# caishiqing/voice-tts

Measured on AMD Instinct MI355X. Metric: audio_seconds_per_second, higher is better.
Workload: dtype bf16

## Files before the change

### include/ixtts_hip.h

```cpp
#ifndef IXTTS_HIP_H
#define IXTTS_HIP_H

#include <stddef.h>
#include <stdint.h>

#ifdef __cplusplus
extern "C" {
#endif

#define IXTTS_OK 0
#define IXTTS_ERR_ARG (-1)
#define IXTTS_ERR_HIP (-2)
#define IXTTS_ERR_STATE (-3)
#define IXTTS_ERR_NOMEM (-4)
#define IXTTS_ERR_NAME (-5)

const char* ixtts_version(void);
const char* ixtts_last_error(void);

int ixtts_aa_snake_f32(const float* x_dev, float* y_dev, const float* up12_dev, const float* down12_dev,
                       const float* log_alpha_dev, const float* log_beta_dev, int B, int C, int T, void* stream);

size_t ixtts_attn_full_workspace_bytes(int B, int H, int T);
int ixtts_attn_full_f32(const float* q_dev, const float* k_dev, const float* v_dev, float* out_dev, int B, int H, int T,
                        int head_dim, long stride_b, long stride_t, long stride_h, long ostride_b, long ostride_t,
                        long ostride_h, float scale, void* workspace_dev, size_t workspace_bytes, void* stream);

size_t ixtts_attn_full_varlen_workspace_bytes(int nseq, int H, int total_tiles);
int ixtts_attn_full_varlen_f32(const float* q_dev, const float* k_dev, const float* v_dev, float* out_dev, const int* table_dev, int nseq,
                               int total_tiles, int n_work, int H, int head_dim, long stride_t, long stride_h, long ostride_t, long ostride_h,
                               float scale, void* workspace_dev, size_t workspace_bytes, void* stream);

int ixtts_adaln_rmsnorm_f32(const float* x_dev, const float* wb_dev, const float* g_dev, float* out_dev, int B, int T, int H, float eps,
                            void* stream);
int ixtts_ln_modulate_f32(const float* x_dev, const float* shift_scale_dev, float* out_dev, int B, int T, int H, float eps, void* stream);
int ixtts_rope_qk_f32(float* qkv_dev, const float* cos_sin_dev, int B, int T, int H, int head_dim, void* stream);
int ixtts_swiglu_f32(const float* u_dev, float* out_dev, long rows, int F, void* stream);
int ixtts_wn_gate_f32(const float* a_dev, const float* g_dev, float* out_dev, int B, int C, int T, long g_stride, int g_offset, void* stream);
int ixtts_wn_gate_rows_f32(const float* a_dev, const float* g_dev, float* out_dev, long rows, int C, long rows_per_batch, int B, long g_stride,
                           int g_offset, void* stream);
int ixtts_reflect_halo_rows_f32(float* p_dev, int B, int T, int C, int left, int right, void* stream);

int ixtts_adaln_rmsnorm_varlen_f32(const float* x_dev, const float* wb_dev, const float* g_dev, float* out_dev, const int* seq_off_dev, int nseq,
                                   long rows, int H, float eps, void* stream);
int ixtts_ln_modulate_varlen_f32(const float* x_dev, const float* shift_scale_dev, float* out_dev, const int* seq_off_dev, int nseq, long rows, int H,
                                 float eps, void* stream);
int ixtts_rope_qk_varlen_f32(float* qkv_dev, const float* cos_sin_dev, const int* seq_off_dev, int nseq, long rows, int H, int head_dim, void* stream);
int ixtts_wn_gate_rows_varlen_f32(const float* a_dev, const float* g_dev, float* out_dev, long rows, int C, const int* seq_off_dev, int nseq,
                                  long g_stride, int g_offset, void* stream);
int ixtts_reflect_halo_rows_varlen_f32(float* p_dev, const int* seq_off_dev, int nseq, int C, int left, int right, void* stream);

size_t ixtts_gemm_x6_packed_bytes(int N, int K);
int ixtts_gemm_x6_pack(const float* w_dev, void* packed_dev, int N, int K, void* stream);
long ixtts_gemm_x6_rows_padded(long rows);
int ixtts_gemm_x6_split(const float* a_dev, long lda, void* planes_dev, long rows, int K, void* stream);
int ixtts_gemm_x6_f32(const void* a_planes_dev, long rows_total, long row0, const void* packed_dev, const float* bias_dev, float* c_dev, long ldc,
                      int M, int N, int K, int accumulate, int tile, void* stream);
int ixtts_gemm_x6_pair_f32(const void* a_planes_dev, long rows_total, long row0, int taps, const void* packed_dev, const float* bias_dev,
                           const float* gate_dev, long gate_ld, long rows_per_batch, int nbatch, float* c_dev, long ldc, int M, int N, int K,
                           int epilogue, int tile, void* stream);
int ixtts_gemm_x6_pair_gate_varlen_f32(const void* a_planes_dev, long rows_total, long row0, int taps, const void* packed_dev, const float* bias_dev,
                                       const float* gate_dev, long gate_ld, const int* seq_off_dev, int nseq, float* c_dev, long ldc, int M, int N,
                                       int K, int tile, void* stream);

#define IXTTS_BIGVGAN_MAX_STAGES 8
#define IXTTS_BIGVGAN_MAX_RESK 4

typedef struct ixtts_bigvgan_cfg {
  int num_mels;
  int upsample_initial_channel;
  int n_stages;
  int upsample_rates[IXTTS_BIGVGAN_MAX_STAGES];
  int upsample_kernel_sizes[IXTTS_BIGVGAN_MAX_STAGES];
  int n_resblock_kernels;
  int resblock_kernel_sizes[IXTTS_BIGVGAN_MAX_RESK];
  int resblock_dilations[IXTTS_BIGVGAN_MAX_RESK][3];
  int max_frames;
  int fast_sin;
} ixtts_bigvgan_cfg;

typedef struct ixtts_bigvgan ixtts_bigvgan;

int ixtts_bigvgan_create(ixtts_bigvgan** out, const ixtts_bigvgan_cfg* cfg);
int ixtts_bigvgan_set_tensor(ixtts_bigvgan* h, const char* name, const float* data_host, const int64_t* shape, int ndim);
int ixtts_bigvgan_finalize(ixtts_bigvgan* h);
int ixtts_bigvgan_arena(ixtts_bigvgan* h, void** ptr_dev, size_t* bytes);
int ixtts_bigvgan_adopt_arena(ixtts_bigvgan* h);
int ixtts_bigvgan_forward(ixtts_bigvgan* h, const float* mel_dev, int B, int F, float* wav_dev, void* stream);
double ixtts_bigvgan_flops(const ixtts_bigvgan* h, int B, int F);
int ixtts_bigvgan_destroy(ixtts_bigvgan* h);

#define IXTTS_DTYPE_F32 0
#define IXTTS_DTYPE_BF16 1

typedef struct ixtts_gpt_cfg {
  int model_dim;
  int layers;
  int heads;
  int n_mel_codes;
  int n_mel_pos;
  int n_text_tokens;
  int n_text_pos;
  int start_mel_token;
  int stop_mel_token;
  int max_seq;
  int max_batch;
  int weight_dtype;
} ixtts_gpt_cfg;

typedef struct ixtts_sampler_cfg {
  float repetition_penalty;
  float temperature;
  int top_k;
  float top_p;
  int do_sample;
  int suppress_stop;
  uint64_t seed;
  float typical_mass;
  float length_penalty;
} ixtts_sampler_cfg;

typedef struct ixtts_gpt ixtts_gpt;

int ixtts_gpt_create(ixtts_gpt** out, const ixtts_gpt_cfg* cfg);
int ixtts_gpt_set_tensor(ixtts_gpt* h, const char* name, const float* data_host, const int64_t* shape, int ndim);
int ixtts_gpt_finalize(ixtts_gpt* h);
int ixtts_gpt_arena(ixtts_gpt* h, void** ptr_dev, size_t* bytes);
int ixtts_gpt_adopt_arena(ixtts_gpt* h);
int ixtts_gpt_share_arena(ixtts_gpt* h, ixtts_gpt* owner);

int ixtts_gpt_prefill(ixtts_gpt* h, int b, const float* embeds_dev, int n_rows, int n_left_pad, void* stream);
int ixtts_gpt_decode(ixtts_gpt* h, int n_active, int n_steps, const ixtts_sampler_cfg* sc, void* stream);
int ixtts_gpt_read(ixtts_gpt* h, int b, int32_t* ids_host, int cap, int* n_ids, int* finished, void* stream);
int ixtts_gpt_read_logits(ixtts_gpt* h, int b, float* logits_host, void* stream);
int ixtts_gpt_read_probs(ixtts_gpt* h, int b, float* probs_host, void* stream);
int ixtts_gpt_force_next(ixtts_gpt* h, int b, int32_t token, void* stream);

int ixtts_gpt_beam_begin(ixtts_gpt* h, int num_beams, void* stream);
int ixtts_gpt_beam_decode(ixtts_gpt* h, int n_steps, const ixtts_sampler_cfg* sc, void* stream);
int ixtts_gpt_beam_read(ixtts_gpt* h, int max_new, int32_t* ids_host, int cap, int* n_ids, int* done, float* score,
                        float* beam_scores_host, int32_t* last_tokens_host, int32_t* beam_idx_host, void* stream);
int ixtts_gpt_beam_force(ixtts_gpt* h, const int32_t* picks_host, int n, void* stream);

int ixtts_gpt_beam_begin_group(ixtts_gpt* h, int group, int num_beams, uint64_t rng_stream, void* stream);
int ixtts_gpt_beam_park_group(ixtts_gpt* h, int group, void* stream);
int ixtts_gpt_beam_decode_groups(ixtts_gpt* h, int n_groups, int n_steps, const ixtts_sampler_cfg* sc, void* stream);
int ixtts_gpt_beam_read_group(ixtts_gpt* h, int group, int max_new, int32_t* ids_host, int cap, int* n_ids, int* done, float* score,
                              float* beam_scores_host, int32_t* last_tokens_host, int32_t* beam_idx_host, void* stream);
int ixtts_gpt_beam_force_group(ixtts_gpt* h, int group, const int32_t* picks_host, int n, void* stream);

int ixtts_gpt_latent(ixtts_gpt* h, const float* prefix_dev, int n_prefix, const int32_t* codes_dev, int n,
                     float* latent_dev, void* stream);

int ixtts_gpt_bench_gemv(ixtts_gpt* h, int which, int layer, int batch, void* stream);
double ixtts_gpt_step_bytes(const ixtts_gpt* h, int B, int S);

int ixtts_gpt_max_batch(void);

int ixtts_gpt_destroy(ixtts_gpt* h);

#define IXTTS_DTYPE_F16 2
#define IXTTS_QWEN_TOPK_MAX 64
#define IXTTS_QWEN_MAX_EOS 8

typedef struct ixtts_qwen_cfg {
  int hidden_size;
  int layers;
  int heads;
  int kv_heads;
  int head_dim;
  int intermediate_size;
  int vocab_size;
  float rms_norm_eps;
  float rope_theta;
  int tie_word_embeddings;
  int max_seq;
  int weight_dtype;
  int n_eos;
  int eos_ids[IXTTS_QWEN_MAX_EOS];
} ixtts_qwen_cfg;

typedef struct ixtts_qwen_sampling {
  int do_sample;
  float temperature;
  int top_k;
  float top_p;
  uint64_t seed;
} ixtts_qwen_sampling;

typedef struct ixtts_qwen ixtts_qwen;

int ixtts_qwen_create(ixtts_qwen** out, const ixtts_qwen_cfg* cfg);
int ixtts_qwen_set_tensor(ixtts_qwen* h, const char* name, const float* data_host, const int64_t* shape, int ndim);
int ixtts_qwen_finalize(ixtts_qwen* h);
int ixtts_qwen_prefill(ixtts_qwen* h, const int32_t* ids_host, int n, void* stream);
int ixtts_qwen_step(ixtts_qwen* h, int n_steps, const ixtts_qwen_sampling* sc, void* stream);
int ixtts_qwen_read(ixtts_qwen* h, int32_t* ids_host, int cap, int* n_ids, int* finished, void* stream);
int ixtts_qwen_generate(ixtts_qwen* h, int max_new, const ixtts_qwen_sampling* sc, int32_t* ids_host, int cap, int* n_ids,
                        int* finished, void* stream);
int ixtts_qwen_read_logits(ixtts_qwen* h, float* logits_host, void* stream);
int ixtts_qwen_read_kept(ixtts_qwen* h, int32_t* ids_host, float* probs_host, int cap, int* n_kept, void* stream);
int ixtts_qwen_draw(ixtts_qwen* h, uint64_t seed, int n, int32_t* ids_host, void* stream);
double ixtts_qwen_step_bytes(const ixtts_qwen* h, int S);
int ixtts_qwen_destroy(ixtts_qwen* h);

#ifdef __cplusplus
}
#endif
#endif
```

### voice-tts_amd/_lib.py

```python
import ctypes as C
import os

HERE = os.path.dirname(os.path.abspath(__file__))
LIB_PATH = os.environ.get("IXTTS_LIB") or os.path.join(HERE, "libixtts_hip.so")

MAX_STAGES = 8
MAX_RESK = 4


class BigVGANCfg(C.Structure):
    _fields_ = [
        ("num_mels", C.c_int), ("upsample_initial_channel", C.c_int), ("n_stages", C.c_int),
        ("upsample_rates", C.c_int * MAX_STAGES), ("upsample_kernel_sizes", C.c_int * MAX_STAGES),
        ("n_resblock_kernels", C.c_int), ("resblock_kernel_sizes", C.c_int * MAX_RESK),
        ("resblock_dilations", (C.c_int * 3) * MAX_RESK), ("max_frames", C.c_int), ("fast_sin", C.c_int),
    ]


class GptCfg(C.Structure):
    _fields_ = [
        ("model_dim", C.c_int), ("layers", C.c_int), ("heads", C.c_int), ("n_mel_codes", C.c_int),
        ("n_mel_pos", C.c_int), ("n_text_tokens", C.c_int), ("n_text_pos", C.c_int),
        ("start_mel_token", C.c_int), ("stop_mel_token", C.c_int), ("max_seq", C.c_int),
        ("max_batch", C.c_int), ("weight_dtype", C.c_int),
    ]


class SamplerCfg(C.Structure):
    _fields_ = [
        ("repetition_penalty", C.c_float), ("temperature", C.c_float), ("top_k", C.c_int),
        ("top_p", C.c_float), ("do_sample", C.c_int), ("suppress_stop", C.c_int), ("seed", C.c_uint64),
        ("typical_mass", C.c_float), ("length_penalty", C.c_float),
    ]


QWEN_TOPK_MAX = 64
QWEN_MAX_EOS = 8


class QwenCfg(C.Structure):
    _fields_ = [
        ("hidden_size", C.c_int), ("layers", C.c_int), ("heads", C.c_int), ("kv_heads", C.c_int), ("head_dim", C.c_int),
        ("intermediate_size", C.c_int), ("vocab_size", C.c_int), ("rms_norm_eps", C.c_float), ("rope_theta", C.c_float),
        ("tie_word_embeddings", C.c_int), ("max_seq", C.c_int), ("weight_dtype", C.c_int), ("n_eos", C.c_int),
        ("eos_ids", C.c_int * QWEN_MAX_EOS),
    ]


class QwenSampling(C.Structure):
    _fields_ = [("do_sample", C.c_int), ("temperature", C.c_float), ("top_k", C.c_int), ("top_p", C.c_float), ("seed", C.c_uint64)]


_P = C.c_void_p
SYMBOLS = {
    "ixtts_version": (C.c_char_p, []),
    "ixtts_last_error": (C.c_char_p, []),
    "ixtts_aa_snake_f32": (C.c_int, [_P, _P, _P, _P, _P, _P, C.c_int, C.c_int, C.c_int, _P]),
    "ixtts_attn_full_workspace_bytes": (C.c_size_t, [C.c_int, C.c_int, C.c_int]),
    "ixtts_attn_full_f32": (C.c_int, [_P, _P, _P, _P, C.c_int, C.c_int, C.c_int, C.c_int, C.c_long, C.c_long, C.c_long, C.c_long, C.c_long,
                                      C.c_long, C.c_float, _P, C.c_size_t, _P]),
    "ixtts_attn_full_varlen_workspace_bytes": (C.c_size_t, [C.c_int, C.c_int, C.c_int]),
    "ixtts_attn_full_varlen_f32": (C.c_int, [_P, _P, _P, _P, _P, C.c_int, C.c_int, C.c_int, C.c_int, C.c_int, C.c_long, C.c_long, C.c_long, C.c_long,
                                             C.c_float, _P, C.c_size_t, _P]),
    "ixtts_adaln_rmsnorm_f32": (C.c_int, [_P, _P, _P, _P, C.c_int, C.c_int, C.c_int, C.c_float, _P]),
    "ixtts_ln_modulate_f32": (C.c_int, [_P, _P, _P, C.c_int, C.c_int, C.c_int, C.c_float, _P]),
    "ixtts_rope_qk_f32": (C.c_int, [_P, _P, C.c_int, C.c_int, C.c_int, C.c_int, _P]),
    "ixtts_swiglu_f32": (C.c_int, [_P, _P, C.c_long, C.c_int, _P]),
    "ixtts_wn_gate_f32": (C.c_int, [_P, _P, _P, C.c_int, C.c_int, C.c_int, C.c_long, C.c_int, _P]),
    "ixtts_wn_gate_rows_f32": (C.c_int, [_P, _P, _P, C.c_long, C.c_int, C.c_long, C.c_int, C.c_long, C.c_int, _P]),
    "ixtts_reflect_halo_rows_f32": (C.c_int, [_P, C.c_int, C.c_int, C.c_int, C.c_int, C.c_int, _P]),
    "ixtts_adaln_rmsnorm_varlen_f32": (C.c_int, [_P, _P, _P, _P, _P, C.c_int, C.c_long, C.c_int, C.c_float, _P]),
    "ixtts_ln_modulate_varlen_f32": (C.c_int, [_P, _P, _P, _P, C.c_int, C.c_long, C.c_int, C.c_float, _P]),
    "ixtts_rope_qk_varlen_f32": (C.c_int, [_P, _P, _P, C.c_int, C.c_long, C.c_int, C.c_int, _P]),
    "ixtts_wn_gate_rows_varlen_f32": (C.c_int, [_P, _P, _P, C.c_long, C.c_int, _P, C.c_int, C.c_long, C.c_int, _P]),
    "ixtts_reflect_halo_rows_varlen_f32": (C.c_int, [_P, _P, C.c_int, C.c_int, C.c_int, C.c_int, _P]),
    "ixtts_gemm_x6_packed_bytes": (C.c_size_t, [C.c_int, C.c_int]),
    "ixtts_gemm_x6_pack": (C.c_int, [_P, _P, C.c_int, C.c_int, _P]),
    "ixtts_gemm_x6_rows_padded": (C.c_long, [C.c_long]),
    "ixtts_gemm_x6_split": (C.c_int, [_P, C.c_long, _P, C.c_long, C.c_int, _P]),
    "ixtts_gemm_x6_f32": (C.c_int, [_P, C.c_long, C.c_long, _P, _P, _P, C.c_long, C.c_int, C.c_int, C.c_int, C.c_int, C.c_int, _P]),
    "ixtts_gemm_x6_pair_f32": (C.c_int, [_P, C.c_long, C.c_long, C.c_int, _P, _P, _P, C.c_long, C.c_long, C.c_int, _P, C.c_long, C.c_int, C.c_int,
                                         C.c_int, C.c_int, C.c_int, _P]),
    "ixtts_gemm_x6_pair_gate_varlen_f32": (C.c_int, [_P, C.c_long, C.c_long, C.c_int, _P, _P, _P, C.c_long, _P, C.c_int, _P, C.c_long, C.c_int, C.c_int,
                                                     C.c_int, C.c_int, _P]),
    "ixtts_bigvgan_create": (C.c_int, [C.POINTER(_P), C.POINTER(BigVGANCfg)]),
    "ixtts_bigvgan_set_tensor": (C.c_int, [_P, C.c_char_p, _P, C.POINTER(C.c_int64), C.c_int]),
    "ixtts_bigvgan_finalize": (C.c_int, [_P]),
    "ixtts_bigvgan_arena": (C.c_int, [_P, C.POINTER(_P), C.POINTER(C.c_size_t)]),
    "ixtts_bigvgan_adopt_arena": (C.c_int, [_P]),
    "ixtts_bigvgan_forward": (C.c_int, [_P, _P, C.c_int, C.c_int, _P, _P]),
    "ixtts_bigvgan_flops": (C.c_double, [_P, C.c_int, C.c_int]),
    "ixtts_bigvgan_destroy": (C.c_int, [_P]),
    "ixtts_gpt_create": (C.c_int, [C.POINTER(_P), C.POINTER(GptCfg)]),
    "ixtts_gpt_set_tensor": (C.c_int, [_P, C.c_char_p, _P, C.POINTER(C.c_int64), C.c_int]),
    "ixtts_gpt_finalize": (C.c_int, [_P]),
    "ixtts_gpt_arena": (C.c_int, [_P, C.POINTER(_P), C.POINTER(C.c_size_t)]),
    "ixtts_gpt_adopt_arena": (C.c_int, [_P]),
    "ixtts_gpt_share_arena": (C.c_int, [_P, _P]),
    "ixtts_gpt_prefill": (C.c_int, [_P, C.c_int, _P, C.c_int, C.c_int, _P]),
    "ixtts_gpt_decode": (C.c_int, [_P, C.c_int, C.c_int, C.POINTER(SamplerCfg), _P]),
    "ixtts_gpt_read": (C.c_int, [_P, C.c_int, _P, C.c_int, C.POINTER(C.c_int), C.POINTER(C.c_int), _P]),
    "ixtts_gpt_read_logits": (C.c_int, [_P, C.c_int, _P, _P]),
    "ixtts_gpt_beam_begin": (C.c_int, [_P, C.c_int, _P]),
    "ixtts_gpt_beam_decode": (C.c_int, [_P, C.c_int, C.POINTER(SamplerCfg), _P]),
    "ixtts_gpt_beam_read": (C.c_int, [_P, C.c_int, _P, C.c_int, C.POINTER(C.c_int), C.POINTER(C.c_int), C.POINTER(C.c_float), _P, _P, _P, _P]),
    "ixtts_gpt_beam_force": (C.c_int, [_P, _P, C.c_int, _P]),
    "ixtts_gpt_beam_begin_group": (C.c_int, [_P, C.c_int, C.c_int, C.c_uint64, _P]),
    "ixtts_gpt_beam_park_group": (C.c_int, [_P, C.c_int, _P]),
    "ixtts_gpt_beam_decode_groups": (C.c_int, [_P, C.c_int, C.c_int, C.POINTER(SamplerCfg), _P]),
    "ixtts_gpt_beam_read_group": (C.c_int, [_P, C.c_int, C.c_int, _P, C.c_int, C.POINTER(C.c_int), C.POINTER(C.c_int), C.POINTER(C.c_float), _P, _P, _P, _P]),
    "ixtts_gpt_beam_force_group": (C.c_int, [_P, C.c_int, _P, C.c_int, _P]),
    "ixtts_gpt_read_probs": (C.c_int, [_P, C.c_int, _P, _P]),
    "ixtts_gpt_force_next": (C.c_int, [_P, C.c_int, C.c_int32, _P]),
    "ixtts_gpt_latent": (C.c_int, [_P, _P, C.c_int, _P, C.c_int, _P, _P]),
    "ixtts_gpt_bench_gemv": (C.c_int, [_P, C.c_int, C.c_int, C.c_int, _P]),
    "ixtts_gpt_step_bytes": (C.c_double, [_P, C.c_int, C.c_int]),
    "ixtts_gpt_max_batch": (C.c_int, []),
    "ixtts_gpt_destroy": (C.c_int, [_P]),
    "ixtts_qwen_create": (C.c_int, [C.POINTER(_P), C.POINTER(QwenCfg)]),
    "ixtts_qwen_set_tensor": (C.c_int, [_P, C.c_char_p, _P, C.POINTER(C.c_int64), C.c_int]),
    "ixtts_qwen_finalize": (C.c_int, [_P]),
    "ixtts_qwen_prefill": (C.c_int, [_P, _P, C.c_int, _P]),
    "ixtts_qwen_step": (C.c_int, [_P, C.c_int, C.POINTER(QwenSampling), _P]),
    "ixtts_qwen_read": (C.c_int, [_P, _P, C.c_int, C.POINTER(C.c_int), C.POINTER(C.c_int), _P]),
    "ixtts_qwen_generate": (C.c_int, [_P, C.c_int, C.POINTER(QwenSampling), _P, C.c_int, C.POINTER(C.c_int), C.POINTER(C.c_int), _P]),
    "ixtts_qwen_read_logits": (C.c_int, [_P, _P, _P]),
    "ixtts_qwen_read_kept": (C.c_int, [_P, _P, _P, C.c_int, C.POINTER(C.c_int), _P]),
    "ixtts_qwen_draw": (C.c_int, [_P, C.c_uint64, C.c_int, _P, _P]),
    "ixtts_qwen_step_bytes": (C.c_double, [_P, C.c_int]),
    "ixtts_qwen_destroy": (C.c_int, [_P]),
}

_lib = None


class IxttsError(RuntimeError):
    pass


def lib():
    global _lib
    if _lib is not None:
        return _lib
    import torch

    if not os.path.exists(LIB_PATH):
        raise IxttsError(
            f"{LIB_PATH} not found: build it with `python -m voice_tts_amd.build` "
            "(there is no CPU fallback for the HIP path)")
    L = C.CDLL(LIB_PATH)
    for name, (res, args) in SYMBOLS.items():
        fn = getattr(L, name)
        fn.restype = res
        fn.argtypes = args
    _lib = L
    return L


def check(rc, what=""):
    if rc != 0:
        msg = lib().ixtts_last_error().decode(errors="replace")
        raise IxttsError(f"{what} failed with code {rc}: {msg}")


def max_batch():
    return int(lib().ixtts_gpt_max_batch())


def current_stream_ptr():
    import torch

    return C.c_void_p(torch.cuda.current_stream().cuda_stream)
```

### voice-tts_amd/csrc/attn_full.h

```cpp
#pragma once
#include "common.h"

namespace ixtts {

constexpr int AF_D = 64;
constexpr int AF_KT = 64;
constexpr int AF_QW = 32;
constexpr int AF_WAVES = 4;
constexpr int AF_KSPLIT = 4;
constexpr int AX_KSPLIT = 5;

struct AttnFullArgs {
  const float* q;
  const float* k;
  const float* v;
  float* o;
  long sb, st, sh;
  long osb, ost, osh;
  int B, H, T;
  float scale;
  float* ws_o;
  float* ws_ml;
  const int* vl_tab;
  int vl_n, vl_tiles;
};

size_t attn_full_x3_plane_bytes(int B, int H, int T);
int launch_attn_full_x3(const AttnFullArgs& a, void* planes, bool split, hipStream_t st);
int launch_attn_full_x3_varlen(const AttnFullArgs& a, void* planes, int n_work, hipStream_t st);

}
```

### voice-tts_amd/csrc/attn_full.hip

```cpp
#include "attn_full.h"

namespace ixtts {

typedef float f32x16 __attribute__((ext_vector_type(16)));

constexpr int AF_KP = AF_D + 4;

template <int KSPLIT>
__global__ __launch_bounds__(AF_WAVES * 64) void attn_full_f32_kernel(AttnFullArgs a) {
  __shared__ __attribute__((aligned(16))) float Ks[AF_KT * AF_KP];
  __shared__ __attribute__((aligned(16))) float Vs[AF_KT * AF_D];
  const int bh = blockIdx.y, b = bh / a.H, h = bh % a.H;
  const int lane = threadIdx.x & 63, wave = threadIdx.x >> 6;
  const int l31 = lane & 31, lh = lane >> 5;
  const int q0 = blockIdx.x * (AF_WAVES * AF_QW) + wave * AF_QW;
  const float* qb = a.q + b * a.sb + h * a.sh;
  const float* kb = a.k + b * a.sb + h * a.sh;
  const float* vb = a.v + b * a.sb + h * a.sh;

  float qr[AF_D / 2];
  {
    const int qi = min(q0 + l31, a.T - 1);
    const float* qp = qb + (long)qi * a.st + 4 * lh;
    const float qs = a.scale * 1.4426950408889634f;
#pragma unroll
    for (int m = 0; m < AF_D / 8; ++m) {
      const float4 t = *reinterpret_cast<const float4*>(qp + 8 * m);
      qr[4 * m] = t.x * qs; qr[4 * m + 1] = t.y * qs; qr[4 * m + 2] = t.z * qs; qr[4 * m + 3] = t.w * qs;
    }
  }
  f32x16 ot[2];
#pragma unroll
  for (int j = 0; j < 2; ++j)
#pragma unroll
    for (int r = 0; r < 16; ++r) ot[j][r] = 0.f;
  float m_run = -INFINITY, l_run = 0.f;

  const int n_tiles = (a.T + AF_KT - 1) / AF_KT;
  const int tiles_per = (n_tiles + KSPLIT - 1) / KSPLIT;
  const int t_lo = (KSPLIT > 1 ? blockIdx.z * tiles_per : 0) * AF_KT;
  const int t_hi = KSPLIT > 1 ? min(a.T, t_lo + tiles_per * AF_KT) : a.T;
  for (int t0 = t_lo; t0 < t_hi; t0 += AF_KT) {
    __syncthreads();
#pragma unroll
    for (int i = 0; i < (AF_KT * AF_D / 4) / (AF_WAVES * 64); ++i) {
      const int idx = threadIdx.x + i * (AF_WAVES * 64);
      const int key = idx >> 4, c4 = idx & 15;
      const int t = min(t0 + key, a.T - 1);
      const float4 kv = *reinterpret_cast<const float4*>(kb + (long)t * a.st + c4 * 4);
      const float4 vv = *reinterpret_cast<const float4*>(vb + (long)t * a.st + c4 * 4);
      *reinterpret_cast<float4*>(Ks + key * AF_KP + c4 * 4) = kv;
      *reinterpret_cast<float4*>(Vs + key * AF_D + c4 * 4) = vv;
    }
    __syncthreads();

    f32x16 st[2];
#pragma unroll
    for (int j = 0; j < 2; ++j)
#pragma unroll
      for (int r = 0; r < 16; ++r) st[j][r] = 0.f;
    const float* kp0 = Ks + l31 * AF_KP + 4 * lh;
    const float* kp1 = kp0 + 32 * AF_KP;
    float4 ka[2][2];
    ka[0][0] = *reinterpret_cast<const float4*>(kp0);
    ka[0][1] = *reinterpret_cast<const float4*>(kp1);
#pragma unroll
    for (int m = 0; m < AF_D / 8; ++m) {
      if (m + 1 < AF_D / 8) {
        ka[(m + 1) & 1][0] = *reinterpret_cast<const float4*>(kp0 + 8 * (m + 1));
        ka[(m + 1) & 1][1] = *reinterpret_cast<const float4*>(kp1 + 8 * (m + 1));
      }
#pragma unroll
      for (int j = 0; j < 2; ++j) {
        const float4 kk4 = ka[m & 1][j];
        st[j] = __builtin_amdgcn_mfma_f32_32x32x2f32(kk4.x, qr[4 * m], st[j], 0, 0, 0);
        st[j] = __builtin_amdgcn_mfma_f32_32x32x2f32(kk4.y, qr[4 * m + 1], st[j], 0, 0, 0);
        st[j] = __builtin_amdgcn_mfma_f32_32x32x2f32(kk4.z, qr[4 * m + 2], st[j], 0, 0, 0);
        st[j] = __builtin_amdgcn_mfma_f32_32x32x2f32(kk4.w, qr[4 * m + 3], st[j], 0, 0, 0);
      }
    }
    if (t0 + AF_KT > a.T) {
#pragma unroll
      for (int j = 0; j < 2; ++j)
#pragma unroll
        for (int r = 0; r < 16; ++r) {
          const int key = t0 + j * 32 + (r & 3) + 8 * (r >> 2) + 4 * lh;
          if (key >= a.T) st[j][r] = -INFINITY;
        }
    }
    float tmax = -INFINITY;
#pragma unroll
    for (int j = 0; j < 2; ++j)
#pragma unroll
      for (int r = 0; r < 16; ++r) tmax = fmaxf(tmax, st[j][r]);
    tmax = fmaxf(tmax, __shfl_xor(tmax, 32, 64));
    const float mn = fmaxf(m_run, tmax);
    const float alpha = __builtin_amdgcn_exp2f(m_run - mn);
    m_run = mn;
    if (alpha != 1.0f) {
#pragma unroll
      for (int j = 0; j < 2; ++j)
#pragma unroll
        for (int r = 0; r < 16; ++r) ot[j][r] *= alpha;
    }
    float psum = 0.f;
    const float* vp = Vs + (4 * lh) * AF_D + l31;
    float va[2][2];
    va[0][0] = vp[0];
    va[0][1] = vp[32];
#pragma unroll
    for (int s = 0; s < 32; ++s) {
      const int j = s >> 4, r = s & 15;
      if (s + 1 < 32) {
        const int j1 = (s + 1) >> 4, r1 = (s + 1) & 15;
        const float* vrow = vp + (j1 * 32 + (r1 & 3) + 8 * (r1 >> 2)) * AF_D;
        va[(s + 1) & 1][0] = vrow[0];
        va[(s + 1) & 1][1] = vrow[32];
      }
      const float pv = __builtin_amdgcn_exp2f(st[j][r] - mn);
      psum += pv;
      ot[0] = __builtin_amdgcn_mfma_f32_32x32x2f32(va[s & 1][0], pv, ot[0], 0, 0, 0);
      ot[1] = __builtin_amdgcn_mfma_f32_32x32x2f32(va[s & 1][1], pv, ot[1], 0, 0, 0);
    }
    psum += __shfl_xor(psum, 32, 64);
    l_run = l_run * alpha + psum;
  }
  const int qi = q0 + l31;
  if (qi < a.T) {
    if constexpr (KSPLIT == 1) {
      const float inv = 1.0f / l_run;
      float* op = a.o + b * a.osb + (long)qi * a.ost + h * a.osh;
#pragma unroll
      for (int j = 0; j < 2; ++j)
#pragma unroll
        for (int r = 0; r < 16; ++r) op[j * 32 + (r & 3) + 8 * (r >> 2) + 4 * lh] = ot[j][r] * inv;
    } else {
      const long row = ((long)blockIdx.z * a.B * a.H + bh) * a.T + qi;
      float* op = a.ws_o + row * AF_D;
#pragma unroll
      for (int j = 0; j < 2; ++j)
#pragma unroll
        for (int r = 0; r < 16; ++r) op[j * 32 + (r & 3) + 8 * (r >> 2) + 4 * lh] = ot[j][r];
      if (lh == 0) *reinterpret_cast<float2*>(a.ws_ml + row * 2) = make_float2(m_run, l_run);
    }
  }
}

template <int KSPLIT>
__global__ __launch_bounds__(256) void attn_full_merge_kernel(AttnFullArgs a) {
  const long row = (long)blockIdx.x * 4 + (threadIdx.x >> 6);
  const long rows = (long)a.B * a.H * a.T;
  if (row >= rows) return;
  const int d = threadIdx.x & 63;
  const int t = (int)(row % a.T);
  const int bh = (int)(row / a.T), b = bh / a.H, h = bh % a.H;
  float2 ml[KSPLIT];
  float o[KSPLIT];
  float M = -INFINITY;
#pragma unroll
  for (int sp = 0; sp < KSPLIT; ++sp) {
    ml[sp] = *reinterpret_cast<const float2*>(a.ws_ml + ((long)sp * rows + row) * 2);
    o[sp] = a.ws_o[((long)sp * rows + row) * AF_D + d];
    M = fmaxf(M, ml[sp].x);
  }
  float L = 0.f, O = 0.f;
#pragma unroll
  for (int sp = 0; sp < KSPLIT; ++sp) {
    const float w = (ml[sp].x > -INFINITY) ? __builtin_amdgcn_exp2f(ml[sp].x - M) : 0.f;
    L = fmaf(ml[sp].y, w, L);
    O = fmaf(o[sp], w, O);
  }
  a.o[b * a.osb + (long)t * a.ost + h * a.osh + d] = O / L;
}

}

static size_t attn_partials_bytes(int B, int H, int T) {
  return (size_t)(ixtts::AF_KSPLIT > ixtts::AX_KSPLIT ? ixtts::AF_KSPLIT : ixtts::AX_KSPLIT) * B * H * T * (ixtts::AF_D + 2) * sizeof(float);
}

extern "C" size_t ixtts_attn_full_workspace_bytes(int B, int H, int T) {
  if (B <= 0 || H <= 0 || T <= 0) return 0;
  return attn_partials_bytes(B, H, T) + ixtts::attn_full_x3_plane_bytes(B, H, T);
}

extern "C" int ixtts_attn_full_f32(const float* q_dev, const float* k_dev, const float* v_dev, float* out_dev, int B, int H, int T,
                                   int head_dim, long stride_b, long stride_t, long stride_h, long ostride_b, long ostride_t,
                                   long ostride_h, float scale, void* workspace_dev, size_t workspace_bytes, void* stream) {
  using namespace ixtts;
  IX_ARG(q_dev && k_dev && v_dev && out_dev, "attn_full: null pointer");
  IX_ARG(head_dim == AF_D, "attn_full: head_dim %d (only 64 is built)", head_dim);
  IX_ARG(B > 0 && H > 0 && T > 0 && (long)B * H <= 65535, "attn_full: bad shape B=%d H=%d T=%d", B, H, T);
  IX_ARG(stride_t % 4 == 0 && stride_h % 4 == 0 && stride_b % 4 == 0, "attn_full: strides must keep 16-byte row alignment");
  AttnFullArgs a;
  a.q = q_dev; a.k = k_dev; a.v = v_dev; a.o = out_dev;
  a.sb = stride_b; a.st = stride_t; a.sh = stride_h;
  a.osb = ostride_b; a.ost = ostride_t; a.osh = ostride_h;
  a.B = B; a.H = H; a.T = T; a.scale = scale;
  a.ws_o = a.ws_ml = nullptr;
  a.vl_tab = nullptr; a.vl_n = a.vl_tiles = 0;
  hipStream_t st = (hipStream_t)stream;
  const int qblocks = ceil_div(T, AF_WAVES * AF_QW);
  const bool have_ws = workspace_dev && workspace_bytes >= ixtts_attn_full_workspace_bytes(B, H, T);
  const bool split = have_ws && T > 4 * AF_KT && (long)qblocks * B * H * AF_WAVES < 2 * 1024;
  const char* mode = getenv("IXTTS_ATTN_FULL");
  const bool x3 = !(mode && strcmp(mode, "f32") == 0);
  const bool use_x3 = x3 && have_ws;
  if (split) {
    a.ws_o = reinterpret_cast<float*>(workspace_dev);
    a.ws_ml = a.ws_o + (size_t)(use_x3 ? AX_KSPLIT : AF_KSPLIT) * B * H * T * AF_D;
  }
  if (use_x3) {
    IX_TRY(launch_attn_full_x3(a, reinterpret_cast<char*>(workspace_dev) + attn_partials_bytes(B, H, T), split, st));
    if (split) {
      const long rows = (long)B * H * T;
      hipLaunchKernelGGL(attn_full_merge_kernel<AX_KSPLIT>, dim3((unsigned)((rows + 3) / 4)), dim3(256), 0, st, a);
    }
    IX_HIP(hipGetLastError());
    return IXTTS_OK;
  }
  if (split) {
    hipLaunchKernelGGL(attn_full_f32_kernel<AF_KSPLIT>, dim3(qblocks, B * H, AF_KSPLIT), dim3(AF_WAVES * 64), 0, st, a);
    const long rows = (long)B * H * T;
    hipLaunchKernelGGL(attn_full_merge_kernel<AF_KSPLIT>, dim3((unsigned)((rows + 3) / 4)), dim3(256), 0, st, a);
  } else {
    hipLaunchKernelGGL(attn_full_f32_kernel<1>, dim3(qblocks, B * H), dim3(AF_WAVES * 64), 0, st, a);
  }
  IX_HIP(hipGetLastError());
  return IXTTS_OK;
}

extern "C" size_t ixtts_attn_full_varlen_workspace_bytes(int nseq, int H, int total_tiles) {
  if (nseq <= 0 || H <= 0 || total_tiles <= 0) return 0;
  return (size_t)H * total_tiles * 2 * 3 * 8 * 64 * 16;
}

extern "C" int ixtts_attn_full_varlen_f32(const float* q_dev, const float* k_dev, const float* v_dev, float* out_dev, const int* table_dev, int nseq,
                                          int total_tiles, int n_work, int H, int head_dim, long stride_t, long stride_h, long ostride_t, long ostride_h,
                                          float scale, void* workspace_dev, size_t workspace_bytes, void* stream) {
  using namespace ixtts;
  IX_ARG(q_dev && k_dev && v_dev && out_dev && table_dev, "attn_full_varlen: null pointer");
  IX_ARG(head_dim == AF_D, "attn_full_varlen: head_dim %d (only 64 is built)", head_dim);
  IX_ARG(nseq > 0 && total_tiles >= nseq && n_work >= nseq && H > 0 && H <= 65535, "attn_full_varlen: bad shape nseq=%d tiles=%d work=%d H=%d", nseq, total_tiles,
         n_work, H);
  IX_ARG(stride_t % 4 == 0 && stride_h % 4 == 0, "attn_full_varlen: strides must keep 16-byte row alignment");
  IX_ARG(workspace_dev && workspace_bytes >= ixtts_attn_full_varlen_workspace_bytes(nseq, H, total_tiles), "attn_full_varlen: workspace of %zu bytes, %zu needed",
         workspace_bytes, ixtts_attn_full_varlen_workspace_bytes(nseq, H, total_tiles));
  AttnFullArgs a;
  a.q = q_dev; a.k = k_dev; a.v = v_dev; a.o = out_dev;
  a.sb = 0; a.st = stride_t; a.sh = stride_h;
  a.osb = 0; a.ost = ostride_t; a.osh = ostride_h;
  a.B = 1; a.H = H; a.T = 0; a.scale = scale;
  a.ws_o = a.ws_ml = nullptr;
  a.vl_tab = table_dev; a.vl_n = nseq; a.vl_tiles = total_tiles;
  return launch_attn_full_x3_varlen(a, workspace_dev, n_work, (hipStream_t)stream);
}
```

### voice-tts_amd/csrc/attn_full_x3.hip

```cpp
#include "attn_full.h"

namespace ixtts {

typedef float ax_f32x16 __attribute__((ext_vector_type(16)));
typedef __bf16 ax_bf16x8 __attribute__((ext_vector_type(8)));

constexpr int AX_TILE_UNITS = 3 * 8 * 64;
constexpr int AX_WAVES = 4;

size_t attn_full_x3_plane_bytes(int B, int H, int T) {
  const size_t tiles = (size_t)(T + AF_KT - 1) / AF_KT;
  return (size_t)B * H * tiles * 2 * AX_TILE_UNITS * 16;
}


template <bool VL>
__global__ __launch_bounds__(256) void attn_kv_planes_kernel(AttnFullArgs a, uint4* __restrict__ planes) {
  int tile = blockIdx.x, T = a.T;
  const float *kb, *vb;
  uint4* kdst;
  if constexpr (VL) {
    const int h = blockIdx.y, s = seq_of_row(a.vl_tab + a.vl_n + 1, a.vl_n, tile);
    const int r0 = a.vl_tab[s];
    T = a.vl_tab[s + 1] - r0;
    kdst = planes + ((size_t)h * a.vl_tiles + tile) * 2 * AX_TILE_UNITS;
    tile -= a.vl_tab[a.vl_n + 1 + s];
    kb = a.k + (long)r0 * a.st + h * a.sh;
    vb = a.v + (long)r0 * a.st + h * a.sh;
  } else {
    const int bh = blockIdx.y, b = bh / a.H, h = bh % a.H;
    const int n_tiles = (a.T + AF_KT - 1) / AF_KT;
    kb = a.k + b * a.sb + h * a.sh;
    vb = a.v + b * a.sb + h * a.sh;
    kdst = planes + ((size_t)bh * n_tiles + tile) * 2 * AX_TILE_UNITS;
  }
  uint4* vdst = kdst + AX_TILE_UNITS;
  const int t0 = tile * AF_KT;
#pragma unroll
  for (int i = 0; i < 2; ++i) {
    const int uid = threadIdx.x + 256 * i;
    const int key = uid >> 3, oct = uid & 7;
    const int t = t0 + key;
    float v[8];
    const float4* src = reinterpret_cast<const float4*>(kb + (long)min(t, T - 1) * a.st + 8 * oct);
    const float4 x0 = src[0], x1 = src[1];
    const bool live = t < T;
    v[0] = live ? x0.x : 0.f; v[1] = live ? x0.y : 0.f; v[2] = live ? x0.z : 0.f; v[3] = live ? x0.w : 0.f;
    v[4] = live ? x1.x : 0.f; v[5] = live ? x1.y : 0.f; v[6] = live ? x1.z : 0.f; v[7] = live ? x1.w : 0.f;
    uint4 ph, pm, pl;
    split8_bf16x3(v, ph, pm, pl);
    kdst[(0 * 8 + oct) * 64 + key] = ph;
    kdst[(1 * 8 + oct) * 64 + key] = pm;
    kdst[(2 * 8 + oct) * 64 + key] = pl;
  }
#pragma unroll
  for (int i = 0; i < 2; ++i) {
    const int d = threadIdx.x & 63, un = (threadIdx.x >> 6) + 4 * i;
    const int j = un >> 2, u = (un >> 1) & 1, kh = un & 1;
    float v[8];
#pragma unroll
    for (int e = 0; e < 8; ++e) {
      const int t = t0 + 32 * j + 16 * u + 8 * (e >> 2) + 4 * kh + (e & 3);
      const float x = vb[(long)min(t, T - 1) * a.st + d];
      v[e] = t < T ? x : 0.f;
    }
    uint4 ph, pm, pl;
    split8_bf16x3(v, ph, pm, pl);
    vdst[(0 * 8 + un) * 64 + d] = ph;
    vdst[(1 * 8 + un) * 64 + d] = pm;
    vdst[(2 * 8 + un) * 64 + d] = pl;
  }
}

template <int KSPLIT, bool VL = false>
__global__ __launch_bounds__(AX_WAVES * 64, 3) void attn_full_x3_kernel(AttnFullArgs a, const uint4* __restrict__ planes) {
  __shared__ uint4 Ks[AX_TILE_UNITS];
  __shared__ uint4 Vs[AX_TILE_UNITS];
  static_assert(!VL || KSPLIT == 1, "packed sequences: no key-range split");
  const int lane = threadIdx.x & 63, wave = threadIdx.x >> 6;
  const int l31 = lane & 31, lh = lane >> 5;
  int T, q0;
  const float* qb;
  const uint4* pb;
  float* ob;
  if constexpr (VL) {
    const int h = blockIdx.y;
    const int* w = a.vl_tab + 2 * (a.vl_n + 1) + 2 * blockIdx.x;
    const int s = w[0], r0 = a.vl_tab[s];
    T = a.vl_tab[s + 1] - r0;
    q0 = w[1] * (AX_WAVES * AF_QW) + wave * AF_QW;
    qb = a.q + (long)r0 * a.st + h * a.sh;
    pb = planes + ((size_t)h * a.vl_tiles + a.vl_tab[a.vl_n + 1 + s]) * 2 * AX_TILE_UNITS;
    ob = a.o + (long)r0 * a.ost + h * a.osh;
  } else {
    const int bh = blockIdx.y, b = bh / a.H, h = bh % a.H;
    T = a.T;
    q0 = blockIdx.x * (AX_WAVES * AF_QW) + wave * AF_QW;
    qb = a.q + b * a.sb + h * a.sh;
    pb = planes + (size_t)bh * ((T + AF_KT - 1) / AF_KT) * 2 * AX_TILE_UNITS;
    ob = a.o + b * a.osb + h * a.osh;
  }

  uint4 qp[4][3];
  {
    const int qi = min(q0 + l31, T - 1);
    const float* qrow = qb + (long)qi * a.st + 8 * lh;
    const float qs = a.scale * 1.4426950408889634f;
#pragma unroll
    for (int s = 0; s < 4; ++s) {
      const float4 x0 = *reinterpret_cast<const float4*>(qrow + 16 * s), x1 = *reinterpret_cast<const float4*>(qrow + 16 * s + 4);
      const float v[8] = {x0.x * qs, x0.y * qs, x0.z * qs, x0.w * qs, x1.x * qs, x1.y * qs, x1.z * qs, x1.w * qs};
      split8_bf16x3(v, qp[s][0], qp[s][1], qp[s][2]);
    }
  }
  ax_f32x16 ot[2];
#pragma unroll
  for (int j = 0; j < 2; ++j)
#pragma unroll
    for (int r = 0; r < 16; ++r) ot[j][r] = 0.f;
  float m_run = -INFINITY, l_run = 0.f;

  const int n_tiles = (T + AF_KT - 1) / AF_KT;
  const int tiles_per = (n_tiles + KSPLIT - 1) / KSPLIT;
  const int tile_lo = KSPLIT > 1 ? blockIdx.z * tiles_per : 0;
  const int tile_hi = KSPLIT > 1 ? min(n_tiles, tile_lo + tiles_per) : n_tiles;
  auto issue_tile = [&](const uint4* __restrict__ src, uint4* __restrict__ dst) {
#pragma unroll
    for (int i = 0; i < AX_TILE_UNITS / (AX_WAVES * 64); ++i)
      __builtin_amdgcn_global_load_lds((const __attribute__((address_space(1))) void*)(src + i * (AX_WAVES * 64) + threadIdx.x),
                                       (__attribute__((address_space(3))) void*)(dst + i * (AX_WAVES * 64) + wave * 64), 16, 0, 0);
  };
  auto mfma6x2 = [](ax_f32x16& c0, ax_f32x16& c1, const uint4 (&A0)[3], const uint4 (&A1)[3], const uint4 (&Bq)[3]) {
    const ax_bf16x8 a0h = __builtin_bit_cast(ax_bf16x8, A0[0]), a0m = __builtin_bit_cast(ax_bf16x8, A0[1]), a0l = __builtin_bit_cast(ax_bf16x8, A0[2]);
    const ax_bf16x8 a1h = __builtin_bit_cast(ax_bf16x8, A1[0]), a1m = __builtin_bit_cast(ax_bf16x8, A1[1]), a1l = __builtin_bit_cast(ax_bf16x8, A1[2]);
    const ax_bf16x8 bh_ = __builtin_bit_cast(ax_bf16x8, Bq[0]), bm = __builtin_bit_cast(ax_bf16x8, Bq[1]), bl = __builtin_bit_cast(ax_bf16x8, Bq[2]);
    c0 = __builtin_amdgcn_mfma_f32_32x32x16_bf16(a0l, bh_, c0, 0, 0, 0);
    c1 = __builtin_amdgcn_mfma_f32_32x32x16_bf16(a1l, bh_, c1, 0, 0, 0);
    c0 = __builtin_amdgcn_mfma_f32_32x32x16_bf16(a0h, bl, c0, 0, 0, 0);
    c1 = __builtin_amdgcn_mfma_f32_32x32x16_bf16(a1h, bl, c1, 0, 0, 0);
    c0 = __builtin_amdgcn_mfma_f32_32x32x16_bf16(a0m, bm, c0, 0, 0, 0);
    c1 = __builtin_amdgcn_mfma_f32_32x32x16_bf16(a1m, bm, c1, 0, 0, 0);
    c0 = __builtin_amdgcn_mfma_f32_32x32x16_bf16(a0m, bh_, c0, 0, 0, 0);
    c1 = __builtin_amdgcn_mfma_f32_32x32x16_bf16(a1m, bh_, c1, 0, 0, 0);
    c0 = __builtin_amdgcn_mfma_f32_32x32x16_bf16(a0h, bm, c0, 0, 0, 0);
    c1 = __builtin_amdgcn_mfma_f32_32x32x16_bf16(a1h, bm, c1, 0, 0, 0);
    c0 = __builtin_amdgcn_mfma_f32_32x32x16_bf16(a0h, bh_, c0, 0, 0, 0);
    c1 = __builtin_amdgcn_mfma_f32_32x32x16_bf16(a1h, bh_, c1, 0, 0, 0);
  };
  if (tile_lo < tile_hi) issue_tile(pb + (size_t)tile_lo * 2 * AX_TILE_UNITS, Ks);
  for (int tile = tile_lo; tile < tile_hi; ++tile) {
    const int t0 = tile * AF_KT;
    asm volatile("s_waitcnt vmcnt(0)" ::: "memory");
    __builtin_amdgcn_s_barrier();
    issue_tile(pb + ((size_t)tile * 2 + 1) * AX_TILE_UNITS, Vs);
    ax_f32x16 st[2];
#pragma unroll
    for (int j = 0; j < 2; ++j)
#pragma unroll
      for (int r = 0; r < 16; ++r) st[j][r] = 0.f;
    const uint4* kp = Ks + lh * 64 + l31;
#pragma unroll
    for (int s = 0; s < 4; ++s) {
      uint4 ka[2][3];
#pragma unroll
      for (int j = 0; j < 2; ++j)
#pragma unroll
        for (int pl = 0; pl < 3; ++pl) ka[j][pl] = kp[(pl * 8 + 2 * s) * 64 + 32 * j];
      mfma6x2(st[0], st[1], ka[0], ka[1], qp[s]);
    }
    if (t0 + AF_KT > T) {
#pragma unroll
      for (int j = 0; j < 2; ++j)
#pragma unroll
        for (int r = 0; r < 16; ++r) {
          const int key = t0 + j * 32 + (r & 3) + 8 * (r >> 2) + 4 * lh;
          if (key >= T) st[j][r] = -INFINITY;
        }
    }
    float tmax = -INFINITY;
#pragma unroll
    for (int j = 0; j < 2; ++j)
#pragma unroll
      for (int r = 0; r < 16; ++r) tmax = fmaxf(tmax, st[j][r]);
    tmax = fmaxf(tmax, __shfl_xor(tmax, 32, 64));
    const float mn = fmaxf(m_run, tmax);
    const float alpha = __builtin_amdgcn_exp2f(m_run - mn);
    m_run = mn;
    if (alpha != 1.0f) {
#pragma unroll
      for (int j = 0; j < 2; ++j)
#pragma unroll
        for (int r = 0; r < 16; ++r) ot[j][r] *= alpha;
    }
    float psum = 0.f;
#pragma unroll
    for (int j = 0; j < 2; ++j)
#pragma unroll
      for (int r = 0; r < 16; ++r) {
        st[j][r] = __builtin_amdgcn_exp2f(st[j][r] - mn);
        psum += st[j][r];
      }
    psum += __shfl_xor(psum, 32, 64);
    l_run = l_run * alpha + psum;
    asm volatile("s_waitcnt vmcnt(0)" ::: "memory");
    __builtin_amdgcn_s_barrier();
    if (tile + 1 < tile_hi) issue_tile(pb + (size_t)(tile + 1) * 2 * AX_TILE_UNITS, Ks);
    const uint4* vp = Vs + lh * 64 + l31;
#pragma unroll
    for (int s = 0; s < 4; ++s) {
      const int j = s >> 1, u = s & 1;
      uint4 va[2][3];
#pragma unroll
      for (int dh = 0; dh < 2; ++dh)
#pragma unroll
        for (int pl = 0; pl < 3; ++pl) va[dh][pl] = vp[(pl * 8 + 2 * s) * 64 + 32 * dh];
      uint4 pp[3];
      {
        float pv[8];
#pragma unroll
        for (int e = 0; e < 8; ++e) pv[e] = st[j][8 * u + e];
        split8_bf16x3(pv, pp[0], pp[1], pp[2]);
      }
      mfma6x2(ot[0], ot[1], va[0], va[1], pp);
    }
  }
  asm volatile("s_waitcnt vmcnt(0)" ::: "memory");
  const int qi = q0 + l31;
  if (qi < T) {
    if constexpr (KSPLIT == 1) {
      const float inv = 1.0f / l_run;
      float* op = ob + (long)qi * a.ost;
#pragma unroll
      for (int j = 0; j < 2; ++j)
#pragma unroll
        for (int r = 0; r < 16; ++r) op[j * 32 + (r & 3) + 8 * (r >> 2) + 4 * lh] = ot[j][r] * inv;
    } else {
      const long row = ((long)blockIdx.z * a.B * a.H + blockIdx.y) * T + qi;
      float* op = a.ws_o + row * AF_D;
#pragma unroll
      for (int j = 0; j < 2; ++j)
#pragma unroll
        for (int r = 0; r < 16; ++r) op[j * 32 + (r & 3) + 8 * (r >> 2) + 4 * lh] = ot[j][r];
      if (lh == 0) *reinterpret_cast<float2*>(a.ws_ml + row * 2) = make_float2(m_run, l_run);
    }
  }
}

int launch_attn_full_x3(const AttnFullArgs& a, void* planes, bool split, hipStream_t st) {
  const int n_tiles = ceil_div(a.T, AF_KT);
  const int qblocks = ceil_div(a.T, AX_WAVES * AF_QW);
  uint4* pl = reinterpret_cast<uint4*>(planes);
  hipLaunchKernelGGL(attn_kv_planes_kernel<false>, dim3(n_tiles, a.B * a.H), dim3(256), 0, st, a, pl);
  if (split) hipLaunchKernelGGL(attn_full_x3_kernel<AX_KSPLIT>, dim3(qblocks, a.B * a.H, AX_KSPLIT), dim3(AX_WAVES * 64), 0, st, a, (const uint4*)pl);
  else hipLaunchKernelGGL(attn_full_x3_kernel<1>, dim3(qblocks, a.B * a.H), dim3(AX_WAVES * 64), 0, st, a, (const uint4*)pl);
  IX_HIP(hipGetLastError());
  return IXTTS_OK;
}

int launch_attn_full_x3_varlen(const AttnFullArgs& a, void* planes, int n_work, hipStream_t st) {
  uint4* pl = reinterpret_cast<uint4*>(planes);
  hipLaunchKernelGGL(attn_kv_planes_kernel<true>, dim3(a.vl_tiles, a.H), dim3(256), 0, st, a, pl);
  hipLaunchKernelGGL((attn_full_x3_kernel<1, true>), dim3(n_work, a.H), dim3(AX_WAVES * 64), 0, st, a, (const uint4*)pl);
  IX_HIP(hipGetLastError());
  return IXTTS_OK;
}

}
```

### voice-tts_amd/csrc/dit_ops.hip

```cpp
#include "common.h"

namespace ixtts {

constexpr int ROW_NV = 8;

template <bool CENTER>
__global__ __launch_bounds__(256) void row_norm_mod_kernel(const float* __restrict__ x, const float* __restrict__ mw, const float* __restrict__ mb,
                                                           const float* __restrict__ g, float* __restrict__ out, long rows, int T, int H, long mstride,
                                                           float eps, float wadd, const int* __restrict__ seq_off = nullptr, int nseq = 0) {
  const long row = (long)blockIdx.x * 4 + (threadIdx.x >> 6);
  if (row >= rows) return;
  const int lane = threadIdx.x & 63;
  const int H4 = H >> 2;
  const float4* xr = reinterpret_cast<const float4*>(x + row * H);
  float4 v[ROW_NV];
#pragma unroll
  for (int i = 0; i < ROW_NV; ++i) {
    const int c = lane + 64 * i;
    v[i] = (c < H4) ? xr[c] : make_float4(0.f, 0.f, 0.f, 0.f);
  }
  float mean = 0.f;
  if constexpr (CENTER) {
    float s = 0.f;
#pragma unroll
    for (int i = 0; i < ROW_NV; ++i) s += (v[i].x + v[i].y) + (v[i].z + v[i].w);
    mean = wave_sum(s) / (float)H;
  }
  float q = 0.f;
#pragma unroll
  for (int i = 0; i < ROW_NV; ++i) {
    const int c = lane + 64 * i;
    if (c < H4) {
      const float a = v[i].x - mean, b = v[i].y - mean, cc = v[i].z - mean, d = v[i].w - mean;
      q += (a * a + b * b) + (cc * cc + d * d);
    }
  }
  const float rstd = 1.0f / sqrtf(wave_sum(q) / (float)H + eps);
  const long bidx = seq_off ? seq_of_row(seq_off, nseq, row) : row / T;
  const float4* w4 = reinterpret_cast<const float4*>(mw + bidx * mstride);
  const float4* b4 = reinterpret_cast<const float4*>(mb + bidx * mstride);
  const float4* g4 = reinterpret_cast<const float4*>(g);
  float4* o4 = reinterpret_cast<float4*>(out + row * H);
#pragma unroll
  for (int i = 0; i < ROW_NV; ++i) {
    const int c = lane + 64 * i;
    if (c < H4) {
      const float4 w = w4[c], b = b4[c];
      float4 n = make_float4((v[i].x - mean) * rstd, (v[i].y - mean) * rstd, (v[i].z - mean) * rstd, (v[i].w - mean) * rstd);
      if (g) {
        const float4 gg = g4[c];
        n.x *= gg.x; n.y *= gg.y; n.z *= gg.z; n.w *= gg.w;
      }
      o4[c] = make_float4(fmaf(w.x + wadd, n.x, b.x), fmaf(w.y + wadd, n.y, b.y), fmaf(w.z + wadd, n.z, b.z), fmaf(w.w + wadd, n.w, b.w));
    }
  }
}

__global__ __launch_bounds__(256) void rope_qk_kernel(float* __restrict__ qkv, const float2* __restrict__ tab, long rows, int T, int H, int hd,
                                                      const int* __restrict__ seq_off = nullptr, int nseq = 0) {
  const int per_row = (2 * H) >> 2;
  const long idx = (long)blockIdx.x * 256 + threadIdx.x;
  if (idx >= rows * per_row) return;
  const long row = idx / per_row;
  const int c4 = (int)(idx % per_row);
  const int col = c4 * 4;
  const int t = seq_off ? (int)(row - seq_off[seq_of_row(seq_off, nseq, row)]) : (int)(row % T);
  const int p = (col % hd) >> 1;
  float4* ptr = reinterpret_cast<float4*>(qkv + row * 3 * H + col);
  const float4 v = *ptr;
  const float2 f0 = tab[(long)t * (hd >> 1) + p], f1 = tab[(long)t * (hd >> 1) + p + 1];
  *ptr = make_float4(v.x * f0.x - v.y * f0.y, v.y * f0.x + v.x * f0.y, v.z * f1.x - v.w * f1.y, v.w * f1.x + v.z * f1.y);
}

__global__ __launch_bounds__(256) void swiglu_kernel(const float* __restrict__ u, float* __restrict__ out, long rows, int Fd) {
  const int F4 = Fd >> 2;
  const long idx = (long)blockIdx.x * 256 + threadIdx.x;
  if (idx >= rows * F4) return;
  const long row = idx / F4;
  const int c = (int)(idx % F4);
  const float4 a = reinterpret_cast<const float4*>(u + row * 2 * Fd)[c];
  const float4 b = reinterpret_cast<const float4*>(u + row * 2 * Fd + Fd)[c];
  auto f = [](float x, float y) { return x / (1.0f + expf(-x)) * y; };
  reinterpret_cast<float4*>(out + row * Fd)[c] = make_float4(f(a.x, b.x), f(a.y, b.y), f(a.z, b.z), f(a.w, b.w));
}

__global__ __launch_bounds__(256) void wn_gate_kernel(const float* __restrict__ a, const float* __restrict__ gvec, float* __restrict__ out, int B, int C, int T,
                                                      long gstride, int goff) {
  const long idx = (long)blockIdx.x * 256 + threadIdx.x;
  const long n = (long)B * C * T;
  if (idx >= n) return;
  const int t = (int)(idx % T);
  const int c = (int)((idx / T) % C);
  const int b = (int)(idx / ((long)T * C));
  const float ga = gvec[b * gstride + goff + c], gb = gvec[b * gstride + goff + C + c];
  const float xa = a[((long)b * 2 * C + c) * T + t] + ga;
  const float xb = a[((long)b * 2 * C + C + c) * T + t] + gb;
  out[idx] = tanhf(xa) * (1.0f / (1.0f + expf(-xb)));
}

__global__ __launch_bounds__(256) void wn_gate_rows_kernel(const float* __restrict__ a, const float* __restrict__ gvec, float* __restrict__ out, long rows, int C,
                                                           long rows_per_batch, int B, long gstride, int goff, const int* __restrict__ seq_off = nullptr) {
  const long idx = (long)blockIdx.x * 256 + threadIdx.x;
  const int C4 = C >> 2;
  if (idx >= rows * C4) return;
  const long r = idx / C4;
  const int c = (int)(idx % C4) * 4;
  const int b = seq_off ? seq_of_row(seq_off, B, r) : (int)min(r / rows_per_batch, (long)B - 1);
  const float4 xa = *reinterpret_cast<const float4*>(a + r * 2 * C + c);
  const float4 xb = *reinterpret_cast<const float4*>(a + r * 2 * C + C + c);
  const float4 ga = *reinterpret_cast<const float4*>(gvec + b * gstride + goff + c);
  const float4 gb = *reinterpret_cast<const float4*>(gvec + b * gstride + goff + C + c);
  float4 o;
  o.x = tanhf(xa.x + ga.x) * (1.0f / (1.0f + expf(-(xb.x + gb.x))));
  o.y = tanhf(xa.y + ga.y) * (1.0f / (1.0f + expf(-(xb.y + gb.y))));
  o.z = tanhf(xa.z + ga.z) * (1.0f / (1.0f + expf(-(xb.z + gb.z))));
  o.w = tanhf(xa.w + ga.w) * (1.0f / (1.0f + expf(-(xb.w + gb.w))));
  *reinterpret_cast<float4*>(out + r * C + c) = o;
}

__global__ __launch_bounds__(256) void reflect_halo_rows_kernel(float* __restrict__ p, int B, int T, int C, int left, int right) {
  const int C4 = C >> 2;
  const long idx = (long)blockIdx.x * 256 + threadIdx.x;
  const long per_b = (long)(left + right) * C4;
  if (idx >= per_b * B) return;
  const int b = (int)(idx / per_b);
  const int h = (int)((idx % per_b) / C4);
  const int c = (int)(idx % C4) * 4;
  float* base = p + (long)b * (left + T + right) * C;
  const int dst = h < left ? left - 1 - h : left + T + (h - left);
  const int src = h < left ? left + h + 1 : left + T - 2 - (h - left);
  *reinterpret_cast<float4*>(base + (long)dst * C + c) = *reinterpret_cast<const float4*>(base + (long)src * C + c);
}

__global__ __launch_bounds__(256) void reflect_halo_rows_varlen_kernel(float* __restrict__ p, const int* __restrict__ off, int n, int C, int left, int right) {
  const int C4 = C >> 2;
  const long idx = (long)blockIdx.x * 256 + threadIdx.x;
  const long per_b = (long)(left + right) * C4;
  if (idx >= per_b * n) return;
  const int b = (int)(idx / per_b);
  const int h = (int)((idx % per_b) / C4);
  const int c = (int)(idx % C4) * 4;
  const int o0 = off[b], T = off[b + 1] - o0 - left - right;
  if (T <= left || T <= right) return;
  float* base = p + (long)o0 * C;
  const int dst = h < left ? left - 1 - h : left + T + (h - left);
  const int src = h < left ? left + h + 1 : left + T - 2 - (h - left);
  *reinterpret_cast<float4*>(base + (long)dst * C + c) = *reinterpret_cast<const float4*>(base + (long)src * C + c);
}

}

using namespace ixtts;

extern "C" int ixtts_adaln_rmsnorm_f32(const float* x_dev, const float* wb_dev, const float* g_dev, float* out_dev, int B, int T, int H, float eps,
                                       void* stream) {
  IX_ARG(x_dev && wb_dev && g_dev && out_dev, "adaln_rmsnorm: null pointer");
  IX_ARG(B > 0 && T > 0 && H > 0 && H % 4 == 0 && H <= 64 * ROW_NV * 4, "adaln_rmsnorm: bad shape B=%d T=%d H=%d", B, T, H);
  const long rows = (long)B * T;
  hipLaunchKernelGGL(row_norm_mod_kernel<false>, dim3((unsigned)((rows + 3) / 4)), dim3(256), 0, (hipStream_t)stream, x_dev, wb_dev, wb_dev + H, g_dev, out_dev,
                     rows, T, H, (long)2 * H, eps, 0.0f);
  IX_HIP(hipGetLastError());
  return IXTTS_OK;
}

extern "C" int ixtts_ln_modulate_f32(const float* x_dev, const float* shift_scale_dev, float* out_dev, int B, int T, int H, float eps, void* stream) {
  IX_ARG(x_dev && shift_scale_dev && out_dev, "ln_modulate: null pointer");
  IX_ARG(B > 0 && T > 0 && H > 0 && H % 4 == 0 && H <= 64 * ROW_NV * 4, "ln_modulate: bad shape B=%d T=%d H=%d", B, T, H);
  const long rows = (long)B * T;
  hipLaunchKernelGGL(row_norm_mod_kernel<true>, dim3((unsigned)((rows + 3) / 4)), dim3(256), 0, (hipStream_t)stream, x_dev, shift_scale_dev + H, shift_scale_dev,
                     (const float*)nullptr, out_dev, rows, T, H, (long)2 * H, eps, 1.0f);
  IX_HIP(hipGetLastError());
  return IXTTS_OK;
}

extern "C" int ixtts_rope_qk_f32(float* qkv_dev, const float* cos_sin_dev, int B, int T, int H, int head_dim, void* stream) {
  IX_ARG(qkv_dev && cos_sin_dev, "rope_qk: null pointer");
  IX_ARG(B > 0 && T > 0 && H > 0 && head_dim > 0 && head_dim % 4 == 0 && H % head_dim == 0, "rope_qk: bad shape B=%d T=%d H=%d hd=%d", B, T, H, head_dim);
  const long n = (long)B * T * (2 * H / 4);
  hipLaunchKernelGGL(rope_qk_kernel, dim3((unsigned)((n + 255) / 256)), dim3(256), 0, (hipStream_t)stream, qkv_dev, reinterpret_cast<const float2*>(cos_sin_dev),
                     (long)B * T, T, H, head_dim);
  IX_HIP(hipGetLastError());
  return IXTTS_OK;
}

extern "C" int ixtts_swiglu_f32(const float* u_dev, float* out_dev, long rows, int F, void* stream) {
  IX_ARG(u_dev && out_dev, "swiglu: null pointer");
  IX_ARG(rows > 0 && F > 0 && F % 4 == 0, "swiglu: bad shape rows=%ld F=%d", rows, F);
  const long n = rows * (F / 4);
  hipLaunchKernelGGL(swiglu_kernel, dim3((unsigned)((n + 255) / 256)), dim3(256), 0, (hipStream_t)stream, u_dev, out_dev, rows, F);
  IX_HIP(hipGetLastError());
  return IXTTS_OK;
}

extern "C" int ixtts_wn_gate_f32(const float* a_dev, const float* g_dev, float* out_dev, int B, int C, int T, long g_stride, int g_offset, void* stream) {
  IX_ARG(a_dev && g_dev && out_dev, "wn_gate: null pointer");
  IX_ARG(B > 0 && C > 0 && T > 0 && g_offset >= 0, "wn_gate: bad shape B=%d C=%d T=%d", B, C, T);
  const long n = (long)B * C * T;
  hipLaunchKernelGGL(wn_gate_kernel, dim3((unsigned)((n + 255) / 256)), dim3(256), 0, (hipStream_t)stream, a_dev, g_dev, out_dev, B, C, T, g_stride, g_offset);
  IX_HIP(hipGetLastError());
  return IXTTS_OK;
}

extern "C" int ixtts_wn_gate_rows_f32(const float* a_dev, const float* g_dev, float* out_dev, long rows, int C, long rows_per_batch, int B, long g_stride,
                                      int g_offset, void* stream) {
  IX_ARG(a_dev && g_dev && out_dev, "wn_gate_rows: null pointer");
  IX_ARG(rows > 0 && C > 0 && C % 4 == 0 && rows_per_batch > 0 && B > 0 && g_offset >= 0 && g_offset % 4 == 0 && g_stride % 4 == 0,
         "wn_gate_rows: bad shape rows=%ld C=%d rows_per_batch=%ld B=%d", rows, C, rows_per_batch, B);
  const long n = rows * (C / 4);
  hipLaunchKernelGGL(wn_gate_rows_kernel, dim3((unsigned)((n + 255) / 256)), dim3(256), 0, (hipStream_t)stream, a_dev, g_dev, out_dev, rows, C, rows_per_batch, B,
                     g_stride, g_offset);
  IX_HIP(hipGetLastError());
  return IXTTS_OK;
}

extern "C" int ixtts_reflect_halo_rows_f32(float* p_dev, int B, int T, int C, int left, int right, void* stream) {
  IX_ARG(p_dev, "reflect_halo_rows: null pointer");
  IX_ARG(B > 0 && C > 0 && C % 4 == 0 && left >= 0 && right >= 0 && T > left && T > right, "reflect_halo_rows: bad shape B=%d T=%d C=%d left=%d right=%d", B, T, C,
         left, right);
  const long n = (long)B * (left + right) * (C / 4);
  if (n == 0) return IXTTS_OK;
  hipLaunchKernelGGL(reflect_halo_rows_kernel, dim3((unsigned)((n + 255) / 256)), dim3(256), 0, (hipStream_t)stream, p_dev, B, T, C, left, right);
  IX_HIP(hipGetLastError());
  return IXTTS_OK;
}


extern "C" int ixtts_adaln_rmsnorm_varlen_f32(const float* x_dev, const float* wb_dev, const float* g_dev, float* out_dev, const int* seq_off_dev, int nseq,
                                              long rows, int H, float eps, void* stream) {
  IX_ARG(x_dev && wb_dev && g_dev && out_dev && seq_off_dev, "adaln_rmsnorm_varlen: null pointer");
  IX_ARG(nseq > 0 && rows > 0 && H > 0 && H % 4 == 0 && H <= 64 * ROW_NV * 4, "adaln_rmsnorm_varlen: bad shape nseq=%d rows=%ld H=%d", nseq, rows, H);
  hipLaunchKernelGGL(row_norm_mod_kernel<false>, dim3((unsigned)((rows + 3) / 4)), dim3(256), 0, (hipStream_t)stream, x_dev, wb_dev, wb_dev + H, g_dev, out_dev,
                     rows, 1, H, (long)2 * H, eps, 0.0f, seq_off_dev, nseq);
  IX_HIP(hipGetLastError());
  return IXTTS_OK;
}

extern "C" int ixtts_ln_modulate_varlen_f32(const float* x_dev, const float* shift_scale_dev, float* out_dev, const int* seq_off_dev, int nseq, long rows, int H,
                                            float eps, void* stream) {
  IX_ARG(x_dev && shift_scale_dev && out_dev && seq_off_dev, "ln_modulate_varlen: null pointer");
  IX_ARG(nseq > 0 && rows > 0 && H > 0 && H % 4 == 0 && H <= 64 * ROW_NV * 4, "ln_modulate_varlen: bad shape nseq=%d rows=%ld H=%d", nseq, rows, H);
  hipLaunchKernelGGL(row_norm_mod_kernel<true>, dim3((unsigned)((rows + 3) / 4)), dim3(256), 0, (hipStream_t)stream, x_dev, shift_scale_dev + H, shift_scale_dev,
                     (const float*)nullptr, out_dev, rows, 1, H, (long)2 * H, eps, 1.0f, seq_off_dev, nseq);
  IX_HIP(hipGetLastError());
  return IXTTS_OK;
}

extern "C" int ixtts_rope_qk_varlen_f32(float* qkv_dev, const float* cos_sin_dev, const int* seq_off_dev, int nseq, long rows, int H, int head_dim, void* stream) {
  IX_ARG(qkv_dev && cos_sin_dev && seq_off_dev, "rope_qk_varlen: null pointer");
  IX_ARG(nseq > 0 && rows > 0 && H > 0 && head_dim > 0 && head_dim % 4 == 0 && H % head_dim == 0, "rope_qk_varlen: bad shape nseq=%d rows=%ld H=%d hd=%d", nseq,
         rows, H, head_dim);
  const long n = rows * (2 * H / 4);
  hipLaunchKernelGGL(rope_qk_kernel, dim3((unsigned)((n + 255) / 256)), dim3(256), 0, (hipStream_t)stream, qkv_dev, reinterpret_cast<const float2*>(cos_sin_dev),
                     rows, 1, H, head_dim, seq_off_dev, nseq);
  IX_HIP(hipGetLastError());
  return IXTTS_OK;
}

extern "C" int ixtts_wn_gate_rows_varlen_f32(const float* a_dev, const float* g_dev, float* out_dev, long rows, int C, const int* seq_off_dev, int nseq,
                                             long g_stride, int g_offset, void* stream) {
  IX_ARG(a_dev && g_dev && out_dev && seq_off_dev, "wn_gate_rows_varlen: null pointer");
  IX_ARG(rows > 0 && C > 0 && C % 4 == 0 && nseq > 0 && g_offset >= 0 && g_offset % 4 == 0 && g_stride % 4 == 0,
         "wn_gate_rows_varlen: bad shape rows=%ld C=%d nseq=%d", rows, C, nseq);
  const long n = rows * (C / 4);
  hipLaunchKernelGGL(wn_gate_rows_kernel, dim3((unsigned)((n + 255) / 256)), dim3(256), 0, (hipStream_t)stream, a_dev, g_dev, out_dev, rows, C, (long)1, nseq,
                     g_stride, g_offset, seq_off_dev);
  IX_HIP(hipGetLastError());
  return IXTTS_OK;
}

extern "C" int ixtts_reflect_halo_rows_varlen_f32(float* p_dev, const int* seq_off_dev, int nseq, int C, int left, int right, void* stream) {
  IX_ARG(p_dev && seq_off_dev, "reflect_halo_rows_varlen: null pointer");
  IX_ARG(nseq > 0 && C > 0 && C % 4 == 0 && left >= 0 && right >= 0, "reflect_halo_rows_varlen: bad shape nseq=%d C=%d left=%d right=%d", nseq, C, left, right);
  const long n = (long)nseq * (left + right) * (C / 4);
  if (n == 0) return IXTTS_OK;
  hipLaunchKernelGGL(reflect_halo_rows_varlen_kernel, dim3((unsigned)((n + 255) / 256)), dim3(256), 0, (hipStream_t)stream, p_dev, seq_off_dev, nseq, C, left,
                     right);
  IX_HIP(hipGetLastError());
  return IXTTS_OK;
}
```

### voice-tts_amd/csrc/gemm_x6.hip

```cpp
#include "common.h"

namespace ixtts {

typedef float gx_f32x16 __attribute__((ext_vector_type(16)));
typedef __bf16 gx_bf16x8 __attribute__((ext_vector_type(8)));
typedef float gx_f32x4 __attribute__((ext_vector_type(4)));
typedef unsigned int gx_u32x4 __attribute__((ext_vector_type(4)));


__global__ void gemm_x6_pack_kernel(const float* __restrict__ w, uint4* __restrict__ out, int N, int K, int Npad) {
  const long total = (long)(K / 8) * Npad;
  for (long idx = blockIdx.x * (long)blockDim.x + threadIdx.x; idx < total; idx += (long)gridDim.x * blockDim.x) {
    const int n = (int)(idx % Npad);
    const int ko = (int)(idx / Npad);
    float v[8];
#pragma unroll
    for (int e = 0; e < 8; ++e) v[e] = n < N ? w[(long)n * K + ko * 8 + e] : 0.f;
    uint4 ph, pm, pl;
    split8_bf16x3(v, ph, pm, pl);
    const int g = ko >> 1, kh = ko & 1;
    uint4* base = out + ((long)g * 6) * Npad + n;
    base[(long)(0 * 2 + kh) * Npad] = ph;
    base[(long)(1 * 2 + kh) * Npad] = pm;
    base[(long)(2 * 2 + kh) * Npad] = pl;
  }
}

__global__ __launch_bounds__(256) void gemm_x6_split_kernel(const float* __restrict__ a, long lda, uint4* __restrict__ out, int M, int K, long Mpad) {
  __shared__ float tile[64][65];
  const int r0 = blockIdx.x * 64, k0 = blockIdx.y * 64;
  const int t = threadIdx.x;
#pragma unroll
  for (int i = 0; i < 4; ++i) {
    const int r = (t >> 4) + 16 * i, kq = t & 15;
    float4 v = make_float4(0.f, 0.f, 0.f, 0.f);
    if (r0 + r < M) v = *reinterpret_cast<const float4*>(a + (long)(r0 + r) * lda + k0 + 4 * kq);
    tile[r][4 * kq + 0] = v.x; tile[r][4 * kq + 1] = v.y; tile[r][4 * kq + 2] = v.z; tile[r][4 * kq + 3] = v.w;
  }
  __syncthreads();
#pragma unroll
  for (int u = 0; u < 2; ++u) {
    const int r = t & 63, o = (t >> 6) + 4 * u;
    float v[8];
#pragma unroll
    for (int e = 0; e < 8; ++e) v[e] = tile[r][o * 8 + e];
    uint4 ph, pm, pl;
    split8_bf16x3(v, ph, pm, pl);
    const int ko = (k0 >> 3) + o, g = ko >> 1, kh = ko & 1;
    uint4* base = out + ((long)g * 6) * Mpad + r0 + r;
    base[(long)(0 * 2 + kh) * Mpad] = ph;
    base[(long)(1 * 2 + kh) * Mpad] = pm;
    base[(long)(2 * 2 + kh) * Mpad] = pl;
  }
}

enum { EPI_PLAIN = 0, EPI_SWIGLU = 1, EPI_GATE = 2 };

struct GemmX6Params {
  const uint4* Ap;
  long Mpad;
  long arow0;
  const uint4* Wp;
  const float* bias;
  float* C;
  long ldc;
  int M, N, Npad, K, accumulate, m_tiles, n_tiles;
  int tap_steps;
  int epi;
  const float* gate;
  long gate_ld, rows_per_batch;
  int nbatch;
  const int* gate_seq_off;
  unsigned long long* dbg;
};


template <int MT, int NT, int NST, int EPI = EPI_PLAIN, int ACC = 0, int SEQ = 0, int DBG = 0, int PIN = 0>
__global__ __launch_bounds__(256, (NST * (MT + NT) * 6 * 64 * 16 <= 80 * 1024) ? 2 : 1) void gemm_x6_kernel(GemmX6Params p) {
  constexpr int BM = 64 * MT, BN = 64 * NT;
  constexpr int A_UNITS = 6 * BM, W_UNITS = 6 * BN, STAGE = A_UNITS + W_UNITS;
  constexpr int NDMA = (6 * (MT + NT)) / 4;
  constexpr int NA = (6 * MT) / 4, NW = NDMA - NA;
  static_assert((6 * MT) % 4 == 0 && (6 * NT) % 4 == 0, "the A pieces and the W pieces are each dealt evenly to the 4 waves");
  static_assert(EPI == EPI_PLAIN || (ACC == 0 && NT == 2), "pair epilogues: the wave's two 32-column blocks are the two halves");
  static_assert(EPI == EPI_GATE || SEQ == 0, "the sequence table belongs to the gate epilogue");
  constexpr int D = NST - 1;
  extern __shared__ uint4 smem[];

  const int nwg = p.m_tiles * p.n_tiles;
  const int bid = blockIdx.x;
  const int xcd = bid & 7, idx = bid >> 3;
  const int qd = nwg >> 3, rm = nwg & 7;
  const int lin = (xcd < rm ? xcd * (qd + 1) : rm * (qd + 1) + (xcd - rm) * qd) + idx;
  const int m_tile = lin / p.n_tiles, n_tile = lin - m_tile * p.n_tiles;
  const int m0 = m_tile * BM, n0 = n_tile * BN;

  const int tid = threadIdx.x, lane = tid & 63;
  const int wave = __builtin_amdgcn_readfirstlane(tid >> 6);
  const int wm = wave >> 1, wn = wave & 1;
  const int l31 = lane & 31, lh = lane >> 5;

  gx_f32x16 acc[MT][NT];
#pragma unroll
  for (int i = 0; i < MT; ++i)
#pragma unroll
    for (int j = 0; j < NT; ++j)
#pragma unroll
      for (int r = 0; r < 16; ++r) acc[i][j][r] = 0.f;

  const uint4* asrc = p.Ap + p.arow0 + m0 + lane;
  const uint4* wsrc = p.Wp + n0 + lane;
  long a_off[NA], w_off[NW];
  int a_lds[NA], w_lds[NW];
#pragma unroll
  for (int q = 0; q < NA; ++q) {
    const int e = q * 4 + wave, run = e / MT, piece = e % MT;
    a_off[q] = run * p.Mpad + piece * 64;
    a_lds[q] = run * BM + piece * 64;
  }
#pragma unroll
  for (int q = 0; q < NW; ++q) {
    const int e = q * 4 + wave, run = e / NT, piece = e % NT;
    w_off[q] = (long)run * p.Npad + piece * 64;
    w_lds[q] = A_UNITS + run * BN + piece * 64;
  }
  const long a_step = 6 * p.Mpad, w_step = 6L * p.Npad;
  const long a_wrap = 1 - p.tap_steps * a_step;
  long a_run = 0, w_run = 0;
  int a_group = 0;
  auto issue_next = [&](uint4* st) {
#pragma unroll
    for (int q = 0; q < NA; ++q)
      __builtin_amdgcn_global_load_lds((const __attribute__((address_space(1))) void*)(asrc + (a_off[q] + a_run)),
                                       (__attribute__((address_space(3))) void*)(st + a_lds[q]), 16, 0, 0);
#pragma unroll
    for (int q = 0; q < NW; ++q)
      __builtin_amdgcn_global_load_lds((const __attribute__((address_space(1))) void*)(wsrc + (w_off[q] + w_run)),
                                       (__attribute__((address_space(3))) void*)(st + w_lds[q]), 16, 0, 0);
    a_run += a_step;
    w_run += w_step;
    if (++a_group == p.tap_steps) {
      a_group = 0;
      a_run += a_wrap;
    }
  };

  const int steps = p.K >> 4;
  auto wg_stamp = [&](int k) {
    if constexpr (DBG == 3) {
      if (tid == 0) p.dbg[128 + (long)blockIdx.x * 4 + k] = __builtin_amdgcn_s_memrealtime();
    }
  };
  auto wait_younger = [&](int y) {
    if (y >= 2) asm volatile("s_waitcnt vmcnt(%0)" ::"n"(2 * NDMA) : "memory");
    else if (y == 1) asm volatile("s_waitcnt vmcnt(%0)" ::"n"(NDMA) : "memory");
    else asm volatile("s_waitcnt vmcnt(0)" ::: "memory");
  };
  static_assert(D >= 1 && D <= 3, "1..3 steps of copies in flight behind the one waited for");
  wg_stamp(0);
  for (int t = 0; t < D && t < steps; ++t) issue_next(smem + t * STAGE);
  wait_younger(min(D, steps) - 1);
  __builtin_amdgcn_s_barrier();
  asm volatile("" ::: "memory");
  wg_stamp(1);

  const unsigned base_addr = (unsigned)(uintptr_t)(const __attribute__((address_space(3))) void*)smem;
  int st_cur = 0, st_nxt = D % NST;
  for (int s = 0; s < steps; ++s) {
    auto stamp = [&](int k) {
      if constexpr (DBG == 3) {
        if (blockIdx.x == 0 && tid == 0 && s < 16) {
          p.dbg[s * 8 + k] = __builtin_amdgcn_s_memtime();
          if (k == 0) p.dbg[s * 8 + 7] = __builtin_amdgcn_s_memrealtime();
        }
      }
    };
    stamp(0);
    if (DBG != 1 && s + D < steps) issue_next(smem + st_nxt * STAGE);
    stamp(1);
    const unsigned cur_addr = base_addr + (unsigned)(st_cur * STAGE * 16);
    if constexpr (DBG != 2) {
      gx_u32x4 af[3][MT], bf[3][NT];
      const unsigned aaddr = cur_addr + (unsigned)((lh * BM + wm * (32 * MT) + l31) * 16);
      const unsigned waddr = cur_addr + (unsigned)((A_UNITS + lh * BN + wn * (32 * NT) + l31) * 16);
      if constexpr (MT == 4 && NT == 2) {
        asm volatile(
            "ds_read_b128 %0, %18 offset:%20\n ds_read_b128 %1, %18 offset:%21\n ds_read_b128 %2, %18 offset:%22\n ds_read_b128 %3, %18 offset:%23\n"
            "ds_read_b128 %4, %18 offset:%24\n ds_read_b128 %5, %18 offset:%25\n ds_read_b128 %6, %18 offset:%26\n ds_read_b128 %7, %18 offset:%27\n"
            "ds_read_b128 %8, %18 offset:%28\n ds_read_b128 %9, %18 offset:%29\n ds_read_b128 %10, %18 offset:%30\n ds_read_b128 %11, %18 offset:%31\n"
            "ds_read_b128 %12, %19 offset:%32\n ds_read_b128 %13, %19 offset:%33\n ds_read_b128 %14, %19 offset:%34\n ds_read_b128 %15, %19 offset:%35\n"
            "ds_read_b128 %16, %19 offset:%36\n ds_read_b128 %17, %19 offset:%37\n s_waitcnt lgkmcnt(0)"
            : "=&v"(af[0][0]), "=&v"(af[0][1]), "=&v"(af[0][2]), "=&v"(af[0][3]), "=&v"(af[1][0]), "=&v"(af[1][1]), "=&v"(af[1][2]), "=&v"(af[1][3]),
              "=&v"(af[2][0]), "=&v"(af[2][1]), "=&v"(af[2][2]), "=&v"(af[2][3]), "=&v"(bf[0][0]), "=&v"(bf[0][1]), "=&v"(bf[1][0]), "=&v"(bf[1][1]),
              "=&v"(bf[2][0]), "=&v"(bf[2][1])
            : "v"(aaddr), "v"(waddr), "n"((0 * 2 * BM + 0) * 16), "n"((0 * 2 * BM + 32) * 16), "n"((0 * 2 * BM + 64) * 16), "n"((0 * 2 * BM + 96) * 16),
              "n"((1 * 2 * BM + 0) * 16), "n"((1 * 2 * BM + 32) * 16), "n"((1 * 2 * BM + 64) * 16), "n"((1 * 2 * BM + 96) * 16), "n"((2 * 2 * BM + 0) * 16),
              "n"((2 * 2 * BM + 32) * 16), "n"((2 * 2 * BM + 64) * 16), "n"((2 * 2 * BM + 96) * 16), "n"((0 * 2 * BN + 0) * 16), "n"((0 * 2 * BN + 32) * 16),
              "n"((1 * 2 * BN + 0) * 16), "n"((1 * 2 * BN + 32) * 16), "n"((2 * 2 * BN + 0) * 16), "n"((2 * 2 * BN + 32) * 16)
            : "memory");
      } else {
        static_assert(MT == 2 && NT == 2, "fragment block written for 256 x 128 and 128 x 128 tiles");
        asm volatile(
            "ds_read_b128 %0, %12 offset:%14\n ds_read_b128 %1, %12 offset:%15\n ds_read_b128 %2, %12 offset:%16\n ds_read_b128 %3, %12 offset:%17\n"
            "ds_read_b128 %4, %12 offset:%18\n ds_read_b128 %5, %12 offset:%19\n ds_read_b128 %6, %13 offset:%20\n ds_read_b128 %7, %13 offset:%21\n"
            "ds_read_b128 %8, %13 offset:%22\n ds_read_b128 %9, %13 offset:%23\n ds_read_b128 %10, %13 offset:%24\n ds_read_b128 %11, %13 offset:%25\n"
            "s_waitcnt lgkmcnt(0)"
            : "=&v"(af[0][0]), "=&v"(af[0][1]), "=&v"(af[1][0]), "=&v"(af[1][1]), "=&v"(af[2][0]), "=&v"(af[2][1]), "=&v"(bf[0][0]), "=&v"(bf[0][1]),
              "=&v"(bf[1][0]), "=&v"(bf[1][1]), "=&v"(bf[2][0]), "=&v"(bf[2][1])
            : "v"(aaddr), "v"(waddr), "n"((0 * 2 * BM + 0) * 16), "n"((0 * 2 * BM + 32) * 16), "n"((1 * 2 * BM + 0) * 16), "n"((1 * 2 * BM + 32) * 16),
              "n"((2 * 2 * BM + 0) * 16), "n"((2 * 2 * BM + 32) * 16), "n"((0 * 2 * BN + 0) * 16), "n"((0 * 2 * BN + 32) * 16), "n"((1 * 2 * BN + 0) * 16),
              "n"((1 * 2 * BN + 32) * 16), "n"((2 * 2 * BN + 0) * 16), "n"((2 * 2 * BN + 32) * 16)
            : "memory");
      }
      stamp(2);
#pragma unroll
      for (int i = 0; i < MT; ++i)
#pragma unroll
        for (int j = 0; j < NT; ++j) {
          const gx_bf16x8 ah = __builtin_bit_cast(gx_bf16x8, af[0][i]), am = __builtin_bit_cast(gx_bf16x8, af[1][i]), al = __builtin_bit_cast(gx_bf16x8, af[2][i]);
          const gx_bf16x8 bh = __builtin_bit_cast(gx_bf16x8, bf[0][j]), bm = __builtin_bit_cast(gx_bf16x8, bf[1][j]), bl = __builtin_bit_cast(gx_bf16x8, bf[2][j]);
          acc[i][j] = __builtin_amdgcn_mfma_f32_32x32x16_bf16(al, bh, acc[i][j], 0, 0, 0);
          acc[i][j] = __builtin_amdgcn_mfma_f32_32x32x16_bf16(ah, bl, acc[i][j], 0, 0, 0);
          acc[i][j] = __builtin_amdgcn_mfma_f32_32x32x16_bf16(am, bm, acc[i][j], 0, 0, 0);
          acc[i][j] = __builtin_amdgcn_mfma_f32_32x32x16_bf16(am, bh, acc[i][j], 0, 0, 0);
          acc[i][j] = __builtin_amdgcn_mfma_f32_32x32x16_bf16(ah, bm, acc[i][j], 0, 0, 0);
          acc[i][j] = __builtin_amdgcn_mfma_f32_32x32x16_bf16(ah, bh, acc[i][j], 0, 0, 0);
        }
      if constexpr (DBG == 3) asm volatile("" ::"v"(acc[0][0][0]), "v"(acc[MT - 1][NT - 1][15]));
      if constexpr (PIN != 0) __builtin_amdgcn_sched_barrier(0);
    }
    stamp(3);
    wait_younger(DBG == 1 ? 0 : max(0, min(D - 1, steps - s - 2)));
    stamp(4);
    __builtin_amdgcn_s_barrier();
    asm volatile("" ::: "memory");
    stamp(5);
    st_cur = st_cur + 1 == NST ? 0 : st_cur + 1;
    st_nxt = st_nxt + 1 == NST ? 0 : st_nxt + 1;
  }

  wg_stamp(2);
  if constexpr (EPI != EPI_PLAIN) {
    const int oc = (n0 + wn * 64) / 2 + l31;
    const int nh = p.N >> 1;
    if (oc < nh) {
      const unsigned rpb = (unsigned)min(p.rows_per_batch, (long)0x7fffffff);
      const float ba = p.bias != nullptr ? p.bias[n0 + wn * 64 + l31] : 0.f, bb = p.bias != nullptr ? p.bias[n0 + wn * 64 + 32 + l31] : 0.f;
#pragma unroll
      for (int i = 0; i < MT; ++i) {
        const int rbase = m0 + wm * (32 * MT) + i * 32 + 4 * lh;
#pragma unroll
        for (int r = 0; r < 16; ++r) {
          const int row = rbase + (r & 3) + 8 * (r >> 2);
          if (row < p.M) {
            float a = acc[i][0][r] + ba, b = acc[i][1][r] + bb, v;
            if constexpr (EPI == EPI_SWIGLU) {
              v = a / (1.0f + expf(-a)) * b;
            } else {
              long gb;
              if constexpr (SEQ != 0) gb = (long)seq_of_row(p.gate_seq_off, p.nbatch, row);
              else gb = min((long)((unsigned)row / rpb), (long)p.nbatch - 1);
              const float* g = p.gate + gb * p.gate_ld;
              a += g[oc];
              b += g[nh + oc];
              v = tanhf(a) * (1.0f / (1.0f + expf(-b)));
            }
            p.C[(long)row * p.ldc + oc] = v;
          }
        }
      }
    }
  } else
#pragma unroll
  for (int j = 0; j < NT; ++j) {
    const int col = n0 + wn * (32 * NT) + j * 32 + l31;
    const bool col_ok = col < p.N;
    const float bv = (p.bias != nullptr && col_ok) ? p.bias[col] : 0.f;
#pragma unroll
    for (int i = 0; i < MT; ++i) {
      const int rbase = m0 + wm * (32 * MT) + i * 32 + 4 * lh;
#pragma unroll
      for (int r = 0; r < 16; ++r) {
        const int row = rbase + (r & 3) + 8 * (r >> 2);
        if (col_ok && row < p.M) {
          float* c = p.C + (long)row * p.ldc + col;
          float v = acc[i][j][r] + bv;
          if constexpr (ACC != 0) v += *c;
          *c = v;
        }
      }
    }
  }
  if constexpr (DBG == 3) {
    asm volatile("s_waitcnt vmcnt(0)" ::: "memory");
    wg_stamp(3);
  }
}

template <int MT, int NT, int NST, int EPI = EPI_PLAIN, int ACC = 0, int SEQ = 0, int DBG = 0, int PIN = 0>
static int launch_gemm_x6(GemmX6Params p, hipStream_t st) {
  constexpr int BM = 64 * MT, BN = 64 * NT;
  constexpr size_t smem = (size_t)NST * (6 * BM + 6 * BN) * 16;
  static_assert(smem <= 160 * 1024, "LDS stages of this tile shape");
  p.m_tiles = ceil_div(p.M, BM);
  p.n_tiles = ceil_div(p.N, BN);
  IX_ARG((long)p.n_tiles * BN <= p.Npad, "gemm_x6: packed weights padded to %d features, the %d-wide tile needs %d", p.Npad, BN, p.n_tiles * BN);
  const int taps = (p.K >> 4) / p.tap_steps;
  IX_ARG(p.arow0 + (long)p.m_tiles * BM + taps - 1 <= p.Mpad, "gemm_x6: activation planes hold %ld rows, the %d-row tiles reach row %ld", p.Mpad, BM,
         p.arow0 + (long)p.m_tiles * BM + taps - 1);
  auto kern = gemm_x6_kernel<MT, NT, NST, EPI, ACC, SEQ, DBG, PIN>;
  static bool done = false;
  if (!done) {
    IX_HIP(hipFuncSetAttribute((const void*)kern, hipFuncAttributeMaxDynamicSharedMemorySize, (int)smem));
    done = true;
  }
  hipLaunchKernelGGL(kern, dim3(p.m_tiles * p.n_tiles), dim3(256), smem, st, p);
  IX_HIP(hipGetLastError());
  return IXTTS_OK;
}

template <int MT, int NT, int NST, bool PAIR>
static int launch_gemm_x6_epilogue(const GemmX6Params& p, hipStream_t st) {
  if (p.epi == EPI_PLAIN) return p.accumulate ? launch_gemm_x6<MT, NT, NST, EPI_PLAIN, 1>(p, st) : launch_gemm_x6<MT, NT, NST, EPI_PLAIN, 0>(p, st);
  if constexpr (PAIR) {
    if (p.epi == EPI_SWIGLU) return launch_gemm_x6<MT, NT, NST, EPI_SWIGLU>(p, st);
    if (p.epi == EPI_GATE)
      return p.gate_seq_off ? launch_gemm_x6<MT, NT, NST, EPI_GATE, 0, 1>(p, st) : launch_gemm_x6<MT, NT, NST, EPI_GATE, 0, 0>(p, st);
  }
  set_error("gemm_x6: epilogue %d on a tile shape built without it", p.epi);
  return IXTTS_ERR_ARG;
}

}

using namespace ixtts;

extern "C" size_t ixtts_gemm_x6_packed_bytes(int N, int K) {
  if (N <= 0 || K <= 0 || K % 64) return 0;
  const size_t Npad = (size_t)(N + 255) / 256 * 256;
  return (size_t)(K / 16) * 6 * Npad * 16;
}

extern "C" int ixtts_gemm_x6_pack(const float* w_dev, void* packed_dev, int N, int K, void* stream) {
  IX_ARG(w_dev && packed_dev && N > 0 && K > 0 && K % 64 == 0, "gemm_x6_pack: bad argument (K must be a multiple of 64)");
  const int Npad = (N + 255) / 256 * 256;
  const long total = (long)(K / 8) * Npad;
  hipLaunchKernelGGL(gemm_x6_pack_kernel, dim3((unsigned)std::min<long>((total + 255) / 256, 4096)), dim3(256), 0, (hipStream_t)stream, w_dev,
                     reinterpret_cast<uint4*>(packed_dev), N, K, Npad);
  IX_HIP(hipGetLastError());
  return IXTTS_OK;
}

extern "C" long ixtts_gemm_x6_rows_padded(long rows) { return rows <= 0 ? 0 : (rows + 255) / 256 * 256 + 256; }

extern "C" int ixtts_gemm_x6_split(const float* a_dev, long lda, void* planes_dev, long rows, int K, void* stream) {
  IX_ARG(a_dev && planes_dev && rows > 0 && K > 0 && K % 64 == 0, "gemm_x6_split: bad argument (K must be a multiple of 64)");
  IX_ARG(lda >= K && lda % 4 == 0 && (reinterpret_cast<uintptr_t>(a_dev) & 15) == 0, "gemm_x6_split: rows must be 16-byte aligned (lda %ld)", lda);
  const long Mpad = ixtts_gemm_x6_rows_padded(rows);
  hipLaunchKernelGGL(gemm_x6_split_kernel, dim3((unsigned)(Mpad / 64), K / 64), dim3(256), 0, (hipStream_t)stream, a_dev, lda,
                     reinterpret_cast<uint4*>(planes_dev), (int)rows, K, Mpad);
  IX_HIP(hipGetLastError());
  return IXTTS_OK;
}

static int run_gemm_x6(GemmX6Params p, int tile, hipStream_t st) {
  if (tile == 0) {
    const long t42 = (long)ceil_div(p.M, 256) * ceil_div(p.N, 128);
    tile = t42 >= 140 ? 2 : 3;
  }
  switch (tile) {
    case 2: return launch_gemm_x6_epilogue<4, 2, 2, true>(p, st);
    case 3: return launch_gemm_x6_epilogue<2, 2, 3, true>(p, st);
    case 4: return launch_gemm_x6_epilogue<4, 2, 4, false>(p, st);
    case 5: return launch_gemm_x6_epilogue<2, 2, 4, false>(p, st);
  }
  if (tile >= 12 && (p.epi != EPI_PLAIN || p.accumulate)) {
    set_error("gemm_x6: the developer variants (tile %d) are built with the plain, overwriting epilogue only", tile);
    return IXTTS_ERR_ARG;
  }
  switch (tile) {
    case 12: return launch_gemm_x6<4, 2, 2, EPI_PLAIN, 0, 0, 1>(p, st);
    case 22: return launch_gemm_x6<4, 2, 2, EPI_PLAIN, 0, 0, 2>(p, st);
    case 32: return launch_gemm_x6<4, 2, 2, EPI_PLAIN, 0, 0, 3>(p, st);
    case 33: return launch_gemm_x6<2, 2, 3, EPI_PLAIN, 0, 0, 3>(p, st);
    case 42: return launch_gemm_x6<4, 2, 2, EPI_PLAIN, 0, 0, 0, 1>(p, st);
    case 43: return launch_gemm_x6<2, 2, 3, EPI_PLAIN, 0, 0, 0, 1>(p, st);
  }
  set_error("gemm_x6: tile %d (0 auto; 2 / 3: 256x128 / 128x128, two workgroups per CU; 4 / 5: the same, one per CU with a 4-stage ring)", tile);
  return IXTTS_ERR_ARG;
}

extern "C" int ixtts_gemm_x6_f32(const void* a_planes_dev, long rows_total, long row0, const void* packed_dev, const float* bias_dev, float* c_dev,
                                 long ldc, int M, int N, int K, int accumulate, int tile, void* stream) {
  IX_ARG(a_planes_dev && packed_dev && c_dev && M > 0 && N > 0 && K > 0 && K % 64 == 0, "gemm_x6: bad argument (K must be a multiple of 64: the split pass works on 64-wide k blocks)");
  IX_ARG(ldc >= N && row0 >= 0 && row0 + M <= rows_total, "gemm_x6: rows [%ld, %ld) of %ld, ldc %ld", row0, row0 + M, rows_total, ldc);
  GemmX6Params p;
  p.Ap = reinterpret_cast<const uint4*>(a_planes_dev); p.Mpad = ixtts_gemm_x6_rows_padded(rows_total); p.arow0 = row0;
  p.Wp = reinterpret_cast<const uint4*>(packed_dev); p.bias = bias_dev; p.C = c_dev; p.ldc = ldc;
  p.M = M; p.N = N; p.Npad = (N + 255) / 256 * 256; p.K = K; p.accumulate = accumulate ? 1 : 0; p.m_tiles = p.n_tiles = 0;
  p.tap_steps = K >> 4; p.epi = EPI_PLAIN; p.gate = nullptr; p.gate_ld = 0; p.rows_per_batch = 1; p.nbatch = 1; p.gate_seq_off = nullptr;
  p.dbg = (tile == 32 || tile == 33) ? reinterpret_cast<unsigned long long*>(const_cast<float*>(bias_dev)) : nullptr;
  if (p.dbg) p.bias = nullptr;
  return run_gemm_x6(p, tile, (hipStream_t)stream);
}

extern "C" int ixtts_gemm_x6_pair_f32(const void* a_planes_dev, long rows_total, long row0, int taps, const void* packed_dev, const float* bias_dev,
                                      const float* gate_dev, long gate_ld, long rows_per_batch, int nbatch, float* c_dev, long ldc, int M, int N, int K,
                                      int epilogue, int tile, void* stream) {
  IX_ARG(a_planes_dev && packed_dev && c_dev && M > 0 && N > 0 && taps > 0 && K > 0, "gemm_x6_pair: bad argument");
  IX_ARG(K % taps == 0 && (K / taps) % 64 == 0 && N % 64 == 0, "gemm_x6_pair: K %d = %d taps of a multiple of 64, N %d a multiple of 64", K, taps, N);
  IX_ARG(epilogue == EPI_SWIGLU || (epilogue == EPI_GATE && gate_dev && rows_per_batch > 0 && nbatch > 0 && gate_ld >= N / 2),
         "gemm_x6_pair: epilogue %d (1 swiglu; 2 gate, with gate biases)", epilogue);
  IX_ARG(ldc >= N / 2 && row0 >= 0 && row0 + M + taps - 1 <= rows_total, "gemm_x6_pair: rows [%ld, %ld) + %d taps of %ld, ldc %ld", row0, row0 + M, taps,
         rows_total, ldc);
  IX_ARG(tile == 0 || tile == 2 || tile == 3, "gemm_x6_pair: tile %d (0 auto, 2, 3)", tile);
  GemmX6Params p;
  p.Ap = reinterpret_cast<const uint4*>(a_planes_dev); p.Mpad = ixtts_gemm_x6_rows_padded(rows_total); p.arow0 = row0;
  p.Wp = reinterpret_cast<const uint4*>(packed_dev); p.bias = bias_dev; p.C = c_dev; p.ldc = ldc;
  p.M = M; p.N = N; p.Npad = (N + 255) / 256 * 256; p.K = K; p.accumulate = 0; p.m_tiles = p.n_tiles = 0;
  p.tap_steps = (K / taps) >> 4; p.epi = epilogue; p.gate = gate_dev; p.gate_ld = gate_ld; p.rows_per_batch = rows_per_batch; p.nbatch = nbatch;
  p.gate_seq_off = nullptr;
  p.dbg = nullptr;
  return run_gemm_x6(p, tile, (hipStream_t)stream);
}

extern "C" int ixtts_gemm_x6_pair_gate_varlen_f32(const void* a_planes_dev, long rows_total, long row0, int taps, const void* packed_dev, const float* bias_dev,
                                                  const float* gate_dev, long gate_ld, const int* seq_off_dev, int nseq, float* c_dev, long ldc, int M, int N,
                                                  int K, int tile, void* stream) {
  IX_ARG(seq_off_dev && nseq > 0, "gemm_x6_pair_gate_varlen: null offsets table or nseq %d", nseq);
  IX_ARG(a_planes_dev && packed_dev && c_dev && gate_dev && M > 0 && N > 0 && taps > 0 && K > 0 && gate_ld >= N / 2, "gemm_x6_pair_gate_varlen: bad argument");
  IX_ARG(K % taps == 0 && (K / taps) % 64 == 0 && N % 64 == 0, "gemm_x6_pair_gate_varlen: K %d = %d taps of a multiple of 64, N %d a multiple of 64", K, taps, N);
  IX_ARG(ldc >= N / 2 && row0 >= 0 && row0 + M + taps - 1 <= rows_total, "gemm_x6_pair_gate_varlen: rows [%ld, %ld) + %d taps of %ld, ldc %ld", row0, row0 + M,
         taps, rows_total, ldc);
  IX_ARG(tile == 0 || tile == 2 || tile == 3, "gemm_x6_pair_gate_varlen: tile %d (0 auto, 2, 3)", tile);
  GemmX6Params p;
  p.Ap = reinterpret_cast<const uint4*>(a_planes_dev); p.Mpad = ixtts_gemm_x6_rows_padded(rows_total); p.arow0 = row0;
  p.Wp = reinterpret_cast<const uint4*>(packed_dev); p.bias = bias_dev; p.C = c_dev; p.ldc = ldc;
  p.M = M; p.N = N; p.Npad = (N + 255) / 256 * 256; p.K = K; p.accumulate = 0; p.m_tiles = p.n_tiles = 0;
  p.tap_steps = (K / taps) >> 4; p.epi = EPI_GATE; p.gate = gate_dev; p.gate_ld = gate_ld; p.rows_per_batch = 1; p.nbatch = nseq;
  p.gate_seq_off = seq_off_dev;
  p.dbg = nullptr;
  return run_gemm_x6(p, tile, (hipStream_t)stream);
}
```

### voice-tts_amd/gemm.py

```python
import ctypes as C

import torch

from . import _lib


class PackedLinear:

    __slots__ = ("N", "K", "packed", "bias")

    def __init__(self, weight, bias=None):
        assert weight.is_cuda and weight.dim() == 2 and weight.shape[1] % 64 == 0, tuple(weight.shape)
        w = weight.detach().to(torch.float32).contiguous()
        self.N, self.K = int(w.shape[0]), int(w.shape[1])
        nbytes = _lib.lib().ixtts_gemm_x6_packed_bytes(self.N, self.K)
        self.packed = torch.empty(nbytes, dtype=torch.uint8, device=w.device)
        with torch.cuda.device(w.device):
            _lib.check(_lib.lib().ixtts_gemm_x6_pack(w.data_ptr(), self.packed.data_ptr(), self.N, self.K, _lib.current_stream_ptr()), "ixtts_gemm_x6_pack")
            torch.cuda.current_stream().synchronize()
        self.bias = None if bias is None else bias.detach().to(w.device, torch.float32).contiguous()


class Planes:

    __slots__ = ("buf", "rows", "K")

    def __init__(self, buf, rows, K):
        self.buf, self.rows, self.K = buf, rows, K


_POOL = {}


def usable(x, K):
    return x.is_cuda and x.dtype == torch.float32 and K % 64 == 0 and x.shape[-1] == K and x.stride(-1) == 1 and x.data_ptr() % 16 == 0 and \
        (x.dim() == 1 or (x.stride(-2) % 4 == 0 and x.stride(-2) >= K))


def split(x, slot=0):
    K = int(x.shape[-1])
    if x.dim() != 2:
        x = x.reshape(-1, K) if x.is_contiguous() else x.contiguous().reshape(-1, K)
    rows, lda = int(x.shape[0]), int(x.stride(0))
    L = _lib.lib()
    nbytes = (K // 16) * 6 * int(L.ixtts_gemm_x6_rows_padded(rows)) * 16
    key = (x.device, nbytes, slot)
    buf = _POOL.get(key)
    if buf is None:
        buf = _POOL[key] = torch.empty(nbytes, dtype=torch.uint8, device=x.device)
    with torch.cuda.device(x.device):
        _lib.check(L.ixtts_gemm_x6_split(x.data_ptr(), lda, buf.data_ptr(), rows, K, _lib.current_stream_ptr()), "ixtts_gemm_x6_split")
    return Planes(buf, rows, K)


def linear(x, pl, out=None, accumulate=False, bias=True, tile=0, row0=0, rows=None, lead=None):
    K, N = pl.K, pl.N
    if not isinstance(x, Planes):
        lead = tuple(x.shape[:-1]) if lead is None else lead
        x = split(x)
    assert x.K == K, (x.K, K)
    M = (x.rows - row0) if rows is None else int(rows)
    if out is None:
        assert not accumulate
        out = torch.empty(*(lead if lead is not None else (M,)), N, dtype=torch.float32, device=pl.packed.device)
    assert out.shape[-1] == N and out.stride(-1) == 1 and out.numel() >= M * N
    ldc = int(out.stride(-2)) if out.dim() >= 2 else N
    b = pl.bias if (bias and pl.bias is not None) else None
    with torch.cuda.device(pl.packed.device):
        rc = _lib.lib().ixtts_gemm_x6_f32(x.buf.data_ptr(), x.rows, int(row0), pl.packed.data_ptr(), b.data_ptr() if b is not None else None, out.data_ptr(), ldc,
                                          M, N, K, 1 if accumulate else 0, int(tile), _lib.current_stream_ptr())
    _lib.check(rc, "ixtts_gemm_x6_f32")
    return out


SWIGLU, GATE = 1, 2


def interleave_halves(a, b):
    F = a.shape[0]
    assert b.shape == a.shape and F % 32 == 0, (tuple(a.shape), tuple(b.shape))
    return torch.stack([a.reshape(F // 32, 32, *a.shape[1:]), b.reshape(F // 32, 32, *b.shape[1:])], 1).reshape(2 * F, *a.shape[1:]).contiguous()


def pair_linear(x, pl, epilogue, taps=1, out=None, gate=None, gate_off=0, rows_per_batch=1, row0=0, rows=None, tile=0, seq_off=None):
    if not isinstance(x, Planes):
        x = split(x)
    assert pl.K == taps * x.K and pl.N % 64 == 0, (pl.K, taps, x.K, pl.N)
    M = (x.rows - row0 - (taps - 1)) if rows is None else int(rows)
    if out is None:
        out = torch.empty(M, pl.N // 2, dtype=torch.float32, device=pl.packed.device)
    assert out.shape[-1] == pl.N // 2 and out.stride(-1) == 1 and out.numel() >= M * (pl.N // 2)
    ldc = int(out.stride(-2)) if out.dim() >= 2 else pl.N // 2
    gp, gld, nb = None, 0, 1
    if epilogue == GATE:
        assert gate.is_contiguous() and gate.dim() == 2 and gate_off + pl.N <= gate.shape[1]
        gp, gld, nb = gate.data_ptr() + 4 * int(gate_off), int(gate.shape[1]), int(gate.shape[0])
    b = pl.bias
    if seq_off is not None:
        assert epilogue == GATE and seq_off.tab.is_cuda and gate.shape[0] >= seq_off.n
        with torch.cuda.device(pl.packed.device):
            rc = _lib.lib().ixtts_gemm_x6_pair_gate_varlen_f32(x.buf.data_ptr(), x.rows, int(row0), int(taps), pl.packed.data_ptr(),
                                                               b.data_ptr() if b is not None else None, gp, gld, seq_off.tab.data_ptr(), int(seq_off.n),
                                                               out.data_ptr(), ldc, M, pl.N, pl.K, int(tile), _lib.current_stream_ptr())
        _lib.check(rc, "ixtts_gemm_x6_pair_gate_varlen_f32")
        return out
    with torch.cuda.device(pl.packed.device):
        rc = _lib.lib().ixtts_gemm_x6_pair_f32(x.buf.data_ptr(), x.rows, int(row0), int(taps), pl.packed.data_ptr(), b.data_ptr() if b is not None else None,
                                               gp, gld, int(rows_per_batch), nb, out.data_ptr(), ldc, M, pl.N, pl.K, int(epilogue), int(tile),
                                               _lib.current_stream_ptr())
    _lib.check(rc, "ixtts_gemm_x6_pair_f32")
    return out
```

### voice-tts_amd/s2mel.py

```python
import math
import os

import torch
import torch.nn.functional as F

from . import gemm as G
from .convs import conv1d

from .weights import fold_weight_norm

S2MEL_CFG = dict(
    hidden_dim=512, num_heads=8, depth=13, in_channels=80, content_dim=512, style_dim=192,
    wavenet_hidden=512, wavenet_layers=8, wavenet_kernel=5, wavenet_dilation_rate=1,
    lr_channels=512, lr_in_channels=1024, lr_n_blocks=4, gpt_dim=1280, codebook_dim=8, codebook_size=8192, semantic_dim=1024,
)


def tiny_s2mel_cfg(**kw):
    c = dict(S2MEL_CFG)
    c.update(hidden_dim=64, num_heads=2, depth=5, content_dim=32, style_dim=12, wavenet_hidden=64, wavenet_layers=3,
             lr_channels=32, lr_in_channels=40, lr_n_blocks=2, gpt_dim=128, codebook_size=8194, semantic_dim=40)
    c.update(kw)
    return c


def _ffn_dim(dim):
    n_hidden = int(2 * (4 * dim) / 3)
    return n_hidden if n_hidden % 256 == 0 else n_hidden + 256 - (n_hidden % 256)


def s2mel_shapes(cfg=S2MEL_CFG):
    H, Hw, C = cfg["hidden_dim"], cfg["wavenet_hidden"], cfg["in_channels"]
    assert H == Hw, "FinalLayer's adaLN takes the DiT timestep embedding: wavenet.hidden_dim must equal DiT.hidden_dim"
    out = [("gpt_layer.0.weight", (256, cfg["gpt_dim"])), ("gpt_layer.0.bias", (256,)), ("gpt_layer.1.weight", (128, 256)),
           ("gpt_layer.1.bias", (128,)), ("gpt_layer.2.weight", (cfg["semantic_dim"], 128)), ("gpt_layer.2.bias", (cfg["semantic_dim"],)),
           ("quantizer.codebook.weight", (cfg["codebook_size"], cfg["codebook_dim"])),
           ("quantizer.out_project.weight", (cfg["semantic_dim"], cfg["codebook_dim"], 1)), ("quantizer.out_project.bias", (cfg["semantic_dim"],))]
    lr = cfg["lr_channels"]
    out += [("length_regulator.content_in_proj.weight", (lr, cfg["lr_in_channels"])), ("length_regulator.content_in_proj.bias", (lr,))]
    for i in range(cfg["lr_n_blocks"]):
        out += [(f"length_regulator.model.{3 * i}.weight", (lr, lr, 3)), (f"length_regulator.model.{3 * i}.bias", (lr,)),
                (f"length_regulator.model.{3 * i + 1}.weight", (lr,)), (f"length_regulator.model.{3 * i + 1}.bias", (lr,))]
    n = 3 * cfg["lr_n_blocks"]
    out += [(f"length_regulator.model.{n}.weight", (lr, lr, 1)), (f"length_regulator.model.{n}.bias", (lr,))]
    e = "cfm.estimator."
    out += [(e + "t_embedder.mlp.0.weight", (H, 256)), (e + "t_embedder.mlp.0.bias", (H,)), (e + "t_embedder.mlp.2.weight", (H, H)), (e + "t_embedder.mlp.2.bias", (H,)),
            (e + "t_embedder2.mlp.0.weight", (Hw, 256)), (e + "t_embedder2.mlp.0.bias", (Hw,)), (e + "t_embedder2.mlp.2.weight", (Hw, Hw)), (e + "t_embedder2.mlp.2.bias", (Hw,)),
            (e + "cond_projection.weight", (H, cfg["content_dim"])), (e + "cond_projection.bias", (H,)),
            (e + "cond_x_merge_linear.weight", (H, H + 2 * C + cfg["style_dim"])), (e + "cond_x_merge_linear.bias", (H,)),
            (e + "skip_linear.weight", (H, H + C)), (e + "skip_linear.bias", (H,)),
            (e + "conv1.weight", (Hw, H)), (e + "conv1.bias", (Hw,)), (e + "conv2.weight", (C, Hw, 1)), (e + "conv2.bias", (C,)),
            (e + "res_projection.weight", (Hw, H)), (e + "res_projection.bias", (Hw,)),
            (e + "final_layer.linear.weight", (Hw, Hw)), (e + "final_layer.linear.bias", (Hw,)),
            (e + "final_layer.adaLN_modulation.1.weight", (2 * Hw, Hw)), (e + "final_layer.adaLN_modulation.1.bias", (2 * Hw,))]
    t = e + "transformer."
    inter = _ffn_dim(H)
    for i in range(cfg["depth"]):
        p = t + f"layers.{i}."
        out += [(p + "attention.wqkv.weight", (3 * H, H)), (p + "attention.wo.weight", (H, H)),
                (p + "feed_forward.w1.weight", (inter, H)), (p + "feed_forward.w3.weight", (inter, H)), (p + "feed_forward.w2.weight", (H, inter)),
                (p + "ffn_norm.project_layer.weight", (2 * H, H)), (p + "ffn_norm.project_layer.bias", (2 * H,)), (p + "ffn_norm.norm.weight", (H,)),
                (p + "attention_norm.project_layer.weight", (2 * H, H)), (p + "attention_norm.project_layer.bias", (2 * H,)), (p + "attention_norm.norm.weight", (H,)),
                (p + "skip_in_linear.weight", (H, 2 * H)), (p + "skip_in_linear.bias", (H,))]
    out += [(t + "norm.project_layer.weight", (2 * H, H)), (t + "norm.project_layer.bias", (2 * H,)), (t + "norm.norm.weight", (H,))]
    w = e + "wavenet."
    nl, k = cfg["wavenet_layers"], cfg["wavenet_kernel"]
    out += [(w + "cond_layer.conv.conv.weight", (2 * Hw * nl, Hw, 1)), (w + "cond_layer.conv.conv.bias", (2 * Hw * nl,))]
    for i in range(nl):
        rs = 2 * Hw if i < nl - 1 else Hw
        out += [(w + f"in_layers.{i}.conv.conv.weight", (2 * Hw, Hw, k)), (w + f"in_layers.{i}.conv.conv.bias", (2 * Hw,)),
                (w + f"res_skip_layers.{i}.conv.conv.weight", (rs, Hw, 1)), (w + f"res_skip_layers.{i}.conv.conv.bias", (rs,))]
    return out


def make_s2mel_weights(cfg=S2MEL_CFG, seed=1234):
    g = torch.Generator().manual_seed(seed)
    W = {}
    for name, shape in s2mel_shapes(cfg):
        if name.endswith("norm.weight") or (".model." in name and len(shape) == 1 and name.endswith(".weight")):
            W[name] = 1.0 + 0.1 * torch.randn(*shape, generator=g)
        elif name.endswith(".bias"):
            W[name] = 0.02 * torch.randn(*shape, generator=g)
        elif name == "quantizer.codebook.weight":
            W[name] = torch.randn(*shape, generator=g)
        else:
            fan = 1
            for d in shape[1:]:
                fan *= d
            W[name] = torch.randn(*shape, generator=g) / math.sqrt(fan)
    return W


def _pad_reflect(x, left, right):
    L = x.shape[-1]
    extra = 0
    if L <= max(left, right):
        extra = max(left, right) - L + 1
        x = F.pad(x, (0, extra))
    y = F.pad(x, (left, right), mode="reflect")
    return y[..., : y.shape[-1] - extra]


def attn_full(q, k, v, scale=None):
    import ctypes as C

    from . import _lib

    B, T, Hh, d = q.shape
    assert d == 64 and q.is_cuda and q.dtype == torch.float32 and k.shape == q.shape and v.shape == q.shape
    for t in (q, k, v):
        assert t.stride(3) == 1 and t.stride() == q.stride() and t.stride(1) % 4 == 0 and t.data_ptr() % 16 == 0
    out = torch.empty(B, T, Hh, d, device=q.device, dtype=torch.float32)
    sc = float(scale if scale is not None else 1.0 / math.sqrt(d))
    L = _lib.lib()
    nws = L.ixtts_attn_full_workspace_bytes(B, Hh, T)
    ws = torch.empty(nws, device=q.device, dtype=torch.uint8)
    with torch.cuda.device(q.device):
        rc = L.ixtts_attn_full_f32(q.data_ptr(), k.data_ptr(), v.data_ptr(), out.data_ptr(), B, Hh, T, d, q.stride(0), q.stride(1),
                                   q.stride(2), out.stride(0), out.stride(1), out.stride(2), C.c_float(sc), ws.data_ptr(), nws,
                                   _lib.current_stream_ptr())
    _lib.check(rc, "ixtts_attn_full_f32")
    return out


def _lin(x, W, name):
    return F.linear(x, W[name + ".weight"], W.get(name + ".bias"))


def _hip_call(name, *args):
    from . import _lib

    _lib.check(getattr(_lib.lib(), name)(*args, _lib.current_stream_ptr()), name)


def adaln_rmsnorm(x, wb, g, eps=1e-5):
    B, T, H = x.shape
    if x.is_cuda:
        import ctypes as C

        x, wb = x.contiguous(), wb.contiguous()
        out = torch.empty_like(x)
        with torch.cuda.device(x.device):
            _hip_call("ixtts_adaln_rmsnorm_f32", x.data_ptr(), wb.data_ptr(), g.data_ptr(), out.data_ptr(), B, T, H, C.c_float(eps))
        return out
    w, b = wb[:, None, :H], wb[:, None, H:]
    return torch.addcmul(b, w, F.rms_norm(x, (H,), g, eps))


def ln_modulate(x, ss, eps=1e-6):
    B, T, H = x.shape
    if x.is_cuda:
        import ctypes as C

        x, ss = x.contiguous(), ss.contiguous()
        out = torch.empty_like(x)
        with torch.cuda.device(x.device):
            _hip_call("ixtts_ln_modulate_f32", x.data_ptr(), ss.data_ptr(), out.data_ptr(), B, T, H, C.c_float(eps))
        return out
    return F.layer_norm(x, (H,), None, None, eps) * (1 + ss[:, None, H:]) + ss[:, None, :H]


def swiglu(u):
    Fd = u.shape[-1] // 2
    if u.is_cuda:
        u = u.contiguous()
        out = torch.empty(*u.shape[:-1], Fd, device=u.device, dtype=u.dtype)
        with torch.cuda.device(u.device):
            _hip_call("ixtts_swiglu_f32", u.data_ptr(), out.data_ptr(), u.numel() // (2 * Fd), Fd)
        return out
    return F.silu(u[..., :Fd]) * u[..., Fd:]


def wn_gate(a, g, off, C_):
    B, _, T = a.shape
    if a.is_cuda:
        a, g = a.contiguous(), g.contiguous()
        out = torch.empty(B, C_, T, device=a.device, dtype=a.dtype)
        with torch.cuda.device(a.device):
            _hip_call("ixtts_wn_gate_f32", a.data_ptr(), g.data_ptr(), out.data_ptr(), B, C_, T, g.shape[1], off)
        return out
    x = a + g[:, off:off + 2 * C_, None]
    return torch.tanh(x[:, :C_]) * torch.sigmoid(x[:, C_:])


def wn_gate_rows(a, g, off, C_, rows_per_batch):
    rows, B = a.shape[0], g.shape[0]
    if a.is_cuda:
        a, g = a.contiguous(), g.contiguous()
        out = torch.empty(rows, C_, device=a.device, dtype=a.dtype)
        with torch.cuda.device(a.device):
            _hip_call("ixtts_wn_gate_rows_f32", a.data_ptr(), g.data_ptr(), out.data_ptr(), rows, C_, rows_per_batch, B, g.shape[1], off)
        return out
    b = (torch.arange(rows, device=a.device) // rows_per_batch).clamp(max=B - 1)
    x = a + g[b, off:off + 2 * C_]
    return torch.tanh(x[:, :C_]) * torch.sigmoid(x[:, C_:])


def reflect_halo_rows(p, T, left, right):
    B, _, C_ = p.shape
    if p.is_cuda:
        assert p.is_contiguous()
        with torch.cuda.device(p.device):
            _hip_call("ixtts_reflect_halo_rows_f32", p.data_ptr(), B, T, C_, left, right)
        return p
    if left:
        p[:, :left] = p[:, left + 1:2 * left + 1].flip(1)
    if right:
        p[:, left + T:] = p[:, left + T - 1 - right:left + T - 1].flip(1)
    return p


class RowPack:

    def __init__(self, lens, device):
        self.lens = [int(t) for t in lens]
        assert self.lens and min(self.lens) >= 1, self.lens
        self.n = len(self.lens)
        self.off = [0]
        for t in self.lens:
            self.off.append(self.off[-1] + t)
        self.rows = self.off[-1]
        self.device = torch.device(device)
        tiles = [0]
        for t in self.lens:
            tiles.append(tiles[-1] + (t + 63) // 64)
        self.tiles = tiles[-1]
        work = [(s, q) for s, t in enumerate(self.lens) for q in range((t + 127) // 128)]
        self.n_work = len(work)
        host = torch.tensor(self.off + tiles + [v for w in work for v in w], dtype=torch.int32)
        self.tab = host.to(self.device)
        if self.device.type != "cuda":
            self.seq = torch.repeat_interleave(torch.arange(self.n), torch.tensor(self.lens))
            self.pos = torch.arange(self.rows) - torch.tensor(self.off[:-1])[self.seq]

    def span(self, s):
        return self.off[s], self.off[s + 1]


def adaln_rmsnorm_packed(x, wb, g, pk, eps=1e-5):
    rows, H = x.shape
    if x.is_cuda:
        import ctypes as C

        x, wb = x.contiguous(), wb.contiguous()
        out = torch.empty_like(x)
        with torch.cuda.device(x.device):
            _hip_call("ixtts_adaln_rmsnorm_varlen_f32", x.data_ptr(), wb.data_ptr(), g.data_ptr(), out.data_ptr(), pk.tab.data_ptr(), pk.n, rows, H, C.c_float(eps))
        return out
    wbr = wb[pk.seq]
    return torch.addcmul(wbr[:, H:], wbr[:, :H], F.rms_norm(x, (H,), g, eps))


def ln_modulate_packed(x, ss, pk, eps=1e-6):
    rows, H = x.shape
    if x.is_cuda:
        import ctypes as C

        x, ss = x.contiguous(), ss.contiguous()
        out = torch.empty_like(x)
        with torch.cuda.device(x.device):
            _hip_call("ixtts_ln_modulate_varlen_f32", x.data_ptr(), ss.data_ptr(), out.data_ptr(), pk.tab.data_ptr(), pk.n, rows, H, C.c_float(eps))
        return out
    ssr = ss[pk.seq]
    return F.layer_norm(x, (H,), None, None, eps) * (1 + ssr[:, H:]) + ssr[:, :H]


def rope_qk_packed(qkv, fc, pk, head_dim):
    rows, H3 = qkv.shape
    H = H3 // 3
    if qkv.is_cuda:
        assert qkv.is_contiguous() and fc.shape[0] >= max(pk.lens)
        with torch.cuda.device(qkv.device):
            _hip_call("ixtts_rope_qk_varlen_f32", qkv.data_ptr(), torch.view_as_real(fc).data_ptr(), pk.tab.data_ptr(), pk.n, rows, H, head_dim)
        return qkv
    f = fc[pk.pos][:, None, :]
    out = qkv.clone()
    for j in range(2):
        xc = torch.view_as_complex(qkv[:, j * H:(j + 1) * H].reshape(rows, H // head_dim, head_dim // 2, 2).contiguous())
        out[:, j * H:(j + 1) * H] = torch.view_as_real(xc * f).reshape(rows, H)
    return out


def attn_full_packed(q, k, v, pk, scale=None):
    import ctypes as C

    from . import _lib

    rows, Hh, d = q.shape
    assert d == 64 and q.is_cuda and q.dtype == torch.float32 and k.shape == q.shape and v.shape == q.shape and rows == pk.rows
    for t in (q, k, v):
        assert t.stride(2) == 1 and t.stride() == q.stride() and t.stride(0) % 4 == 0 and t.data_ptr() % 16 == 0
    out = torch.empty(rows, Hh, d, device=q.device, dtype=torch.float32)
    sc = float(scale if scale is not None else 1.0 / math.sqrt(d))
    L = _lib.lib()
    nws = L.ixtts_attn_full_varlen_workspace_bytes(pk.n, Hh, pk.tiles)
    ws = torch.empty(nws, device=q.device, dtype=torch.uint8)
    with torch.cuda.device(q.device):
        rc = L.ixtts_attn_full_varlen_f32(q.data_ptr(), k.data_ptr(), v.data_ptr(), out.data_ptr(), pk.tab.data_ptr(), pk.n, pk.tiles, pk.n_work, Hh, d,
                                          q.stride(0), q.stride(1), out.stride(0), out.stride(1), C.c_float(sc), ws.data_ptr(), nws, _lib.current_stream_ptr())
    _lib.check(rc, "ixtts_attn_full_varlen_f32")
    return out


def wn_gate_rows_packed(a, g, off, C_, poff):
    rows = a.shape[0]
    if a.is_cuda:
        a, g = a.contiguous(), g.contiguous()
        out = torch.empty(rows, C_, device=a.device, dtype=a.dtype)
        with torch.cuda.device(a.device):
            _hip_call("ixtts_wn_gate_rows_varlen_f32", a.data_ptr(), g.data_ptr(), out.data_ptr(), rows, C_, poff.tab.data_ptr(), poff.n, g.shape[1], off)
        return out
    b = torch.cat([poff.seq, poff.seq.new_full((max(0, rows - poff.rows),), poff.n - 1)])[:rows]
    x = a + g[b, off:off + 2 * C_]
    return torch.tanh(x[:, :C_]) * torch.sigmoid(x[:, C_:])


def _reflect_src(T, left, right):
    idx = _pad_reflect(torch.arange(1, T + 1, dtype=torch.float64)[None, None], left, right)[0, 0].long() - 1
    dst = list(range(left)) + list(range(left + T, left + T + right))
    return dst, [int(idx[i]) + left if int(idx[i]) >= 0 else -1 for i in dst]


def reflect_halo_rows_packed(p, poff, left, right):
    if p.is_cuda:
        assert p.is_contiguous() and min(poff.lens) - left - right > max(left, right)
        with torch.cuda.device(p.device):
            _hip_call("ixtts_reflect_halo_rows_varlen_f32", p.data_ptr(), poff.tab.data_ptr(), poff.n, p.shape[1], left, right)
        return p
    if not hasattr(poff, "halo"):
        dst, src, zero = [], [], []
        for s, L in enumerate(poff.lens):
            o = poff.off[s]
            for d_, s_ in zip(*_reflect_src(L - left - right, left, right)):
                (dst.append(o + d_), src.append(o + s_)) if s_ >= 0 else zero.append(o + d_)
        poff.halo = (torch.tensor(dst, dtype=torch.long), torch.tensor(src, dtype=torch.long), torch.tensor(zero, dtype=torch.long))
    dst, src, zero = poff.halo
    p[dst] = p[src]
    if zero.numel():
        p[zero] = 0
    return p


S2MEL_BATCH_FRAMES = 16384

TUNED_GEMMS = os.path.join(os.path.dirname(os.path.abspath(__file__)), "tunable", "gfx950_s2mel.csv")


def use_tuned_gemms(path=TUNED_GEMMS):
    if not torch.cuda.is_available():
        return False
    import torch.cuda.tunable as tn

    tn.enable(True)
    tn.tuning_enable(os.environ.get("IXTTS_TUNE") == "1")
    try:
        import tempfile

        tn.set_filename(os.path.join(tempfile.gettempdir(), "ixtts_tunableop_online.csv"))
    except Exception:
        pass
    try:
        return bool(os.path.isfile(path) and tn.read_file(path))
    except Exception:
        return False


_TUNED_T0, _TUNED_TH0 = 2322, 1909
_tuned_lengths = set()


def extend_tuned_gemms(T, Th, path=TUNED_GEMMS):
    if (T, Th) in _tuned_lengths or (T, Th) == (_TUNED_T0, _TUNED_TH0):
        return False
    _tuned_lengths.add((T, Th))
    import tempfile

    import torch.cuda.tunable as tn

    sub = {str(2 * _TUNED_T0): str(2 * T), str(_TUNED_T0): str(T), str(_TUNED_TH0): str(Th), str(2 * _TUNED_TH0): str(2 * Th),
           str(2 * _TUNED_TH0 + 4): str(2 * Th + 4)}
    head, rows = [], []
    for line in open(path).read().splitlines():
        f = line.split(",")
        if f[0] == "Validator":
            head.append(line)
        elif len(f) >= 4 and f[2] != "Default" and f[0].endswith("_TN"):
            toks = f[1].split("_")
            if any(t in sub for t in toks):
                rows.append(",".join([f[0], "_".join(sub.get(t, t) for t in toks)] + f[2:]))
    if not rows:
        return False
    with tempfile.NamedTemporaryFile("w", suffix=".csv", delete=False) as fh:
        fh.write("\n".join(head + rows) + "\n")
    try:
        return bool(tn.read_file(fh.name))
    except Exception:
        return False
    finally:
        os.unlink(fh.name)


class S2Mel:
    def __init__(self, W, cfg=S2MEL_CFG, device="cpu"):
        self.cfg = dict(cfg)
        self.device = torch.device(device)
        self.tuned_gemms = False
        if self.device.type == "cuda" and os.environ.get("IXTTS_NO_TUNED_GEMMS") != "1":
            self.tuned_gemms = use_tuned_gemms()
        W = fold_weight_norm(dict(W))
        self.W = {k: v.to(self.device, torch.float32) for k, v in W.items()}
        H = cfg["hidden_dim"]
        self.head_dim = H // cfg["num_heads"]
        half = 128
        self.t_freqs = torch.exp(-math.log(10000.0) * torch.arange(half, dtype=torch.float32) / half).to(self.device)
        self._rope = None
        W, C_, L = self.W, cfg["in_channels"], cfg["depth"]
        t = "cfm.estimator.transformer."
        self.w13 = [torch.cat([W[t + f"layers.{i}.feed_forward.w1.weight"], W[t + f"layers.{i}.feed_forward.w3.weight"]], 0).contiguous() for i in range(L)]
        self.skip_w = {i: (W[t + f"layers.{i}.skip_in_linear.weight"][:, :H].contiguous(), W[t + f"layers.{i}.skip_in_linear.weight"][:, H:].contiguous())
                       for i in range(L // 2 + 1, L)}
        names = [t + f"layers.{i}.{n}" for i in range(L) for n in ("attention_norm", "ffn_norm")] + [t + "norm"]
        self.proj_w = torch.cat([W[n + ".project_layer.weight"] for n in names], 0).contiguous()
        self.proj_b = torch.cat([W[n + ".project_layer.bias"] for n in names], 0).contiguous()
        mw = W["cfm.estimator.cond_x_merge_linear.weight"]
        self.merge_x, self.merge_rest = mw[:, :C_].contiguous(), mw[:, C_:].contiguous()
        wn = "cfm.estimator.wavenet."
        self.wn_taps = [[W[wn + f"in_layers.{i}.conv.conv.weight"][:, :, j].contiguous() for j in range(cfg["wavenet_kernel"])]
                        for i in range(cfg["wavenet_layers"])]
        nl, Hw = cfg["wavenet_layers"], cfg["wavenet_hidden"]
        self.wn_r1, self.wn_r2, self.wn_bin = [], [], []
        carry = torch.zeros(Hw, device=self.device)
        self.wn_out_bias = torch.zeros(Hw, device=self.device)
        for i in range(nl):
            rw, rb = W[wn + f"res_skip_layers.{i}.conv.conv.weight"][:, :, 0], W[wn + f"res_skip_layers.{i}.conv.conv.bias"]
            self.wn_bin.append(W[wn + f"in_layers.{i}.conv.conv.bias"] + sum(self.wn_taps[i]) @ carry)
            if i < nl - 1:
                self.wn_r1.append(rw[:Hw].contiguous())
                self.wn_r2.append(rw[Hw:].contiguous())
                carry = carry + rb[:Hw]
                self.wn_out_bias = self.wn_out_bias + rb[Hw:]
            else:
                self.wn_r1.append(None)
                self.wn_r2.append(rw.contiguous())
                self.wn_out_bias = self.wn_out_bias + rb
        sw = W["cfm.estimator.skip_linear.weight"]
        self.skipl_res, self.skipl_x = sw[:, :H].contiguous(), sw[:, H:].contiguous()
        self.x6_w13, self.x6_wn = None, None
        if self.device.type == "cuda" and H % 64 == 0:
            inter = self.w13[0].shape[0] // 2
            self.x6_w13 = [G.PackedLinear(G.interleave_halves(w[:inter], w[inter:])) for w in self.w13]
            self.x6_wn = [G.PackedLinear(G.interleave_halves(torch.cat(tp, 1)[:Hw], torch.cat(tp, 1)[Hw:]), G.interleave_halves(b[:Hw], b[Hw:]))
                          for tp, b in zip(self.wn_taps, self.wn_bin)]

    def _x6(self, packs):
        return packs is not None and os.environ.get("IXTTS_S2MEL_GEMM", "x6") != "library"

    def gpt_layer(self, latent):
        x = _lin(latent, self.W, "gpt_layer.0")
        x = _lin(x, self.W, "gpt_layer.1")
        return _lin(x, self.W, "gpt_layer.2")

    def vq2emb(self, codes):
        emb = self.W["quantizer.codebook.weight"][codes.long()]
        out = conv1d(emb.transpose(1, 2), self.W["quantizer.out_project.weight"], self.W["quantizer.out_project.bias"])
        return out.transpose(1, 2)

    def length_regulator(self, x, ylens):
        W = self.W
        x = _lin(x, W, "length_regulator.content_in_proj")
        T = int(ylens.max())
        x = F.interpolate(x.transpose(1, 2).contiguous(), size=T, mode="nearest")
        for i in range(self.cfg["lr_n_blocks"]):
            x = conv1d(x, W[f"length_regulator.model.{3 * i}.weight"], W[f"length_regulator.model.{3 * i}.bias"], padding=1)
            x = F.group_norm(x, 1, W[f"length_regulator.model.{3 * i + 1}.weight"], W[f"length_regulator.model.{3 * i + 1}.bias"], 1e-5)
            x = F.mish(x)
        n = 3 * self.cfg["lr_n_blocks"]
        x = conv1d(x, W[f"length_regulator.model.{n}.weight"], W[f"length_regulator.model.{n}.bias"])
        mask = (torch.arange(T, device=x.device).unsqueeze(0) < ylens.unsqueeze(1)).unsqueeze(-1)
        return x.transpose(1, 2) * mask

    def _t_embed(self, t, prefix):
        args = 1000.0 * t[:, None].float() * self.t_freqs[None]
        emb = torch.cat([torch.cos(args), torch.sin(args)], dim=-1)
        h = F.silu(_lin(emb, self.W, prefix + ".mlp.0"))
        return _lin(h, self.W, prefix + ".mlp.2")

    def _rope_cache(self, T):
        if self._rope is None or self._rope.shape[0] < T:
            n = self.head_dim
            freqs = 1.0 / (10000.0 ** (torch.arange(0, n, 2)[: n // 2].float() / n))
            ang = torch.outer(torch.arange(max(T, 64)).float(), freqs)
            self._rope = torch.polar(torch.ones_like(ang), ang).to(self.device)
        return self._rope[:T]

    @staticmethod
    def _rotary(x, fc):
        xc = torch.view_as_complex(x.reshape(*x.shape[:-1], -1, 2))
        return torch.view_as_real(xc * fc.view(1, fc.shape[0], 1, fc.shape[1])).flatten(3)

    def _attention(self, qkv, B, T, mask):
        H, nh, hd = self.cfg["hidden_dim"], self.cfg["num_heads"], self.head_dim
        fc = self._rope_cache(T)
        if mask is None and hd == 64 and qkv.is_cuda:
            with torch.cuda.device(qkv.device):
                _hip_call("ixtts_rope_qk_f32", qkv.data_ptr(), torch.view_as_real(fc).data_ptr(), B, T, H, hd)
            v4 = qkv.view(B, T, 3, nh, hd)
            return attn_full(v4[:, :, 0], v4[:, :, 1], v4[:, :, 2]).reshape(B * T, H)
        q, k, v = qkv.view(B, T, 3 * H).split([H, H, H], dim=-1)
        q = self._rotary(q.reshape(B, T, nh, hd), fc)
        k = self._rotary(k.reshape(B, T, nh, hd), fc)
        v = v.reshape(B, T, nh, hd)
        y = F.scaled_dot_product_attention(q.transpose(1, 2), k.transpose(1, 2), v.transpose(1, 2), attn_mask=mask, dropout_p=0.0)
        return y.transpose(1, 2).reshape(B * T, H)

    def _transformer(self, x, c, mask):
        W, cfg = self.W, self.cfg
        B, T, H = x.shape
        L = cfg["depth"]
        wb_all = F.linear(c, self.proj_w, self.proj_b).view(B, 2 * L + 1, 2 * H).transpose(0, 1).contiguous()
        x = x.reshape(B * T, H)
        x6 = x.is_cuda and self._x6(self.x6_w13)
        skips = []
        for i in range(L):
            p = f"cfm.estimator.transformer.layers.{i}."
            if i > L // 2:
                wa, wb_ = self.skip_w[i]
                x = F.linear(skips.pop(), wb_, W[p + "skip_in_linear.bias"]).addmm_(x, wa.t())
            a = adaln_rmsnorm(x.view(B, T, H), wb_all[2 * i], W[p + "attention_norm.norm.weight"])
            y = self._attention(F.linear(a.view(B * T, H), W[p + "attention.wqkv.weight"]), B, T, mask)
            h = torch.addmm(x, y, W[p + "attention.wo.weight"].t()) if 0 < i <= L // 2 else x.addmm_(y, W[p + "attention.wo.weight"].t())
            f = adaln_rmsnorm(h.view(B, T, H), wb_all[2 * i + 1], W[p + "ffn_norm.norm.weight"]).view(B * T, H)
            u = G.pair_linear(f, self.x6_w13[i], G.SWIGLU) if x6 else swiglu(F.linear(f, self.w13[i]))
            x = h.addmm_(u, W[p + "feed_forward.w2.weight"].t())
            if i < L // 2:
                skips.append(x)
        return adaln_rmsnorm(x.view(B, T, H), wb_all[2 * L], W["cfm.estimator.transformer.norm.norm.weight"])

    def _wavenet(self, x, x_mask, g, full):
        W, cfg = self.W, self.cfg
        Hw, nl, k = cfg["wavenet_hidden"], cfg["wavenet_layers"], cfg["wavenet_kernel"]
        p = "cfm.estimator.wavenet."
        g = F.linear(g, W[p + "cond_layer.conv.conv.weight"][:, :, 0], W[p + "cond_layer.conv.conv.bias"])
        out = None
        for i in range(nl):
            d = cfg["wavenet_dilation_rate"] ** i
            tot = (k - 1) * d
            right = tot // 2
            xin = _pad_reflect(x, tot - right, right)
            if x.is_cuda:
                wk, T_ = self.wn_taps[i], x.shape[-1]
                acc = W[p + f"in_layers.{i}.conv.conv.bias"][None, :, None].expand(x.shape[0], -1, T_)
                for j in range(k):
                    wj, xj = wk[j].expand(x.shape[0], -1, -1), xin[:, :, j * d:j * d + T_]
                    acc = torch.baddbmm(acc, wj, xj) if j == 0 else acc.baddbmm_(wj, xj)
                xin = acc
            else:
                xin = conv1d(xin, W[p + f"in_layers.{i}.conv.conv.weight"], W[p + f"in_layers.{i}.conv.conv.bias"], dilation=d)
            acts = wn_gate(xin, g, i * 2 * Hw, Hw)
            rs = conv1d(acts, W[p + f"res_skip_layers.{i}.conv.conv.weight"], W[p + f"res_skip_layers.{i}.conv.conv.bias"])
            if i < nl - 1:
                x = x + rs[:, :Hw]
                if not full:
                    x = x * x_mask
                out = rs[:, Hw:] if out is None else out + rs[:, Hw:]
            else:
                out = rs if out is None else out + rs
        return out if full else out * x_mask

    def _wavenet_gemm(self, x, g):
        W, cfg = self.W, self.cfg
        Hw, nl, k = cfg["wavenet_hidden"], cfg["wavenet_layers"], cfg["wavenet_kernel"]
        B, _, T_ = x.shape
        p = "cfm.estimator.wavenet."
        g = F.linear(g, W[p + "cond_layer.conv.conv.weight"][:, :, 0], W[p + "cond_layer.conv.conv.bias"])
        x = x.contiguous()
        out = None
        for i in range(nl):
            d = cfg["wavenet_dilation_rate"] ** i
            tot = (k - 1) * d
            right = tot // 2
            xin = _pad_reflect(x, tot - right, right)
            acc = self.wn_bin[i][None, :, None].expand(B, -1, T_)
            for j in range(k):
                wj, xj = self.wn_taps[i][j].expand(B, -1, -1), xin[:, :, j * d:j * d + T_]
                acc = torch.baddbmm(acc, wj, xj) if j == 0 else acc.baddbmm_(wj, xj)
            acts = wn_gate(acc, g, i * 2 * Hw, Hw)
            if i < nl - 1:
                x = x.baddbmm_(self.wn_r1[i].expand(B, -1, -1), acts)
            r2 = self.wn_r2[i].expand(B, -1, -1)
            out = torch.bmm(r2, acts) if out is None else out.baddbmm_(r2, acts)
        return out

    def _wavenet_rows(self, h, g):
        W, cfg = self.W, self.cfg
        Hw, nl, k = cfg["wavenet_hidden"], cfg["wavenet_layers"], cfg["wavenet_kernel"]
        assert cfg["wavenet_dilation_rate"] == 1
        B, T_, _ = h.shape
        p = "cfm.estimator.wavenet."
        g = F.linear(g, W[p + "cond_layer.conv.conv.weight"][:, :, 0], W[p + "cond_layer.conv.conv.bias"])
        tot = k - 1
        right = tot // 2
        left = tot - right
        Tp = T_ + tot
        P = torch.empty(B, Tp, Hw, device=h.device, dtype=h.dtype)
        P[:, left:left + T_] = h
        P2 = P.view(B * Tp, Hw)
        M = B * Tp - tot
        centre = P2[left:left + M]
        out = torch.empty(B * Tp, Hw, device=h.device, dtype=h.dtype)
        x6 = self._x6(self.x6_wn)
        for i in range(nl):
            reflect_halo_rows(P, T_, left, right)
            if x6:
                acts = G.pair_linear(G.split(P2), self.x6_wn[i], G.GATE, taps=k, gate=g, gate_off=i * 2 * Hw, rows_per_batch=Tp)
            else:
                acc = torch.addmm(self.wn_bin[i], P2[:M], self.wn_taps[i][0].t())
                for j in range(1, k):
                    acc.addmm_(P2[j:j + M], self.wn_taps[i][j].t())
                acts = wn_gate_rows(acc, g, i * 2 * Hw, Hw, Tp)
            if i < nl - 1:
                centre.addmm_(acts, self.wn_r1[i].t())
            if i == 0:
                torch.mm(acts, self.wn_r2[i].t(), out=out[:M])
            else:
                out[:M].addmm_(acts, self.wn_r2[i].t())
        return out.view(B, Tp, Hw)[:, :T_]

    def dit_prepare(self, prompt_x, x_lens, style, cond):
        W = self.W
        e = "cfm.estimator."
        B, _, T = prompt_x.shape
        cond = _lin(cond, W, e + "cond_projection")
        rest = torch.cat([prompt_x.transpose(1, 2), cond, style[:, None, :].expand(B, T, style.shape[-1])], dim=-1)
        base = F.linear(rest, self.merge_rest, W[e + "cond_x_merge_linear.bias"])
        x_mask = (torch.arange(T, device=prompt_x.device).unsqueeze(0) < x_lens.unsqueeze(1)).unsqueeze(1)
        full = int(x_lens.min()) >= T
        if full:
            attn_mask = None
        else:
            attn_mask = x_mask[:, None, :].expand(x_mask.shape[0], 1, T, T)
            if attn_mask.shape[0] != B:
                attn_mask = attn_mask.expand(B, 1, T, T)
        return dict(B=B, T=T, base=base, x_mask=x_mask.to(base.dtype), attn_mask=attn_mask, full=full)

    def dit_step(self, ctx, x, t, out_from=0):
        W, cfg = self.W, self.cfg
        e = "cfm.estimator."
        B, T, base = ctx["B"], ctx["T"], ctx["base"]
        xt = x.transpose(1, 2)
        t1 = self._t_embed(t, e + "t_embedder")
        x_in = base + F.linear(xt, self.merge_x)
        x_res = self._transformer(x_in, t1, ctx["attn_mask"])
        halo = sum((cfg["wavenet_kernel"] - 1) * cfg["wavenet_dilation_rate"] ** i for i in range(cfg["wavenet_layers"])) // 2 + 1
        lo = max(0, out_from - halo) if (ctx["full"] and out_from > 0) else 0
        if lo > 0:
            x_res, xt = x_res[:, lo:], xt[:, lo:]
        Th = T - lo
        if self.tuned_gemms and os.environ.get("IXTTS_TUNED_ANY_LENGTH", "1") == "1":
            extend_tuned_gemms(T, Th)
        x_res = F.linear(x_res, self.skipl_res, W[e + "skip_linear.bias"]) + F.linear(xt, self.skipl_x)
        h = _lin(x_res, W, e + "conv1")
        t2 = self._t_embed(t, e + "t_embedder2")
        gemm_form = h.is_cuda and ctx["full"] and Th > 2 * cfg["wavenet_kernel"] * cfg["wavenet_dilation_rate"] ** (cfg["wavenet_layers"] - 1)
        if gemm_form and cfg["wavenet_dilation_rate"] == 1:
            h = self._wavenet_rows(h, t2) + F.linear(x_res, W[e + "res_projection.weight"], W[e + "res_projection.bias"] + self.wn_out_bias)
        elif gemm_form:
            h = self._wavenet_gemm(h.transpose(1, 2), t2).transpose(1, 2) + F.linear(x_res, W[e + "res_projection.weight"],
                                                                                     W[e + "res_projection.bias"] + self.wn_out_bias)
        else:
            mask = ctx["x_mask"][:, :, lo:] if lo > 0 else ctx["x_mask"]
            h = self._wavenet(h.transpose(1, 2), mask, t2, ctx["full"]).transpose(1, 2) + _lin(x_res, W, e + "res_projection")
        ss = _lin(F.silu(t1), W, e + "final_layer.adaLN_modulation.1")
        h = ln_modulate(h, ss)
        h = _lin(h, W, e + "final_layer.linear").transpose(1, 2)
        out = conv1d(h, W[e + "conv2.weight"], W[e + "conv2.bias"])
        return out[:, :, out_from - lo:] if out_from > 0 else out

    def dit(self, x, prompt_x, x_lens, t, style, cond):
        return self.dit_step(self.dit_prepare(prompt_x, x_lens, style, cond), x, t)

    @torch.no_grad()
    def cfm_inference(self, mu, x_lens, prompt, style, n_timesteps=25, inference_cfg_rate=0.7, noise=None, temperature=1.0):
        B, T = mu.shape[0], mu.shape[1]
        assert B == 1, "CFM inference is batch-1 (as the reference)"
        z = (torch.randn(B, self.cfg["in_channels"], T, device=mu.device) if noise is None else noise.to(mu.device, torch.float32)) * temperature
        t_span = torch.linspace(0, 1, n_timesteps + 1, device=mu.device)
        x = z.clone()
        Tp = prompt.shape[-1]
        prompt_x = torch.zeros_like(x)
        prompt_x[..., :Tp] = prompt[..., :Tp]
        x[..., :Tp] = 0
        if inference_cfg_rate > 0:
            ctx = self.dit_prepare(torch.cat([prompt_x, torch.zeros_like(prompt_x)], 0), x_lens, torch.cat([style, torch.zeros_like(style)], 0),
                                   torch.cat([mu, torch.zeros_like(mu)], 0))
        else:
            ctx = self.dit_prepare(prompt_x, x_lens, style, mu)
        t = t_span[0]
        skip = Tp if ctx["full"] else 0
        for step in range(1, len(t_span)):
            dt = t_span[step] - t_span[step - 1]
            if inference_cfg_rate > 0:
                d = self.dit_step(ctx, x, torch.stack([t, t]), out_from=skip)
                dphi = (1.0 + inference_cfg_rate) * d[0:1] - inference_cfg_rate * d[1:2]
            else:
                dphi = self.dit_step(ctx, x, t.expand(B), out_from=skip)
            if skip > 0:
                x[:, :, skip:] += dt * dphi
            else:
                x = x + dt * dphi
            t = t + dt
            x[:, :, :Tp] = 0
        return x

    @torch.no_grad()
    def __call__(self, latent, codes, code_lens, prompt_condition, ref_mel, style, n_timesteps=25, inference_cfg_rate=0.7, noise=None):
        lat = self.gpt_layer(latent)
        S = self.vq2emb(codes) + lat
        target = (code_lens * 1.72).long()
        cond = self.length_regulator(S, target)
        cat = torch.cat([prompt_condition, cond], dim=1)
        lens = torch.tensor([cat.shape[1]], device=cat.device, dtype=torch.long)
        mel = self.cfm_inference(cat, lens, ref_mel, style, n_timesteps, inference_cfg_rate, noise)
        return mel[:, :, ref_mel.shape[-1]:]

    def _attention_packed(self, qkv, pk):
        H, nh, hd = self.cfg["hidden_dim"], self.cfg["num_heads"], self.head_dim
        if qkv.is_cuda and hd == 64 and os.environ.get("IXTTS_ATTN_FULL", "x3") != "f32":
            rope_qk_packed(qkv, self._rope_cache(max(pk.lens)), pk, hd)
            v4 = qkv.view(pk.rows, 3, nh, hd)
            return attn_full_packed(v4[:, 0], v4[:, 1], v4[:, 2], pk).view(pk.rows, H)
        out = torch.empty(pk.rows, H, device=qkv.device, dtype=qkv.dtype)
        if qkv.is_cuda:
            for s in range(pk.n):
                a, b = pk.span(s)
                out[a:b] = self._attention(qkv[a:b], 1, b - a, None)
            return out
        qk = rope_qk_packed(qkv, self._rope_cache(max(pk.lens)), pk, hd)
        for s in range(pk.n):
            a, b = pk.span(s)
            q, k, v = (qk[a:b, :H], qk[a:b, H:2 * H], qkv[a:b, 2 * H:])
            y = F.scaled_dot_product_attention(*(z.reshape(1, b - a, nh, hd).transpose(1, 2) for z in (q, k, v)), dropout_p=0.0)
            out[a:b] = y.transpose(1, 2).reshape(b - a, H)
        return out

    def _transformer_packed(self, x, c, pk):
        W, cfg = self.W, self.cfg
        H, L = cfg["hidden_dim"], cfg["depth"]
        wb_all = F.linear(c, self.proj_w, self.proj_b).view(pk.n, 2 * L + 1, 2 * H).transpose(0, 1).contiguous()
        x6 = x.is_cuda and self._x6(self.x6_w13)
        skips = []
        for i in range(L):
            p = f"cfm.estimator.transformer.layers.{i}."
            if i > L // 2:
                wa, wb_ = self.skip_w[i]
                x = F.linear(skips.pop(), wb_, W[p + "skip_in_linear.bias"]).addmm_(x, wa.t())
            a = adaln_rmsnorm_packed(x, wb_all[2 * i], W[p + "attention_norm.norm.weight"], pk)
            y = self._attention_packed(F.linear(a, W[p + "attention.wqkv.weight"]), pk)
            h = torch.addmm(x, y, W[p + "attention.wo.weight"].t()) if 0 < i <= L // 2 else x.addmm_(y, W[p + "attention.wo.weight"].t())
            f = adaln_rmsnorm_packed(h, wb_all[2 * i + 1], W[p + "ffn_norm.norm.weight"], pk)
            u = G.pair_linear(f, self.x6_w13[i], G.SWIGLU) if x6 else swiglu(F.linear(f, self.w13[i]))
            x = h.addmm_(u, W[p + "feed_forward.w2.weight"].t())
            if i < L // 2:
                skips.append(x)
        return adaln_rmsnorm_packed(x, wb_all[2 * L], W["cfm.estimator.transformer.norm.norm.weight"], pk)

    def _wavenet_packed(self, h, g, hp):
        W, cfg = self.W, self.cfg
        Hw, nl, k = cfg["wavenet_hidden"], cfg["wavenet_layers"], cfg["wavenet_kernel"]
        assert cfg["wavenet_dilation_rate"] == 1
        p = "cfm.estimator.wavenet."
        g = F.linear(g, W[p + "cond_layer.conv.conv.weight"][:, :, 0], W[p + "cond_layer.conv.conv.bias"])
        tot = k - 1
        right = tot // 2
        left = tot - right
        pp, interior = hp.padded, hp.interior
        P2 = torch.empty(pp.rows, Hw, device=h.device, dtype=h.dtype)
        P2[interior] = h
        M = pp.rows - tot
        centre = P2[left:left + M]
        out = torch.empty(pp.rows, Hw, device=h.device, dtype=h.dtype)
        x6 = h.is_cuda and self._x6(self.x6_wn)
        for i in range(nl):
            reflect_halo_rows_packed(P2, pp, left, right)
            if x6:
                acts = G.pair_linear(G.split(P2), self.x6_wn[i], G.GATE, taps=k, gate=g, gate_off=i * 2 * Hw, seq_off=pp)
            else:
                acc = torch.addmm(self.wn_bin[i], P2[:M], self.wn_taps[i][0].t())
                for j in range(1, k):
                    acc.addmm_(P2[j:j + M], self.wn_taps[i][j].t())
                acts = wn_gate_rows_packed(acc, g, i * 2 * Hw, Hw, pp)
            if i < nl - 1:
                centre.addmm_(acts, self.wn_r1[i].t())
            if i == 0:
                torch.mm(acts, self.wn_r2[i].t(), out=out[:M])
            else:
                out[:M].addmm_(acts, self.wn_r2[i].t())
        return out[interior - left]

    def _halo(self):
        cfg = self.cfg
        return sum((cfg["wavenet_kernel"] - 1) * cfg["wavenet_dilation_rate"] ** i for i in range(cfg["wavenet_layers"])) // 2 + 1

    def packable(self, T, Tp, device=None):
        dev = self.device if device is None else torch.device(device)
        if dev.type != "cuda":
            return True
        cfg = self.cfg
        Th = T - max(0, Tp - self._halo())
        return cfg["wavenet_dilation_rate"] == 1 and Th > 2 * cfg["wavenet_kernel"]

    def _cfm_packed(self, segs, n_timesteps, inference_cfg_rate):
        W, cfg = self.W, self.cfg
        e = "cfm.estimator."
        dev = segs[0]["mu"].device
        C_, H = cfg["in_channels"], cfg["hidden_dim"]
        n = len(segs)
        lens = [s["mu"].shape[1] for s in segs]
        Tps = [min(s["prompt"].shape[-1], T) for s, T in zip(segs, lens)]
        R = sum(lens)
        cfg_on = inference_cfg_rate > 0
        nb = 2 if cfg_on else 1
        pk = RowPack(lens * nb, dev)
        xo = pk.off[:n + 1]
        x = torch.cat([s["z"][0].t() for s in segs], 0).contiguous()
        keep = torch.cat([torch.arange(xo[i] + Tps[i], xo[i + 1]) for i in range(n)]).to(dev)
        pmask = torch.ones(R, 1, device=dev)
        for i in range(n):
            pmask[xo[i]:xo[i] + Tps[i]] = 0
        x.mul_(pmask)
        prompt_rows = torch.zeros(R, C_, device=dev)
        for i, s in enumerate(segs):
            prompt_rows[xo[i]:xo[i] + Tps[i]] = s["prompt"][0, :, :Tps[i]].t()
        mu = torch.cat([s["mu"][0] for s in segs], 0)
        style = torch.cat([s["style"].expand(T, -1) for s, T in zip(segs, lens)], 0)
        rest = torch.cat([prompt_rows, _lin(mu, W, e + "cond_projection"), style], -1)
        if cfg_on:
            rest = torch.cat([rest, torch.cat([torch.zeros_like(prompt_rows), _lin(torch.zeros_like(mu), W, e + "cond_projection"), torch.zeros_like(style)], -1)], 0)
        base = F.linear(rest, self.merge_rest, W[e + "cond_x_merge_linear.bias"])
        halo, k = self._halo(), cfg["wavenet_kernel"]
        los = [max(0, Tp - halo) for Tp in Tps] * nb
        head_lens = [L - lo for L, lo in zip(pk.lens, los)]
        hp = RowPack(head_lens, dev)
        hp.padded = RowPack([t + k - 1 for t in head_lens], dev)
        right = (k - 1) // 2
        left = k - 1 - right
        hidx = torch.cat([torch.arange(pk.off[s] + los[s], pk.off[s + 1]) for s in range(pk.n)])
        hp.interior = torch.cat([torch.arange(hp.padded.off[s] + left, hp.padded.off[s] + left + head_lens[s]) for s in range(pk.n)]).to(dev)
        hrows = hidx.to(dev)
        hx = (hidx - torch.tensor(pk.off[:-1]).repeat_interleave(torch.tensor(head_lens)) +
              torch.tensor(xo[:-1] * nb).repeat_interleave(torch.tensor(head_lens))).to(dev)
        hsel = torch.cat([torch.arange(hp.off[s] + Tps[s % n] - los[s], hp.off[s + 1]) for s in range(pk.n)]).to(dev)
        nkeep = keep.numel()
        t_span = torch.linspace(0, 1, n_timesteps + 1, device=dev)
        t = t_span[0]
        for step in range(1, len(t_span)):
            dt = t_span[step] - t_span[step - 1]
            tt = t.expand(pk.n)
            t1 = self._t_embed(tt, e + "t_embedder")
            x_in = (base.view(nb, R, H) + F.linear(x, self.merge_x)).view(nb * R, H)
            x_res = self._transformer_packed(x_in, t1, pk)
            x_res = x_res.index_select(0, hrows)
            xt = x.index_select(0, hx)
            x_res = F.linear(x_res, self.skipl_res, W[e + "skip_linear.bias"]) + F.linear(xt, self.skipl_x)
            h = _lin(x_res, W, e + "conv1")
            t2 = self._t_embed(tt, e + "t_embedder2")
            h = self._wavenet_packed(h, t2, hp) + F.linear(x_res, W[e + "res_projection.weight"], W[e + "res_projection.bias"] + self.wn_out_bias)
            ss = _lin(F.silu(t1), W, e + "final_layer.adaLN_modulation.1")
            h = ln_modulate_packed(h, ss, hp)
            h = _lin(h, W, e + "final_layer.linear")
            d = F.linear(h.index_select(0, hsel), W[e + "conv2.weight"][:, :, 0], W[e + "conv2.bias"])
            dphi = (1.0 + inference_cfg_rate) * d[:nkeep] - inference_cfg_rate * d[nkeep:] if cfg_on else d
            x.index_add_(0, keep, dt * dphi)
            t = t + dt
            x.mul_(pmask)
        return [x[xo[i]:xo[i + 1]].t()[None] for i in range(n)]

    @torch.no_grad()
    def solve_many(self, items, n_timesteps=25, inference_cfg_rate=0.7, noises=None):
        segs = []
        for i, (latent, codes, prompt_condition, ref_mel, style) in enumerate(items):
            code_lens = torch.tensor([codes.shape[-1]], device=codes.device)
            S = self.vq2emb(codes) + self.gpt_layer(latent)
            cond = self.length_regulator(S, (code_lens * 1.72).long())
            mu = torch.cat([prompt_condition, cond], dim=1)
            T = mu.shape[1]
            z = torch.randn(1, self.cfg["in_channels"], T, device=mu.device) if noises is None or noises[i] is None else \
                noises[i].to(mu.device, torch.float32)
            segs.append(dict(mu=mu, prompt=ref_mel, style=style, z=z, Tp=ref_mel.shape[-1]))
        xs = [None] * len(segs)
        budget = max(1, int(os.environ.get("IXTTS_S2MEL_BATCH_FRAMES", str(S2MEL_BATCH_FRAMES))))
        order = sorted(range(len(segs)), key=lambda i: segs[i]["mu"].shape[1])
        groups, cur, used = [], [], 0
        for i in order:
            T = segs[i]["mu"].shape[1]
            if not self.packable(T, segs[i]["Tp"], segs[i]["mu"].device):
                groups.append([i])
                continue
            if cur and used + T > budget:
                groups.append(cur)
                cur, used = [], 0
            cur.append(i)
            used += T
        if cur:
            groups.append(cur)
        for grp in groups:
            if len(grp) == 1 and not self.packable(segs[grp[0]]["mu"].shape[1], segs[grp[0]]["Tp"], segs[grp[0]]["mu"].device):
                s = segs[grp[0]]
                lens = torch.tensor([s["mu"].shape[1]], device=s["mu"].device, dtype=torch.long)
                xs[grp[0]] = self.cfm_inference(s["mu"], lens, s["prompt"], s["style"], n_timesteps, inference_cfg_rate, s["z"])
                continue
            for i, x in zip(grp, self._cfm_packed([segs[i] for i in grp], n_timesteps, inference_cfg_rate)):
                xs[i] = x
        return [x[:, :, s["Tp"]:] for x, s in zip(xs, segs)]
```

Before: 41.36.

## Fuse RoPE into attention, adaLN norm into plane split, reflect-pad into split

New measurement: 41.54 (median of 6 runs). No clear change (+0.4%).

```diff
diff --git a/include/ixtts_hip.h b/include/ixtts_hip.h
--- a/include/ixtts_hip.h
+++ b/include/ixtts_hip.h
@@ -26,6 +26,10 @@
                         int head_dim, long stride_b, long stride_t, long stride_h, long ostride_b, long ostride_t,
                         long ostride_h, float scale, void* workspace_dev, size_t workspace_bytes, void* stream);
 
+int ixtts_attn_full_rope_f32(const float* q_dev, const float* k_dev, const float* v_dev, float* out_dev, const float* cos_sin_dev, int B, int H,
+                             int T, int head_dim, long stride_b, long stride_t, long stride_h, long ostride_b, long ostride_t, long ostride_h,
+                             float scale, void* workspace_dev, size_t workspace_bytes, void* stream);
+
 size_t ixtts_attn_full_varlen_workspace_bytes(int nseq, int H, int total_tiles);
 int ixtts_attn_full_varlen_f32(const float* q_dev, const float* k_dev, const float* v_dev, float* out_dev, const int* table_dev, int nseq,
                                int total_tiles, int n_work, int H, int head_dim, long stride_t, long stride_h, long ostride_t, long ostride_h,
@@ -33,6 +37,8 @@
 
 int ixtts_adaln_rmsnorm_f32(const float* x_dev, const float* wb_dev, const float* g_dev, float* out_dev, int B, int T, int H, float eps,
                             void* stream);
+int ixtts_adaln_rmsnorm_planes_f32(const float* x_dev, const float* wb_dev, const float* g_dev, void* planes_dev, int B, int T, int H, float eps,
+                                   int rows_per_block, void* stream);
 int ixtts_ln_modulate_f32(const float* x_dev, const float* shift_scale_dev, float* out_dev, int B, int T, int H, float eps, void* stream);
 int ixtts_rope_qk_f32(float* qkv_dev, const float* cos_sin_dev, int B, int T, int H, int head_dim, void* stream);
 int ixtts_swiglu_f32(const float* u_dev, float* out_dev, long rows, int F, void* stream);
@@ -54,6 +60,7 @@
 int ixtts_gemm_x6_pack(const float* w_dev, void* packed_dev, int N, int K, void* stream);
 long ixtts_gemm_x6_rows_padded(long rows);
 int ixtts_gemm_x6_split(const float* a_dev, long lda, void* planes_dev, long rows, int K, void* stream);
+int ixtts_gemm_x6_split_reflect(const float* p_dev, void* planes_dev, int B, int T, int K, int left, int right, void* stream);
 int ixtts_gemm_x6_f32(const void* a_planes_dev, long rows_total, long row0, const void* packed_dev, const float* bias_dev, float* c_dev, long ldc,
                       int M, int N, int K, int accumulate, int tile, void* stream);
 int ixtts_gemm_x6_pair_f32(const void* a_planes_dev, long rows_total, long row0, int taps, const void* packed_dev, const float* bias_dev,
diff --git a/voice-tts_amd/_lib.py b/voice-tts_amd/_lib.py
--- a/voice-tts_amd/_lib.py
+++ b/voice-tts_amd/_lib.py
@@ -59,10 +59,13 @@
     "ixtts_attn_full_workspace_bytes": (C.c_size_t, [C.c_int, C.c_int, C.c_int]),
     "ixtts_attn_full_f32": (C.c_int, [_P, _P, _P, _P, C.c_int, C.c_int, C.c_int, C.c_int, C.c_long, C.c_long, C.c_long, C.c_long, C.c_long,
                                       C.c_long, C.c_float, _P, C.c_size_t, _P]),
+    "ixtts_attn_full_rope_f32": (C.c_int, [_P, _P, _P, _P, _P, C.c_int, C.c_int, C.c_int, C.c_int, C.c_long, C.c_long, C.c_long, C.c_long, C.c_long,
+                                           C.c_long, C.c_float, _P, C.c_size_t, _P]),
     "ixtts_attn_full_varlen_workspace_bytes": (C.c_size_t, [C.c_int, C.c_int, C.c_int]),
     "ixtts_attn_full_varlen_f32": (C.c_int, [_P, _P, _P, _P, _P, C.c_int, C.c_int, C.c_int, C.c_int, C.c_int, C.c_long, C.c_long, C.c_long, C.c_long,
                                              C.c_float, _P, C.c_size_t, _P]),
     "ixtts_adaln_rmsnorm_f32": (C.c_int, [_P, _P, _P, _P, C.c_int, C.c_int, C.c_int, C.c_float, _P]),
+    "ixtts_adaln_rmsnorm_planes_f32": (C.c_int, [_P, _P, _P, _P, C.c_int, C.c_int, C.c_int, C.c_float, C.c_int, _P]),
     "ixtts_ln_modulate_f32": (C.c_int, [_P, _P, _P, C.c_int, C.c_int, C.c_int, C.c_float, _P]),
     "ixtts_rope_qk_f32": (C.c_int, [_P, _P, C.c_int, C.c_int, C.c_int, C.c_int, _P]),
     "ixtts_swiglu_f32": (C.c_int, [_P, _P, C.c_long, C.c_int, _P]),
@@ -78,6 +81,7 @@
     "ixtts_gemm_x6_pack": (C.c_int, [_P, _P, C.c_int, C.c_int, _P]),
     "ixtts_gemm_x6_rows_padded": (C.c_long, [C.c_long]),
     "ixtts_gemm_x6_split": (C.c_int, [_P, C.c_long, _P, C.c_long, C.c_int, _P]),
+    "ixtts_gemm_x6_split_reflect": (C.c_int, [_P, _P, C.c_int, C.c_int, C.c_int, C.c_int, C.c_int, _P]),
     "ixtts_gemm_x6_f32": (C.c_int, [_P, C.c_long, C.c_long, _P, _P, _P, C.c_long, C.c_int, C.c_int, C.c_int, C.c_int, C.c_int, _P]),
     "ixtts_gemm_x6_pair_f32": (C.c_int, [_P, C.c_long, C.c_long, C.c_int, _P, _P, _P, C.c_long, C.c_long, C.c_int, _P, C.c_long, C.c_int, C.c_int,
                                          C.c_int, C.c_int, C.c_int, _P]),
diff --git a/voice-tts_amd/csrc/attn_full.h b/voice-tts_amd/csrc/attn_full.h
--- a/voice-tts_amd/csrc/attn_full.h
+++ b/voice-tts_amd/csrc/attn_full.h
@@ -23,6 +23,7 @@
   float* ws_ml;
   const int* vl_tab;
   int vl_n, vl_tiles;
+  const float2* rope;
 };
 
 size_t attn_full_x3_plane_bytes(int B, int H, int T);
diff --git a/voice-tts_amd/csrc/attn_full.hip b/voice-tts_amd/csrc/attn_full.hip
--- a/voice-tts_amd/csrc/attn_full.hip
+++ b/voice-tts_amd/csrc/attn_full.hip
@@ -184,9 +184,9 @@
   return attn_partials_bytes(B, H, T) + ixtts::attn_full_x3_plane_bytes(B, H, T);
 }
 
-extern "C" int ixtts_attn_full_f32(const float* q_dev, const float* k_dev, const float* v_dev, float* out_dev, int B, int H, int T,
-                                   int head_dim, long stride_b, long stride_t, long stride_h, long ostride_b, long ostride_t,
-                                   long ostride_h, float scale, void* workspace_dev, size_t workspace_bytes, void* stream) {
+static int attn_full_run(const float* q_dev, const float* k_dev, const float* v_dev, float* out_dev, const float* cos_sin_dev, int B, int H, int T, int head_dim,
+                         long stride_b, long stride_t, long stride_h, long ostride_b, long ostride_t, long ostride_h, float scale, void* workspace_dev,
+                         size_t workspace_bytes, void* stream) {
   using namespace ixtts;
   IX_ARG(q_dev && k_dev && v_dev && out_dev, "attn_full: null pointer");
   IX_ARG(head_dim == AF_D, "attn_full: head_dim %d (only 64 is built)", head_dim);
@@ -199,6 +199,7 @@
   a.B = B; a.H = H; a.T = T; a.scale = scale;
   a.ws_o = a.ws_ml = nullptr;
   a.vl_tab = nullptr; a.vl_n = a.vl_tiles = 0;
+  a.rope = reinterpret_cast<const float2*>(cos_sin_dev);
   hipStream_t st = (hipStream_t)stream;
   const int qblocks = ceil_div(T, AF_WAVES * AF_QW);
   const bool have_ws = workspace_dev && workspace_bytes >= ixtts_attn_full_workspace_bytes(B, H, T);
@@ -206,6 +207,7 @@
   const char* mode = getenv("IXTTS_ATTN_FULL");
   const bool x3 = !(mode && strcmp(mode, "f32") == 0);
   const bool use_x3 = x3 && have_ws;
+  IX_ARG(!a.rope || use_x3, "attn_full_rope: needs the workspace of ixtts_attn_full_workspace_bytes and the default arithmetic (IXTTS_ATTN_FULL=f32 is set: %d)", !x3);
   if (split) {
     a.ws_o = reinterpret_cast<float*>(workspace_dev);
     a.ws_ml = a.ws_o + (size_t)(use_x3 ? AX_KSPLIT : AF_KSPLIT) * B * H * T * AF_D;
@@ -228,6 +230,22 @@
   }
   IX_HIP(hipGetLastError());
   return IXTTS_OK;
+}
+
+extern "C" int ixtts_attn_full_f32(const float* q_dev, const float* k_dev, const float* v_dev, float* out_dev, int B, int H, int T,
+                                   int head_dim, long stride_b, long stride_t, long stride_h, long ostride_b, long ostride_t,
+                                   long ostride_h, float scale, void* workspace_dev, size_t workspace_bytes, void* stream) {
+  return attn_full_run(q_dev, k_dev, v_dev, out_dev, nullptr, B, H, T, head_dim, stride_b, stride_t, stride_h, ostride_b, ostride_t, ostride_h, scale,
+                       workspace_dev, workspace_bytes, stream);
+}
+
+extern "C" int ixtts_attn_full_rope_f32(const float* q_dev, const float* k_dev, const float* v_dev, float* out_dev, const float* cos_sin_dev, int B, int H,
+                                        int T, int head_dim, long stride_b, long stride_t, long stride_h, long ostride_b, long ostride_t, long ostride_h,
+                                        float scale, void* workspace_dev, size_t workspace_bytes, void* stream) {
+  using namespace ixtts;
+  IX_ARG(cos_sin_dev && (reinterpret_cast<uintptr_t>(cos_sin_dev) & 15) == 0, "attn_full_rope: the (cos, sin) table must be set and 16-byte aligned");
+  return attn_full_run(q_dev, k_dev, v_dev, out_dev, cos_sin_dev, B, H, T, head_dim, stride_b, stride_t, stride_h, ostride_b, ostride_t, ostride_h, scale,
+                       workspace_dev, workspace_bytes, stream);
 }
 
 extern "C" size_t ixtts_attn_full_varlen_workspace_bytes(int nseq, int H, int total_tiles) {
@@ -253,5 +271,6 @@
   a.B = 1; a.H = H; a.T = 0; a.scale = scale;
   a.ws_o = a.ws_ml = nullptr;
   a.vl_tab = table_dev; a.vl_n = nseq; a.vl_tiles = total_tiles;
+  a.rope = nullptr;
   return launch_attn_full_x3_varlen(a, workspace_dev, n_work, (hipStream_t)stream);
 }
diff --git a/voice-tts_amd/csrc/attn_full_x3.hip b/voice-tts_amd/csrc/attn_full_x3.hip
--- a/voice-tts_amd/csrc/attn_full_x3.hip
+++ b/voice-tts_amd/csrc/attn_full_x3.hip
@@ -7,6 +7,19 @@
 
 constexpr int AX_TILE_UNITS = 3 * 8 * 64;
 constexpr int AX_WAVES = 4;
+
+__device__ __forceinline__ void rope_pair(float& x, float& y, const float2 f) {
+  const float rx = fmaf(x, f.x, -__fmul_rn(y, f.y)), ry = fmaf(y, f.x, __fmul_rn(x, f.y));
+  x = rx;
+  y = ry;
+}
+__device__ __forceinline__ void rope8(float (&v)[8], const float2* __restrict__ tab, int oct) {
+  const float4 f01 = *reinterpret_cast<const float4*>(tab + 4 * oct), f23 = *reinterpret_cast<const float4*>(tab + 4 * oct + 2);
+  rope_pair(v[0], v[1], make_float2(f01.x, f01.y));
+  rope_pair(v[2], v[3], make_float2(f01.z, f01.w));
+  rope_pair(v[4], v[5], make_float2(f23.x, f23.y));
+  rope_pair(v[6], v[7], make_float2(f23.z, f23.w));
+}
 
 size_t attn_full_x3_plane_bytes(int B, int H, int T) {
   const size_t tiles = (size_t)(T + AF_KT - 1) / AF_KT;
@@ -14,7 +27,7 @@
 }
 
 
-template <bool VL>
+template <bool VL, bool ROPE = false>
 __global__ __launch_bounds__(256) void attn_kv_planes_kernel(AttnFullArgs a, uint4* __restrict__ planes) {
   int tile = blockIdx.x, T = a.T;
   const float *kb, *vb;
@@ -45,8 +58,16 @@
     const float4* src = reinterpret_cast<const float4*>(kb + (long)min(t, T - 1) * a.st + 8 * oct);
     const float4 x0 = src[0], x1 = src[1];
     const bool live = t < T;
-    v[0] = live ? x0.x : 0.f; v[1] = live ? x0.y : 0.f; v[2] = live ? x0.z : 0.f; v[3] = live ? x0.w : 0.f;
-    v[4] = live ? x1.x : 0.f; v[5] = live ? x1.y : 0.f; v[6] = live ? x1.z : 0.f; v[7] = live ? x1.w : 0.f;
+    if constexpr (ROPE) {
+      static_assert(!VL, "RoPE in the split pass: single-sequence entry only");
+      float r[8] = {x0.x, x0.y, x0.z, x0.w, x1.x, x1.y, x1.z, x1.w};
+      rope8(r, a.rope + (long)min(t, T - 1) * (AF_D / 2), oct);
+#pragma unroll
+      for (int e = 0; e < 8; ++e) v[e] = live ? r[e] : 0.f;
+    } else {
+      v[0] = live ? x0.x : 0.f; v[1] = live ? x0.y : 0.f; v[2] = live ? x0.z : 0.f; v[3] = live ? x0.w : 0.f;
+      v[4] = live ? x1.x : 0.f; v[5] = live ? x1.y : 0.f; v[6] = live ? x1.z : 0.f; v[7] = live ? x1.w : 0.f;
+    }
     uint4 ph, pm, pl;
     split8_bf16x3(v, ph, pm, pl);
     kdst[(0 * 8 + oct) * 64 + key] = ph;
@@ -72,7 +93,7 @@
   }
 }
 
-template <int KSPLIT, bool VL = false>
+template <int KSPLIT, bool VL = false, bool ROPE = false>
 __global__ __launch_bounds__(AX_WAVES * 64, 3) void attn_full_x3_kernel(AttnFullArgs a, const uint4* __restrict__ planes) {
   __shared__ uint4 Ks[AX_TILE_UNITS];
   __shared__ uint4 Vs[AX_TILE_UNITS];
@@ -109,8 +130,16 @@
 #pragma unroll
     for (int s = 0; s < 4; ++s) {
       const float4 x0 = *reinterpret_cast<const float4*>(qrow + 16 * s), x1 = *reinterpret_cast<const float4*>(qrow + 16 * s + 4);
-      const float v[8] = {x0.x * qs, x0.y * qs, x0.z * qs, x0.w * qs, x1.x * qs, x1.y * qs, x1.z * qs, x1.w * qs};
-      split8_bf16x3(v, qp[s][0], qp[s][1], qp[s][2]);
+      if constexpr (ROPE) {
+        static_assert(!VL, "RoPE in the attention kernel: single-sequence entry only");
+        float r[8] = {x0.x, x0.y, x0.z, x0.w, x1.x, x1.y, x1.z, x1.w};
+        rope8(r, a.rope + (long)qi * (AF_D / 2), 2 * s + lh);
+        const float v[8] = {r[0] * qs, r[1] * qs, r[2] * qs, r[3] * qs, r[4] * qs, r[5] * qs, r[6] * qs, r[7] * qs};
+        split8_bf16x3(v, qp[s][0], qp[s][1], qp[s][2]);
+      } else {
+        const float v[8] = {x0.x * qs, x0.y * qs, x0.z * qs, x0.w * qs, x1.x * qs, x1.y * qs, x1.z * qs, x1.w * qs};
+        split8_bf16x3(v, qp[s][0], qp[s][1], qp[s][2]);
+      }
     }
   }
   ax_f32x16 ot[2];
@@ -250,6 +279,13 @@
   const int n_tiles = ceil_div(a.T, AF_KT);
   const int qblocks = ceil_div(a.T, AX_WAVES * AF_QW);
   uint4* pl = reinterpret_cast<uint4*>(planes);
+  if (a.rope) {
+    hipLaunchKernelGGL((attn_kv_planes_kernel<false, true>), dim3(n_tiles, a.B * a.H), dim3(256), 0, st, a, pl);
+    if (split) hipLaunchKernelGGL((attn_full_x3_kernel<AX_KSPLIT, false, true>), dim3(qblocks, a.B * a.H, AX_KSPLIT), dim3(AX_WAVES * 64), 0, st, a, (const uint4*)pl);
+    else hipLaunchKernelGGL((attn_full_x3_kernel<1, false, true>), dim3(qblocks, a.B * a.H), dim3(AX_WAVES * 64), 0, st, a, (const uint4*)pl);
+    IX_HIP(hipGetLastError());
+    return IXTTS_OK;
+  }
   hipLaunchKernelGGL(attn_kv_planes_kernel<false>, dim3(n_tiles, a.B * a.H), dim3(256), 0, st, a, pl);
   if (split) hipLaunchKernelGGL(attn_full_x3_kernel<AX_KSPLIT>, dim3(qblocks, a.B * a.H, AX_KSPLIT), dim3(AX_WAVES * 64), 0, st, a, (const uint4*)pl);
   else hipLaunchKernelGGL(attn_full_x3_kernel<1>, dim3(qblocks, a.B * a.H), dim3(AX_WAVES * 64), 0, st, a, (const uint4*)pl);
diff --git a/voice-tts_amd/csrc/dit_ops.hip b/voice-tts_amd/csrc/dit_ops.hip
--- a/voice-tts_amd/csrc/dit_ops.hip
+++ b/voice-tts_amd/csrc/dit_ops.hip
@@ -53,6 +53,72 @@
       }
       o4[c] = make_float4(fmaf(w.x + wadd, n.x, b.x), fmaf(w.y + wadd, n.y, b.y), fmaf(w.z + wadd, n.z, b.z), fmaf(w.w + wadd, n.w, b.w));
     }
+  }
+}
+
+template <int R>
+__global__ __launch_bounds__(256) void adaln_rmsnorm_planes_kernel(const float* __restrict__ x, const float* __restrict__ mw, const float* __restrict__ mb,
+                                                                   const float* __restrict__ g, uint4* __restrict__ out, long rows, long Mpad, int T, int H,
+                                                                   long mstride, float eps, float wadd) {
+  static_assert(R % 4 == 0, "every wavefront takes R / 4 rows");
+  extern __shared__ float4 nrm[];
+  const int lane = threadIdx.x & 63, wave = threadIdx.x >> 6;
+  const int H4 = H >> 2, pitch = H4 + 1;
+  const float4* g4 = reinterpret_cast<const float4*>(g);
+  for (int j = 0; j < R / 4; ++j) {
+    const int rl = 4 * j + wave;
+    const long row = (long)blockIdx.x * R + rl;
+    float4* dst = nrm + rl * pitch;
+    if (row >= rows) {
+#pragma unroll
+      for (int i = 0; i < ROW_NV; ++i) {
+        const int c = lane + 64 * i;
+        if (c < H4) dst[c] = make_float4(0.f, 0.f, 0.f, 0.f);
+      }
+      continue;
+    }
+    const float4* xr = reinterpret_cast<const float4*>(x + row * H);
+    float4 v[ROW_NV];
+#pragma unroll
+    for (int i = 0; i < ROW_NV; ++i) {
+      const int c = lane + 64 * i;
+      v[i] = (c < H4) ? xr[c] : make_float4(0.f, 0.f, 0.f, 0.f);
+    }
+    float q = 0.f;
+#pragma unroll
+    for (int i = 0; i < ROW_NV; ++i) {
+      const int c = lane + 64 * i;
+      if (c < H4) q += (__fmul_rn(v[i].x, v[i].x) + __fmul_rn(v[i].y, v[i].y)) + (__fmul_rn(v[i].z, v[i].z) + __fmul_rn(v[i].w, v[i].w));
+    }
+    const float rstd = 1.0f / sqrtf(wave_sum(q) / (float)H + eps);
+    const long bidx = row / T;
+    const float4* w4 = reinterpret_cast<const float4*>(mw + bidx * mstride);
+    const float4* b4 = reinterpret_cast<const float4*>(mb + bidx * mstride);
+#pragma unroll
+    for (int i = 0; i < ROW_NV; ++i) {
+      const int c = lane + 64 * i;
+      if (c < H4) {
+        const float4 w = w4[c], b = b4[c], gg = g4[c];
+        const float nx = __fmul_rn(__fmul_rn(v[i].x, rstd), gg.x), ny = __fmul_rn(__fmul_rn(v[i].y, rstd), gg.y);
+        const float nz = __fmul_rn(__fmul_rn(v[i].z, rstd), gg.z), nw = __fmul_rn(__fmul_rn(v[i].w, rstd), gg.w);
+        dst[c] = make_float4(fmaf(w.x + wadd, nx, b.x), fmaf(w.y + wadd, ny, b.y), fmaf(w.z + wadd, nz, b.z), fmaf(w.w + wadd, nw, b.w));
+      }
+    }
+  }
+  __syncthreads();
+  const int units = R * (H >> 3);
+  for (int u = threadIdx.x; u < units; u += 256) {
+    const int r = u % R, ko = u / R;
+    const float4* src = nrm + r * pitch + 2 * ko;
+    const float4 x0 = src[0], x1 = src[1];
+    const float v[8] = {x0.x, x0.y, x0.z, x0.w, x1.x, x1.y, x1.z, x1.w};
+    uint4 ph, pm, pl;
+    split8_bf16x3(v, ph, pm, pl);
+    const int kg = ko >> 1, kh = ko & 1;
+    uint4* base = out + ((long)kg * 6) * Mpad + (long)blockIdx.x * R + r;
+    base[(long)(0 * 2 + kh) * Mpad] = ph;
+    base[(long)(1 * 2 + kh) * Mpad] = pm;
+    base[(long)(2 * 2 + kh) * Mpad] = pl;
   }
 }
 
@@ -163,6 +229,40 @@
   return IXTTS_OK;
 }
 
+template <int R>
+static int launch_adaln_rmsnorm_planes(const float* x_dev, const float* wb_dev, const float* g_dev, void* planes_dev, long rows, long Mpad, int T, int H, float eps,
+                                       hipStream_t st) {
+  const size_t smem = (size_t)R * (H / 4 + 1) * sizeof(float4);
+  auto kern = adaln_rmsnorm_planes_kernel<R>;
+  static bool done = false;
+  if (!done) {
+    IX_HIP(hipFuncSetAttribute((const void*)kern, hipFuncAttributeMaxDynamicSharedMemorySize, 16 * (1024 / 4 + 1) * (int)sizeof(float4)));
+    done = true;
+  }
+  hipLaunchKernelGGL(kern, dim3((unsigned)(Mpad / R)), dim3(256), smem, st, x_dev, wb_dev, wb_dev + H, g_dev, reinterpret_cast<uint4*>(planes_dev), rows, Mpad,
+                     T, H, (long)2 * H, eps, 0.0f);
+  IX_HIP(hipGetLastError());
+  return IXTTS_OK;
+}
+
+extern "C" long ixtts_gemm_x6_rows_padded(long rows);
+
+extern "C" int ixtts_adaln_rmsnorm_planes_f32(const float* x_dev, const float* wb_dev, const float* g_dev, void* planes_dev, int B, int T, int H, float eps,
+                                              int rows_per_block, void* stream) {
+  IX_ARG(x_dev && wb_dev && g_dev && planes_dev, "adaln_rmsnorm_planes: null pointer");
+  IX_ARG(B > 0 && T > 0 && H > 0 && H % 64 == 0 && H <= 1024, "adaln_rmsnorm_planes: bad shape B=%d T=%d H=%d (H a multiple of 64, at most 1024)", B, T, H);
+  const long rows = (long)B * T, Mpad = ixtts_gemm_x6_rows_padded(rows);
+  hipStream_t st = (hipStream_t)stream;
+  switch (rows_per_block) {
+    case 4: return launch_adaln_rmsnorm_planes<4>(x_dev, wb_dev, g_dev, planes_dev, rows, Mpad, T, H, eps, st);
+    case 8: return launch_adaln_rmsnorm_planes<8>(x_dev, wb_dev, g_dev, planes_dev, rows, Mpad, T, H, eps, st);
+    case 0:
+    case 16: return launch_adaln_rmsnorm_planes<16>(x_dev, wb_dev, g_dev, planes_dev, rows, Mpad, T, H, eps, st);
+  }
+  set_error("adaln_rmsnorm_planes: rows_per_block %d (0, 4, 8, 16)", rows_per_block);
+  return IXTTS_ERR_ARG;
+}
+
 extern "C" int ixtts_ln_modulate_f32(const float* x_dev, const float* shift_scale_dev, float* out_dev, int B, int T, int H, float eps, void* stream) {
   IX_ARG(x_dev && shift_scale_dev && out_dev, "ln_modulate: null pointer");
   IX_ARG(B > 0 && T > 0 && H > 0 && H % 4 == 0 && H <= 64 * ROW_NV * 4, "ln_modulate: bad shape B=%d T=%d H=%d", B, T, H);
diff --git a/voice-tts_amd/csrc/gemm_x6.hip b/voice-tts_amd/csrc/gemm_x6.hip
--- a/voice-tts_amd/csrc/gemm_x6.hip
+++ b/voice-tts_amd/csrc/gemm_x6.hip
@@ -26,7 +26,9 @@
   }
 }
 
-__global__ __launch_bounds__(256) void gemm_x6_split_kernel(const float* __restrict__ a, long lda, uint4* __restrict__ out, int M, int K, long Mpad) {
+template <bool REFLECT>
+__global__ __launch_bounds__(256) void gemm_x6_split_kernel(const float* __restrict__ a, long lda, uint4* __restrict__ out, int M, int K, long Mpad, int T = 0,
+                                                            int left = 0, int right = 0) {
   __shared__ float tile[64][65];
   const int r0 = blockIdx.x * 64, k0 = blockIdx.y * 64;
   const int t = threadIdx.x;
@@ -34,7 +36,14 @@
   for (int i = 0; i < 4; ++i) {
     const int r = (t >> 4) + 16 * i, kq = t & 15;
     float4 v = make_float4(0.f, 0.f, 0.f, 0.f);
-    if (r0 + r < M) v = *reinterpret_cast<const float4*>(a + (long)(r0 + r) * lda + k0 + 4 * kq);
+    if (r0 + r < M) {
+      int src = r0 + r;
+      if constexpr (REFLECT) {
+        const int j = src % (left + T + right);
+        src += j < left ? 2 * (left - j) : (j >= left + T ? 2 * (left + T - 1 - j) : 0);
+      }
+      v = *reinterpret_cast<const float4*>(a + (long)src * lda + k0 + 4 * kq);
+    }
     tile[r][4 * kq + 0] = v.x; tile[r][4 * kq + 1] = v.y; tile[r][4 * kq + 2] = v.z; tile[r][4 * kq + 3] = v.w;
   }
   __syncthreads();
@@ -357,8 +366,20 @@
   IX_ARG(a_dev && planes_dev && rows > 0 && K > 0 && K % 64 == 0, "gemm_x6_split: bad argument (K must be a multiple of 64)");
   IX_ARG(lda >= K && lda % 4 == 0 && (reinterpret_cast<uintptr_t>(a_dev) & 15) == 0, "gemm_x6_split: rows must be 16-byte aligned (lda %ld)", lda);
   const long Mpad = ixtts_gemm_x6_rows_padded(rows);
-  hipLaunchKernelGGL(gemm_x6_split_kernel, dim3((unsigned)(Mpad / 64), K / 64), dim3(256), 0, (hipStream_t)stream, a_dev, lda,
-                     reinterpret_cast<uint4*>(planes_dev), (int)rows, K, Mpad);
+  hipLaunchKernelGGL(gemm_x6_split_kernel<false>, dim3((unsigned)(Mpad / 64), K / 64), dim3(256), 0, (hipStream_t)stream, a_dev, lda,
+                     reinterpret_cast<uint4*>(planes_dev), (int)rows, K, Mpad, 0, 0, 0);
+  IX_HIP(hipGetLastError());
+  return IXTTS_OK;
+}
+
+extern "C" int ixtts_gemm_x6_split_reflect(const float* p_dev, void* planes_dev, int B, int T, int K, int left, int right, void* stream) {
+  IX_ARG(p_dev && planes_dev && B > 0 && K > 0 && K % 64 == 0, "gemm_x6_split_reflect: bad argument (K must be a multiple of 64)");
+  IX_ARG(left >= 0 && right >= 0 && T > left && T > right, "gemm_x6_split_reflect: bad shape B=%d T=%d left=%d right=%d", B, T, left, right);
+  IX_ARG((reinterpret_cast<uintptr_t>(p_dev) & 15) == 0 && (long)B * (left + T + right) <= 0x7fffffffL, "gemm_x6_split_reflect: unaligned buffer or too many rows");
+  const long rows = (long)B * (left + T + right);
+  const long Mpad = ixtts_gemm_x6_rows_padded(rows);
+  hipLaunchKernelGGL(gemm_x6_split_kernel<true>, dim3((unsigned)(Mpad / 64), K / 64), dim3(256), 0, (hipStream_t)stream, p_dev, (long)K,
+                     reinterpret_cast<uint4*>(planes_dev), (int)rows, K, Mpad, T, left, right);
   IX_HIP(hipGetLastError());
   return IXTTS_OK;
 }
diff --git a/voice-tts_amd/gemm.py b/voice-tts_amd/gemm.py
--- a/voice-tts_amd/gemm.py
+++ b/voice-tts_amd/gemm.py
@@ -37,20 +37,45 @@
         (x.dim() == 1 or (x.stride(-2) % 4 == 0 and x.stride(-2) >= K))
 
 
+def _plane_buf(device, rows, K, slot):
+    nbytes = (K // 16) * 6 * int(_lib.lib().ixtts_gemm_x6_rows_padded(rows)) * 16
+    key = (device, nbytes, slot)
+    buf = _POOL.get(key)
+    if buf is None:
+        buf = _POOL[key] = torch.empty(nbytes, dtype=torch.uint8, device=device)
+    return buf
+
+
 def split(x, slot=0):
     K = int(x.shape[-1])
     if x.dim() != 2:
         x = x.reshape(-1, K) if x.is_contiguous() else x.contiguous().reshape(-1, K)
     rows, lda = int(x.shape[0]), int(x.stride(0))
-    L = _lib.lib()
-    nbytes = (K // 16) * 6 * int(L.ixtts_gemm_x6_rows_padded(rows)) * 16
-    key = (x.device, nbytes, slot)
-    buf = _POOL.get(key)
-    if buf is None:
-        buf = _POOL[key] = torch.empty(nbytes, dtype=torch.uint8, device=x.device)
+    buf = _plane_buf(x.device, rows, K, slot)
     with torch.cuda.device(x.device):
-        _lib.check(L.ixtts_gemm_x6_split(x.data_ptr(), lda, buf.data_ptr(), rows, K, _lib.current_stream_ptr()), "ixtts_gemm_x6_split")
+        _lib.check(_lib.lib().ixtts_gemm_x6_split(x.data_ptr(), lda, buf.data_ptr(), rows, K, _lib.current_stream_ptr()), "ixtts_gemm_x6_split")
     return Planes(buf, rows, K)
+
+
+def split_reflect(p, T, left, right, slot=0):
+    B, Tp, K = (int(n) for n in p.shape)
+    assert p.is_cuda and p.dtype == torch.float32 and p.is_contiguous() and Tp == left + T + right and K % 64 == 0, (tuple(p.shape), T, left, right)
+    buf = _plane_buf(p.device, B * Tp, K, slot)
+    with torch.cuda.device(p.device):
+        _lib.check(_lib.lib().ixtts_gemm_x6_split_reflect(p.data_ptr(), buf.data_ptr(), B, int(T), K, int(left), int(right), _lib.current_stream_ptr()),
+                   "ixtts_gemm_x6_split_reflect")
+    return Planes(buf, B * Tp, K)
+
+
+def adaln_rmsnorm_planes(x, wb, g, eps=1e-5, slot=0, rows_per_block=0):
+    B, T, H = (int(n) for n in x.shape)
+    assert x.is_cuda and x.dtype == torch.float32 and H % 64 == 0 and H <= 1024, (tuple(x.shape), x.dtype)
+    x, wb = x.contiguous(), wb.contiguous()
+    buf = _plane_buf(x.device, B * T, H, slot)
+    with torch.cuda.device(x.device):
+        _lib.check(_lib.lib().ixtts_adaln_rmsnorm_planes_f32(x.data_ptr(), wb.data_ptr(), g.data_ptr(), buf.data_ptr(), B, T, H, C.c_float(eps),
+                                                             int(rows_per_block), _lib.current_stream_ptr()), "ixtts_adaln_rmsnorm_planes_f32")
+    return Planes(buf, B * T, H)
 
 
 def linear(x, pl, out=None, accumulate=False, bias=True, tile=0, row0=0, rows=None, lead=None):
diff --git a/voice-tts_amd/s2mel.py b/voice-tts_amd/s2mel.py
--- a/voice-tts_amd/s2mel.py
+++ b/voice-tts_amd/s2mel.py
@@ -101,7 +101,7 @@
     return y[..., : y.shape[-1] - extra]
 
 
-def attn_full(q, k, v, scale=None):
+def attn_full(q, k, v, scale=None, rope=None):
     import ctypes as C
 
     from . import _lib
@@ -115,12 +115,25 @@
     L = _lib.lib()
     nws = L.ixtts_attn_full_workspace_bytes(B, Hh, T)
     ws = torch.empty(nws, device=q.device, dtype=torch.uint8)
+    if rope is not None:
+        tab = torch.view_as_real(rope)
+        assert tab.is_cuda and tab.is_contiguous() and tuple(tab.shape) == (T, d // 2, 2) and tab.data_ptr() % 16 == 0
+        with torch.cuda.device(q.device):
+            rc = L.ixtts_attn_full_rope_f32(q.data_ptr(), k.data_ptr(), v.data_ptr(), out.data_ptr(), tab.data_ptr(), B, Hh, T, d, q.stride(0),
+                                            q.stride(1), q.stride(2), out.stride(0), out.stride(1), out.stride(2), C.c_float(sc), ws.data_ptr(), nws,
+                                            _lib.current_stream_ptr())
+        _lib.check(rc, "ixtts_attn_full_rope_f32")
+        return out
     with torch.cuda.device(q.device):
         rc = L.ixtts_attn_full_f32(q.data_ptr(), k.data_ptr(), v.data_ptr(), out.data_ptr(), B, Hh, T, d, q.stride(0), q.stride(1),
                                    q.stride(2), out.stride(0), out.stride(1), out.stride(2), C.c_float(sc), ws.data_ptr(), nws,
                                    _lib.current_stream_ptr())
     _lib.check(rc, "ixtts_attn_full_f32")
     return out
+
+
+def passes_fused():
+    return os.environ.get("IXTTS_S2MEL_PASSES", "fused") != "separate"
 
 
 def _lin(x, W, name):
@@ -502,9 +515,11 @@
         H, nh, hd = self.cfg["hidden_dim"], self.cfg["num_heads"], self.head_dim
         fc = self._rope_cache(T)
         if mask is None and hd == 64 and qkv.is_cuda:
+            v4 = qkv.view(B, T, 3, nh, hd)
+            if passes_fused() and os.environ.get("IXTTS_ATTN_FULL", "x3") != "f32":
+                return attn_full(v4[:, :, 0], v4[:, :, 1], v4[:, :, 2], rope=fc).reshape(B * T, H)
             with torch.cuda.device(qkv.device):
                 _hip_call("ixtts_rope_qk_f32", qkv.data_ptr(), torch.view_as_real(fc).data_ptr(), B, T, H, hd)
-            v4 = qkv.view(B, T, 3, nh, hd)
             return attn_full(v4[:, :, 0], v4[:, :, 1], v4[:, :, 2]).reshape(B * T, H)
         q, k, v = qkv.view(B, T, 3 * H).split([H, H, H], dim=-1)
         q = self._rotary(q.reshape(B, T, nh, hd), fc)
@@ -520,6 +535,7 @@
         wb_all = F.linear(c, self.proj_w, self.proj_b).view(B, 2 * L + 1, 2 * H).transpose(0, 1).contiguous()
         x = x.reshape(B * T, H)
         x6 = x.is_cuda and self._x6(self.x6_w13)
+        norm_planes = x6 and H <= 1024 and passes_fused()
         skips = []
         for i in range(L):
             p = f"cfm.estimator.transformer.layers.{i}."
@@ -529,8 +545,11 @@
             a = adaln_rmsnorm(x.view(B, T, H), wb_all[2 * i], W[p + "attention_norm.norm.weight"])
             y = self._attention(F.linear(a.view(B * T, H), W[p + "attention.wqkv.weight"]), B, T, mask)
             h = torch.addmm(x, y, W[p + "attention.wo.weight"].t()) if 0 < i <= L // 2 else x.addmm_(y, W[p + "attention.wo.weight"].t())
-            f = adaln_rmsnorm(h.view(B, T, H), wb_all[2 * i + 1], W[p + "ffn_norm.norm.weight"]).view(B * T, H)
-            u = G.pair_linear(f, self.x6_w13[i], G.SWIGLU) if x6 else swiglu(F.linear(f, self.w13[i]))
+            if norm_planes:
+                u = G.pair_linear(G.adaln_rmsnorm_planes(h.view(B, T, H), wb_all[2 * i + 1], W[p + "ffn_norm.norm.weight"]), self.x6_w13[i], G.SWIGLU)
+            else:
+                f = adaln_rmsnorm(h.view(B, T, H), wb_all[2 * i + 1], W[p + "ffn_norm.norm.weight"]).view(B * T, H)
+                u = G.pair_linear(f, self.x6_w13[i], G.SWIGLU) if x6 else swiglu(F.linear(f, self.w13[i]))
             x = h.addmm_(u, W[p + "feed_forward.w2.weight"].t())
             if i < L // 2:
                 skips.append(x)
@@ -602,17 +621,20 @@
         right = tot // 2
         left = tot - right
         Tp = T_ + tot
-        P = torch.empty(B, Tp, Hw, device=h.device, dtype=h.dtype)
+        x6 = self._x6(self.x6_wn)
+        through_map = x6 and passes_fused() and T_ > max(left, right)
+        P = (torch.zeros if through_map else torch.empty)(B, Tp, Hw, device=h.device, dtype=h.dtype)
         P[:, left:left + T_] = h
         P2 = P.view(B * Tp, Hw)
         M = B * Tp - tot
         centre = P2[left:left + M]
         out = torch.empty(B * Tp, Hw, device=h.device, dtype=h.dtype)
-        x6 = self._x6(self.x6_wn)
         for i in range(nl):
-            reflect_halo_rows(P, T_, left, right)
+            if not through_map:
+                reflect_halo_rows(P, T_, left, right)
             if x6:
-                acts = G.pair_linear(G.split(P2), self.x6_wn[i], G.GATE, taps=k, gate=g, gate_off=i * 2 * Hw, rows_per_batch=Tp)
+                planes = G.split_reflect(P, T_, left, right) if through_map else G.split(P2)
+                acts = G.pair_linear(planes, self.x6_wn[i], G.GATE, taps=k, gate=g, gate_off=i * 2 * Hw, rows_per_batch=Tp)
             else:
                 acc = torch.addmm(self.wn_bin[i], P2[:M], self.wn_taps[i][0].t())
                 for j in range(1, k):
```
